# ru-wang/slam-plus-plus

Hardware: AMD Instinct MI355X
Metric: Λ-solve block-nnz/sec + batch GN iters/sec, Venice BA, 1→8 MI355X (higher is better)
Workload: dtype f64; 1 GPU; venice871-shaped synthetic BA (871 cams, 530304 points, 2838740 observations, LM-damped); nnzb=3369915, n=1596138, mode=schur+dense, n_reduced=5226, schur_pairs=12875640, parallelism=single GPU

## Files before the change

### include/spp_hip.h

```cpp
#ifndef SPP_HIP_H
#define SPP_HIP_H

#include <stddef.h>
#include <stdint.h>

#ifdef __cplusplus
extern "C" {
#endif

#define SPP_OK            0
#define SPP_NOT_POSDEF    1
#define SPP_E_BADARG     -1
#define SPP_E_NOMEM      -2
#define SPP_E_HIP        -3
#define SPP_E_NO_DEVICE  -4
#define SPP_E_STATE      -5
#define SPP_E_UNSUPPORTED -6

#define SPP_MODE_AUTO     0
#define SPP_MODE_SPARSE   1
#define SPP_MODE_SCHUR    2
#define SPP_MODE_SCHUR_SPARSE 3

#define SPP_FLAG_PROFILE  1
#define SPP_FLAG_SCHUR_PARTIAL 2

typedef struct spp_ctx spp_ctx;

spp_ctx *spp_create(int device, int flags);
void spp_destroy(spp_ctx *ctx);
int spp_free_memory(spp_ctx *ctx);
int spp_last_error(const spp_ctx *ctx, char *buf, size_t buf_size);
double *spp_host_staging(spp_ctx *ctx, int64_t n_doubles);
int spp_set_stream(spp_ctx *ctx, void *hip_stream);
int spp_synchronize(spp_ctx *ctx);

int spp_analyze(spp_ctx *ctx, int64_t nb, const int64_t *h_col_ptr, const int64_t *h_row_idx,
	const int64_t *h_blk_off, const int32_t *h_dim, int mode);

int spp_set_shard(spp_ctx *ctx, int rank, int world_size);

#define SPP_MODE_SCHUR_MIS 4

#define SPP_INFO_MODE           0
#define SPP_INFO_N              1
#define SPP_INFO_NNZB           2
#define SPP_INFO_NVALS          3
#define SPP_INFO_FACTOR_NNZ     4
#define SPP_INFO_FACTOR_FLOPS   5
#define SPP_INFO_N_REDUCED      6
#define SPP_INFO_N_POSES        7
#define SPP_INFO_N_LANDMARKS    8
#define SPP_INFO_SCHUR_PAIRS    9
#define SPP_INFO_N_OBS          10
#define SPP_INFO_SOLVE_BYTES    11
#define SPP_INFO_N_SUPERNODES   12
#define SPP_INFO_N_LEVELS       13
#define SPP_INFO_S_LD           14
#define SPP_INFO_S_NNZB         15
#define SPP_INFO_DENSE_STREAMED 16
#define SPP_INFO_LM_STREAM      17
#define SPP_INFO_BS_GROUPS      18
#define SPP_INFO_SCHUR_SIDE     19
#define SPP_INFO_S_CLEAR        20
#define SPP_INFO_S_DEVICE_PTR   21
#define SPP_INFO_ASM_HUB_CHUNK   22
#define SPP_INFO_SOLVE_ASYNC    23
#define SPP_INFO_FACTOR_KEPT    24
#define SPP_INFO_SPARSE_FACTOR_KEPT 25
#define SPP_INFO_SCHUR_SPARSE_FACTOR_KEPT 26
int spp_get_info(const spp_ctx *ctx, int what, int64_t *out);
int spp_get_ordering(const spp_ctx *ctx, int64_t *h_order);
int64_t spp_sparse_fronts(const spp_ctx *ctx, int64_t capacity, int32_t *h, int32_t *w, int32_t *pad, int32_t *cls, int32_t *level,
	int32_t *parent, int32_t *team);

#define SPP_ORDER_AMD 0
#define SPP_ORDER_ND  1
int spp_block_ordering(int64_t nb, const int64_t *col_ptr, const int64_t *row_idx, int method, int64_t *h_order);

int spp_schur_plan_host(int64_t nb, const int32_t *dim, const int64_t *col_ptr, const int64_t *row_idx, int shard_rank,
	int shard_world, int sparse_S, int64_t *out, double *seconds);

int spp_factor_solve(spp_ctx *ctx, const double *h_vals, double *h_rhs_inout);

int spp_factor_solve_device(spp_ctx *ctx, const double *d_vals, double *d_rhs_inout);

int spp_solve_device(spp_ctx *ctx, const double *d_vals, double *d_B, int64_t ldb, int64_t nrhs);
int spp_marginals_device(spp_ctx *ctx, const double *d_vals, int64_t n_sel, const int64_t *h_vertices, double *d_cov);

int spp_sparse_solve_device(spp_ctx *ctx, double *d_B, int64_t ldb, int64_t nrhs);
int spp_sparse_marginals_device(spp_ctx *ctx, int64_t n_sel, const int64_t *h_vertices, double *d_cov);
int spp_sparse_sigma_device(spp_ctx *ctx, double *d_sigma);

int spp_schur_sigma_device(spp_ctx *ctx, const double *d_vals, double *d_sigma);

int spp_schur_sparse_solve_device(spp_ctx *ctx, const double *d_vals, double *d_B, int64_t ldb, int64_t nrhs);
int spp_schur_sparse_marginals_device(spp_ctx *ctx, const double *d_vals, int64_t n_sel, const int64_t *h_vertices, double *d_cov);
int spp_schur_sparse_sigma_device(spp_ctx *ctx, const double *d_vals, double *d_sigma);

int spp_schur_buffer_size(const spp_ctx *ctx, int64_t *n_doubles);
int spp_schur_form(spp_ctx *ctx, const double *d_vals, const double *d_rhs, double *d_S_rhs);
int spp_schur_finish(spp_ctx *ctx, const double *d_vals, double *d_S_rhs, double *d_rhs_inout);
int spp_schur_packed_size(const spp_ctx *ctx, int64_t *n_doubles);
int spp_schur_pack(spp_ctx *ctx, const double *d_S_rhs, double *d_packed);
int spp_schur_unpack(spp_ctx *ctx, const double *d_packed, double *d_S_rhs);

int spp_assemble_analyze(spp_ctx *ctx, int64_t nv, const int32_t *h_dim,
	int64_t ne, const int64_t *h_v0, const int64_t *h_v1, int d0, int d1, int rd,
	int64_t unary_vertex);
int spp_assemble_get_structure(const spp_ctx *ctx, int64_t *h_col_ptr, int64_t *h_row_idx,
	int64_t *h_blk_off);
int spp_assemble_device(spp_ctx *ctx, const double *d_J0, const double *d_J1,
	const double *d_Omega, const double *d_r, double damping, double *d_vals_out, double *d_eta_out);
int spp_assemble_set_edge_weights(spp_ctx *ctx, const double *d_w);
#define SPP_MAX_EDGE_GROUPS 4
int spp_assemble_analyze_groups(spp_ctx *ctx, int64_t nv, const int32_t *h_dim, int n_groups,
	const int64_t *h_ne, const int64_t *const *h_v0, const int64_t *const *h_v1, const int64_t *const *h_seq,
	const int32_t *h_d0, const int32_t *h_d1, const int32_t *h_rd, int64_t unary_vertex);
int spp_assemble_groups_device(spp_ctx *ctx, const double *const *d_J0, const double *const *d_J1,
	const double *const *d_Omega, const double *const *d_r, double damping, double *d_vals_out, double *d_eta_out);
int spp_assemble_set_group_edge_weights(spp_ctx *ctx, int group, const double *d_w);
int spp_assemble_analyze_ternary(spp_ctx *ctx, int64_t nv, const int32_t *h_dim, int64_t ne, const int64_t *h_v0,
	const int64_t *h_v1, const int64_t *h_v2, int d0, int d1, int d2, int live2, int rd, int64_t unary_vertex);
int spp_assemble_ternary_device(spp_ctx *ctx, const double *d_J0, const double *d_J1, const double *d_J2,
	const double *d_Omega, const double *d_r, double damping, double *d_vals_out, double *d_eta_out);
int spp_edge_robust_weights_device(spp_ctx *ctx, int64_t n_edges, int rd, int kind, double scale, double param,
	const double *d_r, double *d_w_out);

int spp_se2_linearize_device(spp_ctx *ctx, int64_t n_edges, const int32_t *d_v0, const int32_t *d_v1,
	const double *d_poses, const double *d_measurements, double *d_J0, double *d_J1, double *d_r);
int spp_se2_update_device(spp_ctx *ctx, int64_t n_vertices, double *d_poses, const double *d_dx, int apply,
	double *h_dx_norm2);

int spp_se2_linearize_at_device(spp_ctx *ctx, int64_t n_edges, const int64_t *d_off0, const int64_t *d_off1,
	const double *d_state, const double *d_measurements, double *d_J0, double *d_J1, double *d_r);
int spp_se2_rb_linearize_device(spp_ctx *ctx, int64_t n_edges, const int64_t *d_pose_off, const int64_t *d_lm_off,
	const double *d_state, const double *d_measurements, double *d_J0, double *d_J1, double *d_r);
int spp_slam2d_update_device(spp_ctx *ctx, int64_t n, double *d_state, const double *d_dx, int64_t n_pose_angles,
	const int64_t *d_angle_off, int apply, double *h_dx_norm2);

int spp_se3_linearize_device(spp_ctx *ctx, int64_t n_edges, const int32_t *d_v0, const int32_t *d_v1,
	const double *d_poses, const double *d_measurements, double *d_J0, double *d_J1, double *d_r);
int spp_se3_update_device(spp_ctx *ctx, int64_t n_vertices, double *d_poses, const double *d_dx, int apply,
	double *h_dx_norm2);

int spp_se3_linearize_at_device(spp_ctx *ctx, int64_t n_edges, const int64_t *d_off0, const int64_t *d_off1,
	const double *d_state, const double *d_measurements, double *d_J0, double *d_J1, double *d_r);
int spp_se3_xyz_linearize_device(spp_ctx *ctx, int64_t n_edges, const int64_t *d_pose_off, const int64_t *d_lm_off,
	const double *d_state, const double *d_measurements, double *d_J0, double *d_J1, double *d_r);
int spp_slam3d_update_device(spp_ctx *ctx, int64_t n, double *d_state, const double *d_dx, int64_t n_poses,
	const int64_t *d_pose_off, int apply, double *h_dx_norm2);

int spp_rocv_range_linearize_device(spp_ctx *ctx, int64_t n_edges, const int64_t *d_recv_off, const int64_t *d_lm_off,
	const double *d_state, const double *d_measurements, double *d_J0, double *d_J1, double *d_r);
int spp_rocv_cv_linearize_device(spp_ctx *ctx, int64_t n_edges, const int64_t *d_off0, const int64_t *d_off1,
	const double *d_state, const double *d_dt, double *d_J0, double *d_J1, double *d_r);

int spp_ba_linearize_device(spp_ctx *ctx, int64_t n_obs, const int32_t *d_cam_of, const int32_t *d_pt_of,
	const double *d_cams, const double *d_intrinsics, const double *d_points, const double *d_measurements,
	double *d_J0, double *d_J1, double *d_r);
int spp_ba_update_device(spp_ctx *ctx, int64_t n_cams, double *d_cams, const int64_t *d_cam_dxoff,
	int64_t n_points, double *d_points, const int64_t *d_pt_dxoff, const double *d_dx, int64_t n_dx, int apply,
	double *h_dx_norm2);

int spp_sim3_ba_linearize_device(spp_ctx *ctx, int64_t n_obs, const int32_t *d_cam_of, const int32_t *d_pt_of,
	const double *d_cams, const double *d_intrinsics, const double *d_points, const double *d_measurements,
	double *d_J0, double *d_J1, double *d_r);
int spp_sim3_update_device(spp_ctx *ctx, int64_t n_cams, double *d_cams, const int64_t *d_cam_dxoff,
	int64_t n_points, double *d_points, const int64_t *d_pt_dxoff, const double *d_dx, int64_t n_dx, int apply,
	double *h_dx_norm2);

int spp_ba_stereo_linearize_device(spp_ctx *ctx, int64_t n_obs, const int32_t *d_cam_of, const int32_t *d_pt_of,
	const double *d_cams, const double *d_intrinsics, const double *d_points, const double *d_measurements,
	double *d_J0, double *d_J1, double *d_r);

int spp_ba_intrinsics_linearize_device(spp_ctx *ctx, int64_t n_obs, const int32_t *d_cam_of, const int32_t *d_pt_of,
	const int32_t *d_intr_of, const double *d_cams, const double *d_intrinsics, const double *d_points,
	const double *d_measurements, double *d_J0, double *d_J1, double *d_J2, double *d_r);
int spp_ba_intrinsics_update_device(spp_ctx *ctx, int64_t n_intrinsics, double *d_intrinsics, const int64_t *d_intr_dxoff,
	const double *d_dx, int apply, double *h_dx_norm2);

int spp_edge_chi2_device(spp_ctx *ctx, int64_t n_edges, int rd, const double *d_r, const double *d_Omega, double *h_chi2);
int spp_edge_hessian_maxdiag_device(spp_ctx *ctx, int64_t n_edges, int rd, int d0, int d1, const double *d_J0,
	const double *d_J1, const double *d_Omega, double *h_max);
int spp_lm_gain_denominator_device(spp_ctx *ctx, int64_t n, const double *d_dx, const double *d_eta, double alpha,
	double *h_out);

int spp_device_malloc(spp_ctx *ctx, size_t bytes, void **d_ptr);
int spp_device_free(spp_ctx *ctx, void *d_ptr);
int spp_memcpy_h2d(spp_ctx *ctx, void *d_dst, const void *h_src, size_t bytes);
int spp_memcpy_d2h(spp_ctx *ctx, void *h_dst, const void *d_src, size_t bytes);
int spp_memcpy_d2d(spp_ctx *ctx, void *d_dst, const void *d_src, size_t bytes);

int spp_set_profiling(spp_ctx *ctx, int on);

#define SPP_PHASE_PERMUTE   0
#define SPP_PHASE_SCHUR_INV 1
#define SPP_PHASE_SCHUR_GEMM 2
#define SPP_PHASE_SCHUR_RHS 3
#define SPP_PHASE_FACTOR    4
#define SPP_PHASE_TRISOLVE  5
#define SPP_PHASE_BACKSUBST 6
#define SPP_PHASE_ASSEMBLE  7
#define SPP_PHASE_TOTAL     8
#define SPP_N_PHASES        9
int spp_get_phase_ms(spp_ctx *ctx, double *ms_out );
int spp_get_dominant_kernel(spp_ctx *ctx, double *ms_total, int64_t *n_launches, double *flops);

int spp_microbench_copy(spp_ctx *ctx, size_t bytes, int iters, double *gb_per_s);
int spp_microbench_mfma_f64(spp_ctx *ctx, int iters, double *tflops);
int spp_microbench_ctile(spp_ctx *ctx, int n, int iters, double *gb_per_s);
int spp_microbench_update(spp_ctx *ctx, int64_t m, int iters, double *ms_per_launch);

int spp_dense_potrf_upper(spp_ctx *ctx, double *d_A, int64_t n, int64_t ld);
int spp_dense_posv(spp_ctx *ctx, double *d_A, int64_t n, int64_t ld, double *d_b);
int spp_dense_posv_multi(spp_ctx *ctx, double *d_A, int64_t n, int64_t ld, double *d_B, int64_t ldb, int64_t nrhs);
int spp_dense_potri(spp_ctx *ctx, double *d_A, int64_t n, int64_t ld, double *d_Z, int64_t ldz);
int spp_schur_sigma_dense_device(spp_ctx *ctx);
int spp_schur_sparse_sigma_inverse_device(spp_ctx *ctx);
int spp_dense_posv_masked(spp_ctx *ctx, double *d_A, int64_t n, int64_t ld, double *d_b, const uint64_t *words, int64_t nwords);
int spp_tile_mask_host(int64_t n, int bs, int64_t nblk, const int32_t *i1, const int32_t *i2, int has_rhs, int fill,
	uint64_t *words, int64_t *n_updates);
int spp_schur_tile_mask_host(int64_t nb, const int32_t *dim, const int64_t *col_ptr, const int64_t *row_idx, int shard_rank,
	int shard_world, uint64_t *words);
int spp_schur_cam_order_host(int64_t nb, const int32_t *dim, const int64_t *col_ptr, const int64_t *row_idx, int shard_rank,
	int shard_world, int flags, const int64_t *order_in, int64_t *cam_order, double *figures);
int spp_tail_order_host(int64_t n, int has_rhs, const uint64_t *words, int64_t nwords, int resident, int early, double beta,
	int32_t *table, int32_t *info);
int spp_tail_plan_host(int64_t n, int has_rhs, const uint64_t *words, int64_t nwords, const int32_t *step_order, int64_t norder,
	int front, int tail_rows, int resident, int early, double beta, uint64_t *rowbits, int32_t *steps, int32_t *table, int32_t *info);
int spp_dense_posv_ordered(spp_ctx *ctx, double *d_A, int64_t n, int64_t ld, double *d_b, const uint64_t *words, int64_t nwords,
	const int32_t *step_order);
int spp_tail_step_order_host(int64_t n, const uint64_t *words, int64_t nwords, int32_t *step_order);
int spp_schur_step_order_host(int64_t nb, const int32_t *dim, const int64_t *col_ptr, const int64_t *row_idx, int shard_rank,
	int shard_world, int flags, int32_t *step_order);
int spp_dense_gemm_tn_sub(spp_ctx *ctx, int64_t m, int64_t n, int64_t k,
	const double *d_A, int64_t lda, const double *d_B, int64_t ldb, double *d_C, int64_t ldc);
int spp_dense_gemm_tn_sub_upper(spp_ctx *ctx, int64_t m, int64_t n, int64_t k,
	const double *d_A, int64_t lda, const double *d_B, int64_t ldb, double *d_C, int64_t ldc);
int spp_dense_front_factor(spp_ctx *ctx, double *d_F, int64_t ld, int64_t w, int64_t h, double *d_image);

const char *spp_version(void);

#ifdef __cplusplus
}
#endif
#endif
```

### slam_plus_plus_amd/api.py

```python
import ctypes
import os

import numpy as np

_HERE = os.path.dirname(os.path.abspath(__file__))
LIB_PATH = os.environ.get("SPP_LIB") or os.path.join(_HERE, "libspp_hip.so")

SPP_OK, SPP_NOT_POSDEF = 0, 1
MODE_AUTO, MODE_SPARSE, MODE_SCHUR, MODE_SCHUR_SPARSE, MODE_SCHUR_MIS = 0, 1, 2, 3, 4
FLAG_PROFILE = 1
INFO = dict(MODE=0, N=1, NNZB=2, NVALS=3, FACTOR_NNZ=4, FACTOR_FLOPS=5, N_REDUCED=6, N_POSES=7,
            N_LANDMARKS=8, SCHUR_PAIRS=9, N_OBS=10, SOLVE_BYTES=11, N_SUPERNODES=12, N_LEVELS=13, S_LD=14, S_NNZB=15, DENSE_STREAMED=16,
            LM_STREAM=17, BS_GROUPS=18, SCHUR_SIDE=19, S_CLEAR=20, S_DEVICE_PTR=21, ASM_HUB_CHUNK=22, SOLVE_ASYNC=23, FACTOR_KEPT=24,
            SPARSE_FACTOR_KEPT=25, SCHUR_SPARSE_FACTOR_KEPT=26)
PHASES = ["permute", "schur_inv", "schur_gemm", "schur_rhs", "factor", "trisolve", "backsubst", "assemble", "total"]

EXPORTS = [
    "spp_create", "spp_destroy", "spp_free_memory", "spp_last_error", "spp_host_staging", "spp_set_stream", "spp_synchronize",
    "spp_analyze", "spp_set_shard", "spp_get_info", "spp_get_ordering", "spp_sparse_fronts", "spp_factor_solve",
    "spp_factor_solve_device", "spp_solve_device", "spp_marginals_device", "spp_sparse_solve_device", "spp_sparse_marginals_device", "spp_sparse_sigma_device",
    "spp_schur_sigma_device", "spp_dense_potri", "spp_schur_sigma_dense_device",
    "spp_schur_sparse_solve_device", "spp_schur_sparse_marginals_device", "spp_schur_sparse_sigma_device",
    "spp_schur_sparse_sigma_inverse_device",
    "spp_schur_buffer_size", "spp_schur_form", "spp_schur_finish",
    "spp_schur_packed_size", "spp_schur_pack", "spp_schur_unpack",
    "spp_assemble_analyze", "spp_assemble_get_structure", "spp_assemble_device", "spp_assemble_set_edge_weights",
    "spp_assemble_analyze_groups", "spp_assemble_groups_device", "spp_assemble_set_group_edge_weights",
    "spp_assemble_analyze_ternary", "spp_assemble_ternary_device", "spp_ba_intrinsics_linearize_device",
    "spp_ba_intrinsics_update_device",
    "spp_se2_linearize_at_device", "spp_se2_rb_linearize_device", "spp_slam2d_update_device",
    "spp_se3_linearize_at_device", "spp_se3_xyz_linearize_device", "spp_slam3d_update_device", "spp_rocv_range_linearize_device",
    "spp_rocv_cv_linearize_device", "spp_device_malloc",
    "spp_device_free", "spp_memcpy_h2d", "spp_memcpy_d2h", "spp_memcpy_d2d", "spp_get_phase_ms", "spp_get_dominant_kernel",
    "spp_microbench_copy", "spp_microbench_mfma_f64", "spp_microbench_ctile", "spp_microbench_update", "spp_block_ordering", "spp_schur_plan_host", "spp_set_profiling", "spp_se2_linearize_device", "spp_se2_update_device", "spp_ba_linearize_device", "spp_ba_stereo_linearize_device", "spp_ba_update_device", "spp_sim3_ba_linearize_device", "spp_sim3_update_device", "spp_se3_linearize_device", "spp_se3_update_device", "spp_edge_chi2_device", "spp_edge_robust_weights_device", "spp_edge_hessian_maxdiag_device",
    "spp_lm_gain_denominator_device", "spp_dense_potrf_upper", "spp_dense_posv", "spp_dense_posv_multi",
    "spp_dense_posv_masked", "spp_tile_mask_host", "spp_schur_tile_mask_host", "spp_tail_order_host", "spp_tail_plan_host", "spp_schur_cam_order_host",
    "spp_dense_posv_ordered", "spp_tail_step_order_host", "spp_schur_step_order_host",
    "spp_dense_gemm_tn_sub", "spp_dense_gemm_tn_sub_upper", "spp_dense_front_factor", "spp_version",
]

_lib = None
_c_i64p = ctypes.POINTER(ctypes.c_int64)
_c_i32p = ctypes.POINTER(ctypes.c_int32)
_c_f64p = ctypes.POINTER(ctypes.c_double)


class SppError(RuntimeError):
    """std::runtime_error of the C++ adapter (reference LinearSolver_Schur_GPU.cpp:734-797)."""


def load_library():
    global _lib
    if _lib is not None:
        return _lib
    if not os.path.exists(LIB_PATH):
        raise SppError("libspp_hip.so is not built: run `python -m slam_plus_plus_amd.build` "
                       "(hipcc --offload-arch=gfx950); there is no CPU fallback")
    lib = ctypes.CDLL(LIB_PATH)
    vp, i64, i32, dbl, cint = ctypes.c_void_p, ctypes.c_int64, ctypes.c_int32, ctypes.c_double, ctypes.c_int
    sig = {
        "spp_create": (vp, [cint, cint]),
        "spp_destroy": (None, [vp]),
        "spp_free_memory": (cint, [vp]),
        "spp_last_error": (cint, [vp, ctypes.c_char_p, ctypes.c_size_t]),
        "spp_host_staging": (vp, [vp, i64]),
        "spp_set_stream": (cint, [vp, vp]),
        "spp_synchronize": (cint, [vp]),
        "spp_analyze": (cint, [vp, i64, vp, vp, vp, vp, cint]),
        "spp_set_shard": (cint, [vp, cint, cint]),
        "spp_get_info": (cint, [vp, cint, _c_i64p]),
        "spp_get_ordering": (cint, [vp, vp]),
        "spp_sparse_fronts": (i64, [vp, i64, vp, vp, vp, vp, vp, vp, vp]),
        "spp_factor_solve": (cint, [vp, vp, vp]),
        "spp_factor_solve_device": (cint, [vp, vp, vp]),
        "spp_solve_device": (cint, [vp, vp, vp, i64, i64]),
        "spp_marginals_device": (cint, [vp, vp, i64, vp, vp]),
        "spp_sparse_solve_device": (cint, [vp, vp, i64, i64]),
        "spp_sparse_marginals_device": (cint, [vp, i64, vp, vp]),
        "spp_sparse_sigma_device": (cint, [vp, vp]),
        "spp_schur_sigma_device": (cint, [vp, vp, vp]),
        "spp_schur_sigma_dense_device": (cint, [vp]),
        "spp_schur_sparse_solve_device": (cint, [vp, vp, vp, i64, i64]),
        "spp_schur_sparse_marginals_device": (cint, [vp, vp, i64, vp, vp]),
        "spp_schur_sparse_sigma_device": (cint, [vp, vp, vp]),
        "spp_schur_sparse_sigma_inverse_device": (cint, [vp]),
        "spp_dense_potri": (cint, [vp, vp, i64, i64, vp, i64]),
        "spp_schur_buffer_size": (cint, [vp, _c_i64p]),
        "spp_schur_form": (cint, [vp, vp, vp, vp]),
        "spp_schur_finish": (cint, [vp, vp, vp, vp]),
        "spp_schur_packed_size": (cint, [vp, _c_i64p]),
        "spp_schur_pack": (cint, [vp, vp, vp]),
        "spp_schur_unpack": (cint, [vp, vp, vp]),
        "spp_assemble_analyze": (cint, [vp, i64, vp, i64, vp, vp, cint, cint, cint, i64]),
        "spp_assemble_get_structure": (cint, [vp, vp, vp, vp]),
        "spp_assemble_device": (cint, [vp, vp, vp, vp, vp, dbl, vp, vp]),
        "spp_assemble_set_edge_weights": (cint, [vp, vp]),
        "spp_assemble_analyze_groups": (cint, [vp, i64, vp, cint, vp, vp, vp, vp, vp, vp, vp, i64]),
        "spp_assemble_groups_device": (cint, [vp, vp, vp, vp, vp, dbl, vp, vp]),
        "spp_assemble_set_group_edge_weights": (cint, [vp, cint, vp]),
        "spp_assemble_analyze_ternary": (cint, [vp, i64, vp, i64, vp, vp, vp, cint, cint, cint, cint, cint, i64]),
        "spp_assemble_ternary_device": (cint, [vp, vp, vp, vp, vp, vp, dbl, vp, vp]),
        "spp_ba_intrinsics_linearize_device": (cint, [vp, i64, vp, vp, vp, vp, vp, vp, vp, vp, vp, vp, vp]),
        "spp_ba_intrinsics_update_device": (cint, [vp, i64, vp, vp, vp, cint, _c_f64p]),
        "spp_se2_linearize_at_device": (cint, [vp, i64, vp, vp, vp, vp, vp, vp, vp]),
        "spp_se2_rb_linearize_device": (cint, [vp, i64, vp, vp, vp, vp, vp, vp, vp]),
        "spp_slam2d_update_device": (cint, [vp, i64, vp, vp, i64, vp, cint, _c_f64p]),
        "spp_se3_linearize_at_device": (cint, [vp, i64, vp, vp, vp, vp, vp, vp, vp]),
        "spp_se3_xyz_linearize_device": (cint, [vp, i64, vp, vp, vp, vp, vp, vp, vp]),
        "spp_slam3d_update_device": (cint, [vp, i64, vp, vp, i64, vp, cint, _c_f64p]),
        "spp_rocv_range_linearize_device": (cint, [vp, i64, vp, vp, vp, vp, vp, vp, vp]),
        "spp_rocv_cv_linearize_device": (cint, [vp, i64, vp, vp, vp, vp, vp, vp, vp]),
        "spp_device_malloc": (cint, [vp, ctypes.c_size_t, ctypes.POINTER(vp)]),
        "spp_device_free": (cint, [vp, vp]),
        "spp_memcpy_h2d": (cint, [vp, vp, vp, ctypes.c_size_t]),
        "spp_memcpy_d2h": (cint, [vp, vp, vp, ctypes.c_size_t]),
        "spp_memcpy_d2d": (cint, [vp, vp, vp, ctypes.c_size_t]),
        "spp_get_phase_ms": (cint, [vp, _c_f64p]),
        "spp_get_dominant_kernel": (cint, [vp, _c_f64p, _c_i64p, _c_f64p]),
        "spp_microbench_copy": (cint, [vp, ctypes.c_size_t, cint, _c_f64p]),
        "spp_microbench_mfma_f64": (cint, [vp, cint, _c_f64p]),
        "spp_microbench_ctile": (cint, [vp, cint, cint, _c_f64p]),
        "spp_microbench_update": (cint, [vp, ctypes.c_int64, cint, _c_f64p]),
        "spp_block_ordering": (cint, [ctypes.c_int64, vp, vp, cint, vp]),
        "spp_schur_plan_host": (cint, [ctypes.c_int64, vp, vp, vp, cint, cint, cint, vp, vp]),
        "spp_set_profiling": (cint, [vp, cint]),
        "spp_se2_linearize_device": (cint, [vp, ctypes.c_int64, vp, vp, vp, vp, vp, vp, vp]),
        "spp_se2_update_device": (cint, [vp, ctypes.c_int64, vp, vp, cint, _c_f64p]),
        "spp_se3_linearize_device": (cint, [vp, ctypes.c_int64, vp, vp, vp, vp, vp, vp, vp]),
        "spp_se3_update_device": (cint, [vp, ctypes.c_int64, vp, vp, cint, _c_f64p]),
        "spp_edge_chi2_device": (cint, [vp, ctypes.c_int64, cint, vp, vp, _c_f64p]),
        "spp_edge_robust_weights_device": (cint, [vp, ctypes.c_int64, cint, cint, dbl, dbl, vp, vp]),
        "spp_edge_hessian_maxdiag_device": (cint, [vp, ctypes.c_int64, cint, cint, cint, vp, vp, vp, _c_f64p]),
        "spp_lm_gain_denominator_device": (cint, [vp, ctypes.c_int64, vp, vp, ctypes.c_double, _c_f64p]),
        "spp_ba_linearize_device": (cint, [vp, ctypes.c_int64, vp, vp, vp, vp, vp, vp, vp, vp, vp]),
        "spp_ba_stereo_linearize_device": (cint, [vp, ctypes.c_int64, vp, vp, vp, vp, vp, vp, vp, vp, vp]),
        "spp_ba_update_device": (cint, [vp, ctypes.c_int64, vp, vp, ctypes.c_int64, vp, vp, vp, ctypes.c_int64, cint, _c_f64p]),
        "spp_sim3_ba_linearize_device": (cint, [vp, ctypes.c_int64, vp, vp, vp, vp, vp, vp, vp, vp, vp]),
        "spp_sim3_update_device": (cint, [vp, ctypes.c_int64, vp, vp, ctypes.c_int64, vp, vp, vp, ctypes.c_int64, cint, _c_f64p]),
        "spp_dense_potrf_upper": (cint, [vp, vp, i64, i64]),
        "spp_dense_posv": (cint, [vp, vp, i64, i64, vp]),
        "spp_dense_posv_multi": (cint, [vp, vp, i64, i64, vp, i64, i64]),
        "spp_dense_posv_masked": (cint, [vp, vp, i64, i64, vp, vp, i64]),
        "spp_tile_mask_host": (cint, [i64, cint, i64, vp, vp, cint, cint, vp, vp]),
        "spp_schur_tile_mask_host": (cint, [i64, vp, vp, vp, cint, cint, vp]),
        "spp_tail_order_host": (cint, [i64, cint, vp, i64, cint, cint, dbl, vp, vp]),
        "spp_tail_plan_host": (cint, [i64, cint, vp, i64, vp, i64, cint, cint, cint, cint, dbl, vp, vp, vp, vp]),
        "spp_schur_cam_order_host": (cint, [i64, vp, vp, vp, cint, cint, cint, vp, vp, vp]),
        "spp_dense_posv_ordered": (cint, [vp, vp, i64, i64, vp, vp, i64, vp]),
        "spp_tail_step_order_host": (cint, [i64, vp, i64, vp]),
        "spp_schur_step_order_host": (cint, [i64, vp, vp, vp, cint, cint, cint, vp]),
        "spp_dense_gemm_tn_sub": (cint, [vp, i64, i64, i64, vp, i64, vp, i64, vp, i64]),
        "spp_dense_gemm_tn_sub_upper": (cint, [vp, i64, i64, i64, vp, i64, vp, i64, vp, i64]),
        "spp_dense_front_factor": (cint, [vp, vp, i64, i64, i64, vp]),
        "spp_version": (ctypes.c_char_p, []),
    }
    for name, (res, args) in sig.items():
        fn = getattr(lib, name)
        fn.restype = res
        fn.argtypes = args
    _lib = lib
    return lib


def _ptr(a):
    return a.ctypes.data_as(ctypes.c_void_p)


ORDER_AMD, ORDER_ND = 0, 1


def block_ordering(lam, method=ORDER_AMD):
    lib = load_library()
    col_ptr = np.ascontiguousarray(lam.col_ptr, dtype=np.int64)
    row_idx = np.ascontiguousarray(lam.row_idx, dtype=np.int64)
    out = np.empty(lam.nb, dtype=np.int64)
    code = lib.spp_block_ordering(lam.nb, _ptr(col_ptr), _ptr(row_idx), method, _ptr(out))
    if code != 0:
        raise SppError("spp_block_ordering failed: %d" % code)
    return out


def schur_plan_host(lam, shard_rank=0, shard_world=1, sparse_S=False, mis=False):
    lib = load_library()
    col_ptr = np.ascontiguousarray(lam.col_ptr, dtype=np.int64)
    row_idx = np.ascontiguousarray(lam.row_idx, dtype=np.int64)
    dim = np.ascontiguousarray(lam.dim, dtype=np.int32)
    out = np.zeros(9, dtype=np.int64)
    sec = ctypes.c_double(0.0)
    code = lib.spp_schur_plan_host(lam.nb, _ptr(dim), _ptr(col_ptr), _ptr(row_idx), shard_rank, shard_world,
                                   (1 if sparse_S else 0) | (2 if mis else 0), _ptr(out), ctypes.byref(sec))
    if code != 0:
        raise SppError("spp_schur_plan_host failed: %d" % code)
    keys = ("nc", "nl", "no", "n_pairs", "n_sblk", "n_items", "n_multi", "checksum", "checksum_all")
    d = dict(zip(keys, (int(v) for v in out)))
    d["seconds"] = sec.value
    return d


def tile_mask_host(n, bs, i1, i2, has_rhs=True, fill=True):
    lib = load_library()
    i1 = np.ascontiguousarray(i1, dtype=np.int32)
    i2 = np.ascontiguousarray(i2, dtype=np.int32)
    words = np.zeros(64, dtype=np.uint64)
    upd = ctypes.c_int64(0)
    code = lib.spp_tile_mask_host(n, bs, i1.size, _ptr(i1), _ptr(i2), 1 if has_rhs else 0, 1 if fill else 0, _ptr(words),
                                  ctypes.byref(upd))
    if code < 0:
        raise SppError("spp_tile_mask_host failed: %d" % code)
    return words[:code].copy(), upd.value


def schur_tile_mask_host(lam, shard_rank=0, shard_world=1):
    lib = load_library()
    col_ptr = np.ascontiguousarray(lam.col_ptr, dtype=np.int64)
    row_idx = np.ascontiguousarray(lam.row_idx, dtype=np.int64)
    dim = np.ascontiguousarray(lam.dim, dtype=np.int32)
    words = np.zeros(64, dtype=np.uint64)
    code = lib.spp_schur_tile_mask_host(lam.nb, _ptr(dim), _ptr(col_ptr), _ptr(row_idx), shard_rank, shard_world, _ptr(words))
    if code < 0:
        raise SppError("spp_schur_tile_mask_host failed: %d" % code)
    return words[:code].copy()


def schur_cam_order_host(lam, order=None, sparse_S=False, mis=False, shard_rank=0, shard_world=1):
    lib = load_library()
    col_ptr = np.ascontiguousarray(lam.col_ptr, dtype=np.int64)
    row_idx = np.ascontiguousarray(lam.row_idx, dtype=np.int64)
    dim = np.ascontiguousarray(lam.dim, dtype=np.int32)
    nc = int((dim == dim.max()).sum()) if not mis else int(dim.size)
    out = np.full(max(nc, 1), -1, dtype=np.int64)
    fig = np.zeros(8, dtype=np.float64)
    oin = None if order is None else np.ascontiguousarray(order, dtype=np.int64)
    if oin is not None and oin.size != nc:
        raise SppError("schur_cam_order_host: order must list every camera once")
    code = lib.spp_schur_cam_order_host(lam.nb, _ptr(dim), _ptr(col_ptr), _ptr(row_idx), shard_rank, shard_world,
                                        (1 if sparse_S else 0) | (2 if mis else 0),
                                        _ptr(oin) if oin is not None else None, _ptr(out), _ptr(fig))
    if code < 0:
        raise SppError("spp_schur_cam_order_host failed: %d" % code)
    keys = ("tiles", "updates", "path", "cost_us")
    natural = dict(zip(keys, (int(fig[0]), int(fig[1]), int(fig[2]), float(fig[3]))))
    chosen = dict(zip(keys, (int(fig[4]), int(fig[5]), int(fig[6]), float(fig[7]))))
    return out[out >= 0], bool(code), natural, chosen


def tail_order_host(n, words, has_rhs=True, resident=256, early=True, beta=0.0):
    lib = load_library()
    words = np.ascontiguousarray(words if words is not None else [], dtype=np.uint64)
    table = np.zeros(64 * 65 // 2 + 64, dtype=np.int32)
    info = np.zeros(5, dtype=np.int32)
    code = lib.spp_tail_order_host(int(n), 1 if has_rhs else 0, _ptr(words) if words.size else None, words.size, int(resident),
                                   int(early), float(beta), _ptr(table), _ptr(info))
    if code < 0:
        raise SppError("spp_tail_order_host failed: %d" % code)
    tiles = [(int(t) >> 16, int(t) & 0xffff) for t in table[:code]]
    return tiles, dict(zip(("n_early", "r_star", "rows_resident", "live_demand", "widest"), (int(v) for v in info)))


TAIL_NO_STEP = 127
SPP_E_BADARG = -1


def tail_plan_host(n, words, step_order=None, front=0, has_rhs=True, tail_rows=44, resident=256, early=3, beta=0.0, tail_mask=True):
    lib = load_library()
    words = np.ascontiguousarray(words if words is not None else [], dtype=np.uint64)
    so = np.ascontiguousarray(step_order if step_order is not None else [], dtype=np.int32)
    rowbits = np.zeros(65, dtype=np.uint64)
    steps = np.zeros(72, dtype=np.int32)
    table = np.zeros(64 * 65 // 2 + 64, dtype=np.int32)
    info = np.zeros(5, dtype=np.int32)
    code = lib.spp_tail_plan_host(int(n), 1 if has_rhs else 0, _ptr(words) if words.size else None, words.size,
                                  _ptr(so) if so.size else None, so.size, int(front), int(tail_rows), int(resident),
                                  int(early) | (0 if tail_mask else 4), float(beta), _ptr(rowbits), _ptr(steps), _ptr(table), _ptr(info))
    if code < 0:
        err = SppError("spp_tail_plan_host failed: %d" % code)
        err.code = code
        raise err
    if code == 0:
        return None
    tr = -(-int(n) // 128) - int(front)
    return {"rowbits": [int(w) for w in rowbits[:tr + 1]], "steps": steps.tolist(),
            "tiles": [(int(t) >> 16, int(t) & 0xffff) for t in table[:code]],
            "info": dict(zip(("n_early", "r_star", "rows_resident", "live_demand", "widest"), (int(v) for v in info)))}


def tail_step_order_host(n, words):
    lib = load_library()
    words = np.ascontiguousarray(words, dtype=np.uint64)
    out = np.zeros(64, dtype=np.int32)
    code = lib.spp_tail_step_order_host(int(n), _ptr(words), words.size, _ptr(out))
    if code < 0:
        raise SppError("spp_tail_step_order_host failed: %d" % code)
    return out[:code].copy()


def schur_step_order_host(lam, sparse_S=False, mis=False, shard_rank=0, shard_world=1):
    lib = load_library()
    col_ptr = np.ascontiguousarray(lam.col_ptr, dtype=np.int64)
    row_idx = np.ascontiguousarray(lam.row_idx, dtype=np.int64)
    dim = np.ascontiguousarray(lam.dim, dtype=np.int32)
    out = np.zeros(64, dtype=np.int32)
    code = lib.spp_schur_step_order_host(lam.nb, _ptr(dim), _ptr(col_ptr), _ptr(row_idx), shard_rank, shard_world,
                                         (1 if sparse_S else 0) | (2 if mis else 0), _ptr(out))
    if code < 0:
        raise SppError("spp_schur_step_order_host failed: %d" % code)
    return out[:code].copy()


class DeviceArray:

    def __init__(self, ctx, n, dtype=np.float64):
        self.ctx, self.n, self.dtype = ctx, int(n), np.dtype(dtype)
        p = ctypes.c_void_p()
        ctx._check(ctx.lib.spp_device_malloc(ctx.h, self.n * self.dtype.itemsize, ctypes.byref(p)))
        self.ptr = p.value

    @classmethod
    def from_host(cls, ctx, arr):
        arr = np.ascontiguousarray(arr)
        d = cls(ctx, arr.size, arr.dtype)
        d.upload(arr)
        return d

    def upload(self, arr):
        arr = np.ascontiguousarray(arr, dtype=self.dtype)
        assert arr.size == self.n
        self.ctx._check(self.ctx.lib.spp_memcpy_h2d(self.ctx.h, self.ptr, _ptr(arr), arr.nbytes))

    def download(self):
        out = np.empty(self.n, dtype=self.dtype)
        self.ctx._check(self.ctx.lib.spp_memcpy_d2h(self.ctx.h, _ptr(out), self.ptr, out.nbytes))
        return out

    def copy_from(self, other):
        assert other.n * other.dtype.itemsize <= self.n * self.dtype.itemsize
        self.ctx._check(self.ctx.lib.spp_memcpy_d2d(self.ctx.h, self.ptr, other.ptr, other.n * other.dtype.itemsize))

    def free(self):
        if self.ptr:
            self.ctx.lib.spp_device_free(self.ctx.h, self.ptr)
            self.ptr = None


class Context:

    def __init__(self, device=0, flags=0):
        self.lib = load_library()
        self.h = self.lib.spp_create(int(device), int(flags))
        if not self.h:
            raise SppError("spp_create failed: no usable HIP device %d (the solver has no CPU fallback)" % device)

    def close(self):
        if getattr(self, "h", None):
            self.lib.spp_destroy(self.h)
            self.h = None

    def __del__(self):
        try:
            self.close()
        except Exception:
            pass

    def last_error(self):
        buf = ctypes.create_string_buffer(1024)
        self.lib.spp_last_error(self.h, buf, 1024)
        return buf.value.decode(errors="replace")

    def _check(self, code):
        if code < 0:
            if code == -2:
                raise MemoryError(self.last_error())
            raise SppError("spp error %d: %s" % (code, self.last_error()))
        return code

    def analyze(self, bcsc, mode=MODE_AUTO):
        self._keep = bcsc
        return self._check(self.lib.spp_analyze(self.h, bcsc.nb, _ptr(bcsc.col_ptr), _ptr(bcsc.row_idx),
                                                 _ptr(bcsc.blk_off), _ptr(bcsc.dim), mode))

    def set_shard(self, rank, world):
        return self._check(self.lib.spp_set_shard(self.h, rank, world))

    def info(self, key):
        out = ctypes.c_int64()
        self._check(self.lib.spp_get_info(self.h, INFO[key], ctypes.byref(out)))
        return out.value

    def ordering(self, nb):
        out = np.empty(nb, dtype=np.int64)
        self._check(self.lib.spp_get_ordering(self.h, _ptr(out)))
        return out

    def sparse_fronts(self):
        keys = ("h", "w", "pad", "cls", "level", "parent", "team")
        ns = self._check(self.lib.spp_sparse_fronts(self.h, 0, None, None, None, None, None, None, None))
        out = {k: np.zeros(ns, dtype=np.int32) for k in keys}
        if ns:
            self._check(self.lib.spp_sparse_fronts(self.h, ns, *[_ptr(out[k]) for k in keys]))
        return out

    def se2_linearize_device(self, n_edges, d_v0, d_v1, d_poses, d_meas, d_J0, d_J1, d_r):
        return self._check(self.lib.spp_se2_linearize_device(self.h, n_edges, d_v0, d_v1, d_poses, d_meas, d_J0, d_J1, d_r))

    def se2_update_device(self, n_vertices, d_poses, d_dx, apply=True):
        out = ctypes.c_double()
        self._check(self.lib.spp_se2_update_device(self.h, n_vertices, d_poses, d_dx, 1 if apply else 0, ctypes.byref(out)))
        return out.value ** 0.5

    def se2_linearize_at_device(self, n_edges, d_off0, d_off1, d_state, d_meas, d_J0, d_J1, d_r):
        return self._check(self.lib.spp_se2_linearize_at_device(self.h, n_edges, d_off0, d_off1, d_state, d_meas, d_J0, d_J1, d_r))

    def se2_rb_linearize_device(self, n_edges, d_pose_off, d_lm_off, d_state, d_meas, d_J0, d_J1, d_r):
        return self._check(self.lib.spp_se2_rb_linearize_device(self.h, n_edges, d_pose_off, d_lm_off, d_state, d_meas, d_J0, d_J1, d_r))

    def slam2d_update_device(self, n, d_state, d_dx, n_pose_angles, d_angle_off, apply=True):
        out = ctypes.c_double()
        self._check(self.lib.spp_slam2d_update_device(self.h, n, d_state, d_dx, n_pose_angles, d_angle_off, 1 if apply else 0,
                                                      ctypes.byref(out)))
        return out.value ** 0.5

    def se3_linearize_at_device(self, n_edges, d_off0, d_off1, d_state, d_meas, d_J0, d_J1, d_r):
        return self._check(self.lib.spp_se3_linearize_at_device(self.h, n_edges, d_off0, d_off1, d_state, d_meas, d_J0, d_J1, d_r))

    def se3_xyz_linearize_device(self, n_edges, d_pose_off, d_lm_off, d_state, d_meas, d_J0, d_J1, d_r):
        return self._check(self.lib.spp_se3_xyz_linearize_device(self.h, n_edges, d_pose_off, d_lm_off, d_state, d_meas, d_J0, d_J1, d_r))

    def slam3d_update_device(self, n, d_state, d_dx, n_poses, d_pose_off, apply=True):
        out = ctypes.c_double()
        self._check(self.lib.spp_slam3d_update_device(self.h, n, d_state, d_dx, n_poses, d_pose_off, 1 if apply else 0,
                                                      ctypes.byref(out)))
        return out.value ** 0.5

    def rocv_range_linearize_device(self, n_edges, d_recv_off, d_lm_off, d_state, d_meas, d_J0, d_J1, d_r):
        return self._check(self.lib.spp_rocv_range_linearize_device(self.h, n_edges, d_recv_off, d_lm_off, d_state, d_meas, d_J0, d_J1, d_r))

    def rocv_cv_linearize_device(self, n_edges, d_off0, d_off1, d_state, d_dt, d_J0, d_J1, d_r):
        return self._check(self.lib.spp_rocv_cv_linearize_device(self.h, n_edges, d_off0, d_off1, d_state, d_dt, d_J0, d_J1, d_r))

# ... 346 lines not shown
```

### slam_plus_plus_amd/csrc/spp_api.cpp

```cpp

#include "spp_internal.h"
#include <string.h>
#include <new>

using namespace spp;

namespace spp {

void phases_reset(spp_ctx *ctx)
{
	if(!(ctx->flags & SPP_FLAG_PROFILE))
		return;
	if(!ctx->timer.created) {
		for(int i = 0; i < 2 * SPP_N_PHASES; ++ i)
			SPP_HIP_CHECK(hipEventCreate(&ctx->timer.ev[i]));
		ctx->timer.created = true;
	}
	for(int i = 0; i < SPP_N_PHASES; ++ i) {
		ctx->timer.used[i] = false;
		ctx->phase_ms[i] = 0;
	}
	ctx->dom_used = 0;
	ctx->dom_flops = 0;
}

void phase_begin(spp_ctx *ctx, int phase)
{
	if(!(ctx->flags & SPP_FLAG_PROFILE) || !ctx->timer.created)
		return;
	SPP_HIP_CHECK(hipEventRecord(ctx->timer.ev[2 * phase], ctx->stream));
}

void phase_end(spp_ctx *ctx, int phase)
{
	if(!(ctx->flags & SPP_FLAG_PROFILE) || !ctx->timer.created)
		return;
	SPP_HIP_CHECK(hipEventRecord(ctx->timer.ev[2 * phase + 1], ctx->stream));
	ctx->timer.used[phase] = true;
}

void phases_collect(spp_ctx *ctx)
{
	if(!(ctx->flags & SPP_FLAG_PROFILE) || !ctx->timer.created)
		return;
	SPP_HIP_CHECK(hipStreamSynchronize(ctx->stream));
	for(int i = 0; i < SPP_N_PHASES; ++ i) {
		if(!ctx->timer.used[i])
			continue;
		float ms = 0;
		if(hipEventElapsedTime(&ms, ctx->timer.ev[2 * i], ctx->timer.ev[2 * i + 1]) == hipSuccess)
			ctx->phase_ms[i] = ms;
	}
}

void dom_begin(spp_ctx *ctx)
{
	if(!(ctx->flags & SPP_FLAG_PROFILE))
		return;
	if(ctx->dom_used + 2 > ctx->dom_events.size()) {
		size_t old = ctx->dom_events.size();
		ctx->dom_events.resize(old + 64);
		for(size_t i = old; i < ctx->dom_events.size(); ++ i)
			SPP_HIP_CHECK(hipEventCreate(&ctx->dom_events[i]));
	}
	SPP_HIP_CHECK(hipEventRecord(ctx->dom_events[ctx->dom_used], ctx->stream));
}

void dom_end(spp_ctx *ctx, double flops)
{
	if(!(ctx->flags & SPP_FLAG_PROFILE))
		return;
	SPP_HIP_CHECK(hipEventRecord(ctx->dom_events[ctx->dom_used + 1], ctx->stream));
	ctx->dom_used += 2;
	ctx->dom_flops += flops;
}

}

static inline void drop_kept_factors(spp_ctx *ctx)
{
	ctx->schur.factor_kept = false;
	ctx->schur.sparse_factor_kept = false;
	ctx->sparse_factor_kept = false;
}

static void ctx_drain(spp_ctx *ctx)
{
	(void)hipStreamSynchronize(ctx->stream);
	if(ctx->side_stream)
		(void)hipStreamSynchronize(ctx->side_stream);
	ctx->status_pending = false;
}

#define SPP_TRY(ctx) try {
#define SPP_CATCH(ctx) } catch(const spp::Error &e) { if(ctx) (ctx)->last_error = e.what(); return e.code; } \
	catch(const std::bad_alloc &) { if(ctx) (ctx)->last_error = "host allocation failed"; return SPP_E_NOMEM; } \
	catch(const std::exception &e) { if(ctx) (ctx)->last_error = e.what(); return SPP_E_HIP; }

static inline void store_if(double *h_out, double value)
{
	if(h_out)
		*h_out = value;
}

template <class Body>
static int geometry_call(spp_ctx *ctx, Body body)
{
	SPP_TRY(ctx)
	SPP_HIP_CHECK(hipSetDevice(ctx->device));
	body();
	return SPP_OK;
	SPP_CATCH(ctx)
}

extern "C" {

const char *spp_version(void)
{
	return "slam_plus_plus_amd 0.1 (gfx950, fp64)";
}

spp_ctx *spp_create(int device, int flags)
{
	int count = 0;
	if(hipGetDeviceCount(&count) != hipSuccess || count <= 0 || device < 0 || device >= count)
		return nullptr;
	if(hipSetDevice(device) != hipSuccess)
		return nullptr;
	spp_ctx *ctx = new(std::nothrow) spp_ctx;
	if(!ctx)
		return nullptr;
	ctx->device = device;
	ctx->flags = flags;
	if(hipStreamCreateWithFlags(&ctx->stream, hipStreamNonBlocking) != hipSuccess) {
		delete ctx;
		return nullptr;
	}
	ctx->own_stream = true;
	return ctx;
}

int spp_free_memory(spp_ctx *ctx)
{
	if(!ctx)
		return SPP_E_BADARG;
	SPP_TRY(ctx)
	(void)hipSetDevice(ctx->device);
	ctx_drain(ctx);
	drop_kept_factors(ctx);
	ctx->schur.release_all();
	sparse_release(ctx);
	assemble_release(ctx);
	ctx->dense.trsm_w.release();
	ctx->again_panel.release();
	ctx->again_cols.release();
	ctx->again_rows.release();
	ctx->dense.tinv.release();
	ctx->dense.tinv_all.release();
	ctx->dense.xtmp.release();
	ctx->dense.la_cnt.release();
	ctx->dense.la_trace.release();
	ctx->geom_partial.release();
	ctx->dense.flags.release();
	ctx->dense.trsv_pay.release();
	ctx->dense.trsv_m.release();
	ctx->dense.tail_pub.release();
	ctx->dense.tail_order.release();
	ctx->dense.tail_plan.key = TailPlan::Key();
	ctx->dense.tail_dinv.release();
	ctx->dense.tail_epoch = 0;
	ctx->dense.epoch = 0;
	ctx->dense.sync.release();
	ctx->dense.fuse_cnt.release();
	ctx->dense.fuse_expect.clear();
	ctx->dense.sync_epoch = 0;
	ctx->d_vals.release();
	ctx->d_rhs.release();
	ctx->mode = -1;
	return SPP_OK;
	SPP_CATCH(ctx)
}

void spp_destroy(spp_ctx *ctx)
{
	if(!ctx)
		return;
	if(ctx->plan_trash.joinable())
		ctx->plan_trash.join();
	spp_free_memory(ctx);
	ctx->dense.info.release();
	if(ctx->dense.aux) {
		dense_aux_park(ctx->device, ctx->dense.aux);
		(void)hipEventDestroy(ctx->dense.ev[0]);
		(void)hipEventDestroy(ctx->dense.ev[1]);
	}
	if(ctx->dense.chain) {
		(void)hipStreamDestroy(ctx->dense.chain);
		if(ctx->dense.ev_chain)
			(void)hipEventDestroy(ctx->dense.ev_chain);
	}
	if(ctx->side_stream) {
		(void)hipStreamDestroy(ctx->side_stream);
		(void)hipEventDestroy(ctx->side_ev[0]);
		(void)hipEventDestroy(ctx->side_ev[1]);
	}
	for(int i = 0; i < 2; ++ i)
		if(ctx->status_ev[i])
			(void)hipEventDestroy(ctx->status_ev[i]);
	if(ctx->h_status)
		(void)hipHostFree(ctx->h_status);
	if(ctx->dense.h_chain_err)
		(void)hipHostFree(ctx->dense.h_chain_err);
	if(ctx->h_staging)
		(void)hipHostFree(ctx->h_staging);
	if(ctx->timer.created)
		for(int i = 0; i < 2 * SPP_N_PHASES; ++ i)
			(void)hipEventDestroy(ctx->timer.ev[i]);
	for(size_t i = 0; i < ctx->dom_events.size(); ++ i)
		(void)hipEventDestroy(ctx->dom_events[i]);
	if(ctx->own_stream && ctx->stream)
		(void)hipStreamDestroy(ctx->stream);
	delete ctx;
}

int spp_last_error(const spp_ctx *ctx, char *buf, size_t buf_size)
{
	if(!ctx || !buf || !buf_size)
		return SPP_E_BADARG;
	strncpy(buf, ctx->last_error.c_str(), buf_size - 1);
	buf[buf_size - 1] = 0;
	return SPP_OK;
}

double *spp_host_staging(spp_ctx *ctx, int64_t n_doubles)
{
	if(!ctx || n_doubles < 0)
		return nullptr;
	if((size_t)n_doubles <= ctx->h_staging_cap && ctx->h_staging)
		return ctx->h_staging;
	(void)hipSetDevice(ctx->device);
	(void)hipStreamSynchronize(ctx->stream);
	if(ctx->h_staging) {
		(void)hipHostFree(ctx->h_staging);
		ctx->h_staging = nullptr;
		ctx->h_staging_cap = 0;
	}
	const size_t want = (size_t)(n_doubles > 0 ? n_doubles : 1);
	if(hipHostMalloc((void**)&ctx->h_staging, want * sizeof(double), hipHostMallocDefault) != hipSuccess) {
		(void)hipGetLastError();
		ctx->h_staging = nullptr;
		ctx->last_error = "hipHostMalloc of the staging buffer failed";
		return nullptr;
	}
	ctx->h_staging_cap = want;
	return ctx->h_staging;
}

int spp_set_stream(spp_ctx *ctx, void *hip_stream)
{
	if(!ctx)
		return SPP_E_BADARG;
	ctx_drain(ctx);
	if(ctx->own_stream && ctx->stream)
		(void)hipStreamDestroy(ctx->stream);
	ctx->stream = (hipStream_t)hip_stream;
	ctx->own_stream = false;
	return SPP_OK;
}

int spp_synchronize(spp_ctx *ctx)
{
	if(!ctx)
		return SPP_E_BADARG;
	SPP_TRY(ctx)
	SPP_HIP_CHECK(hipStreamSynchronize(ctx->stream));
	dense_chain_check(ctx);
	return SPP_OK;
	SPP_CATCH(ctx)
}

int spp_set_profiling(spp_ctx *ctx, int on)
{
	if(!ctx)
		return SPP_E_BADARG;
	ctx->flags = on ? (ctx->flags | SPP_FLAG_PROFILE) : (ctx->flags & ~SPP_FLAG_PROFILE);
	return SPP_OK;
}

int spp_set_shard(spp_ctx *ctx, int rank, int world_size)
{
	if(!ctx || world_size < 1 || rank < 0 || rank >= world_size)
		return SPP_E_BADARG;
	drop_kept_factors(ctx);
	ctx->shard_rank = rank;
	ctx->shard_world = world_size;
	return SPP_OK;
}

int spp_analyze(spp_ctx *ctx, int64_t nb, const int64_t *col_ptr, const int64_t *row_idx,
	const int64_t *blk_off, const int32_t *dim, int mode)
{
	if(!ctx)
		return SPP_E_BADARG;
	SPP_TRY(ctx)
	SPP_REQUIRE(nb > 0 && col_ptr && row_idx && blk_off && dim, SPP_E_BADARG, "spp_analyze: null or empty structure");
	SPP_REQUIRE(col_ptr[0] == 0 && col_ptr[nb] >= nb, SPP_E_BADARG, "spp_analyze: column pointers must start at 0 and hold every diagonal block");
	SPP_HIP_CHECK(hipSetDevice(ctx->device));
	ctx->mode = -1;
	drop_kept_factors(ctx);
	ctx_drain(ctx);
	VClock clk("spp_analyze");
	Structure st;
	st.nb = nb;
	st.nnzb = col_ptr[nb];
	st.col_ptr.assign(col_ptr, col_ptr + nb + 1);
	SPP_REQUIRE(st.nnzb >= nb, SPP_E_BADARG, "spp_analyze: fewer blocks than block columns");
	for(int64_t j = 0; j < nb; ++ j)
		SPP_REQUIRE(col_ptr[j + 1] > col_ptr[j], SPP_E_BADARG, "every block column needs its diagonal block");
	st.dim.assign(dim, dim + nb);
	st.base.resize(nb + 1);
	st.base[0] = 0;
	for(int64_t j = 0; j < nb; ++ j) {
		SPP_REQUIRE(dim[j] > 0 && dim[j] <= 8, SPP_E_BADARG, "block widths must be in 1..8");
		st.base[j + 1] = st.base[j] + dim[j];
	}
	st.n = st.base[nb];
	st.row_idx.resize(st.nnzb);
	st.blk_off.resize(st.nnzb);
	{
		const int nt = plan_threads(st.nnzb);
		std::vector<int64_t> jcut, nvals_t(nt, 0);
		balanced_cuts(st.col_ptr, nt, jcut);
		run_threads(nt, [&](int t) {
			const int64_t p0 = col_ptr[jcut[t]], p1 = col_ptr[jcut[t + 1]];
			if(p1 > p0) {
				memcpy(st.row_idx.data() + p0, row_idx + p0, (size_t)(p1 - p0) * sizeof(int64_t));
				memcpy(st.blk_off.data() + p0, blk_off + p0, (size_t)(p1 - p0) * sizeof(int64_t));
			}
			int64_t nv = 0;
			for(int64_t j = jcut[t]; j < jcut[t + 1]; ++ j) {
				for(int64_t p = col_ptr[j]; p < col_ptr[j + 1]; ++ p) {
					const int64_t i = row_idx[p];
					SPP_REQUIRE(i >= 0 && i <= j, SPP_E_BADARG, "only the upper triangle may be stored");
					SPP_REQUIRE(p == col_ptr[j] || row_idx[p - 1] < i, SPP_E_BADARG, "rows must ascend within a column");
					SPP_REQUIRE(blk_off[p] >= 0, SPP_E_BADARG, "negative block offset");
					nv = std::max<int64_t>(nv, blk_off[p] + (int64_t)dim[i] * dim[j]);
				}
				SPP_REQUIRE(row_idx[col_ptr[j + 1] - 1] == j, SPP_E_BADARG, "diagonal block missing (must be last in its column)");
			}
			nvals_t[t] = nv;
		});
		st.nvals = 0;
		for(int t = 0; t < nt; ++ t)
			st.nvals = std::max(st.nvals, nvals_t[t]);
	}
	ctx->st = std::move(st);
	Structure &st_ref = ctx->st;
	clk.lap("structure copied + validated");
	ctx->schur.release_all();
	sparse_release(ctx);
	clk.lap("old plans released");
	int dp, dl;
	int chosen = mode;
	if(mode == SPP_MODE_AUTO) {
		chosen = SPP_MODE_SPARSE;
		if(schur_applicable(st_ref, &dp, &dl)) {
			int64_t n_red = 0;
			for(int64_t j = 0; j < nb; ++ j)
				n_red += (dim[j] == dp) ? dp : 0;
			chosen = (n_red <= 16384) ? SPP_MODE_SCHUR : SPP_MODE_SCHUR_SPARSE;
		}
	}
	SPP_REQUIRE(chosen == SPP_MODE_SCHUR || chosen == SPP_MODE_SPARSE || chosen == SPP_MODE_SCHUR_SPARSE ||
		chosen == SPP_MODE_SCHUR_MIS, SPP_E_BADARG, "unknown mode");
	SPP_REQUIRE((chosen != SPP_MODE_SPARSE && chosen != SPP_MODE_SCHUR_MIS) || ctx->shard_world == 1, SPP_E_UNSUPPORTED,
		"only the Schur modes shard (over landmarks); pose graphs run as replicas (DESIGN.md, multi-GPU)");
	ctx->mode = -1;
	if(chosen == SPP_MODE_SCHUR || chosen == SPP_MODE_SCHUR_SPARSE || chosen == SPP_MODE_SCHUR_MIS) {
		const bool mis = chosen == SPP_MODE_SCHUR_MIS;
		const bool sparse_S = chosen != SPP_MODE_SCHUR;
		build_schur_plan(ctx, sparse_S, mis);
		clk.lap("schur plan (all of it)");
		ctx->schur.mis = mis;
		ctx->order.clear();
		ctx->order.reserve((size_t)st_ref.nb);
		if(sparse_S) {
			sparse_analyze(ctx, ctx->schur.s_st);
			std::vector<int64_t> red = ctx->order;
			ctx->order.clear();
			for(size_t i = 0; i < red.size(); ++ i)
				ctx->order.push_back(ctx->schur.pose_block[red[i]]);
			chosen = SPP_MODE_SCHUR;
		} else
		for(size_t i = 0; i < ctx->schur.pose_block.size(); ++ i)
			ctx->order.push_back(ctx->schur.pose_block[i]);
		for(int64_t j = 0; j < st_ref.nb; ++ j)
			if(ctx->schur.is_lm[j])
				ctx->order.push_back(j);
	} else
		sparse_analyze(ctx, ctx->st);
	ctx->mode = chosen;
	clk.lap("plan + ordering");
	return SPP_OK;
	SPP_CATCH(ctx)
}

int spp_get_info(const spp_ctx *ctx, int what, int64_t *out)
{
	if(!ctx || !out)
		return SPP_E_BADARG;
	if(ctx->mode < 0 && what != SPP_INFO_NNZB && what != SPP_INFO_NVALS && what != SPP_INFO_N && what != SPP_INFO_DENSE_STREAMED &&
	   what != SPP_INFO_ASM_HUB_CHUNK && what != SPP_INFO_FACTOR_KEPT && what != SPP_INFO_SPARSE_FACTOR_KEPT &&
	   what != SPP_INFO_SCHUR_SPARSE_FACTOR_KEPT)
		return SPP_E_STATE;
	switch(what) {
	case SPP_INFO_MODE: *out = (ctx->mode != SPP_MODE_SCHUR) ? ctx->mode : ctx->schur.mis ? SPP_MODE_SCHUR_MIS :
		ctx->schur.sparse_S ? SPP_MODE_SCHUR_SPARSE : SPP_MODE_SCHUR; break;
	case SPP_INFO_N: *out = ctx->st.n; break;
	case SPP_INFO_NNZB: *out = ctx->st.nnzb; break;
	case SPP_INFO_NVALS: *out = ctx->st.nvals; break;
	case SPP_INFO_FACTOR_NNZ: *out = ctx->factor_nnz; break;
	case SPP_INFO_FACTOR_FLOPS: *out = ctx->factor_flops; break;
	case SPP_INFO_N_REDUCED: *out = (ctx->mode == SPP_MODE_SCHUR) ? ctx->schur.n_red : 0; break;
	case SPP_INFO_N_POSES: *out = (ctx->mode == SPP_MODE_SCHUR) ? ctx->schur.nc : ctx->st.nb; break;
	case SPP_INFO_N_LANDMARKS: *out = (ctx->mode == SPP_MODE_SCHUR) ? ctx->schur.nl : 0; break;
	case SPP_INFO_SCHUR_PAIRS: *out = (ctx->mode == SPP_MODE_SCHUR) ? ctx->schur.n_pairs : 0; break;
	case SPP_INFO_N_OBS: *out = (ctx->mode == SPP_MODE_SCHUR) ? ctx->schur.no : 0; break;
	case SPP_INFO_SOLVE_BYTES: *out = ctx->solve_bytes; break;
	case SPP_INFO_N_SUPERNODES: *out = ctx->sparse ? sparse_info(ctx, what) : 0; break;
	case SPP_INFO_N_LEVELS: *out = ctx->sparse ? sparse_info(ctx, what) : 0; break;
	case SPP_INFO_S_LD: *out = (ctx->mode == SPP_MODE_SCHUR && !ctx->schur.sparse_S) ? ctx->schur.ld : 0; break;
	case SPP_INFO_S_NNZB: *out = (ctx->mode == SPP_MODE_SCHUR) ? ctx->schur.n_sblk : 0; break;
	case SPP_INFO_DENSE_STREAMED: *out = ctx->dense.tail_rows_last; break;
	case SPP_INFO_LM_STREAM: *out = (ctx->mode == SPP_MODE_SCHUR) ? ctx->schur.lm_stream_last : 0; break;
	case SPP_INFO_BS_GROUPS: *out = (ctx->mode == SPP_MODE_SCHUR) ? ctx->schur.n_bs : 0; break;
	case SPP_INFO_SCHUR_SIDE: *out = (ctx->mode == SPP_MODE_SCHUR) ? ctx->schur.side_last : 0; break;
	case SPP_INFO_SOLVE_ASYNC: *out = (ctx->mode == SPP_MODE_SCHUR) ? ctx->schur.async_last : 0; break;
	case SPP_INFO_S_CLEAR: *out = (ctx->mode == SPP_MODE_SCHUR) ? ctx->schur.clear_last : 0; break;
	case SPP_INFO_S_DEVICE_PTR: *out = (ctx->mode == SPP_MODE_SCHUR) ? (int64_t)(uintptr_t)ctx->schur.S.p : 0; break;
	case SPP_INFO_ASM_HUB_CHUNK: *out = ASM_HUB_CHUNK; break;
	case SPP_INFO_FACTOR_KEPT: *out = (ctx->mode == SPP_MODE_SCHUR && ctx->schur.factor_kept) ? 1 : 0; break;
	case SPP_INFO_SPARSE_FACTOR_KEPT: *out = (ctx->mode == SPP_MODE_SPARSE && ctx->sparse_factor_kept) ? 1 : 0; break;
	case SPP_INFO_SCHUR_SPARSE_FACTOR_KEPT: *out = (ctx->mode == SPP_MODE_SCHUR && ctx->schur.sparse_factor_kept) ? 1 : 0; break;
	default: return SPP_E_BADARG;
	}
	return SPP_OK;
}

int spp_get_ordering(const spp_ctx *ctx, int64_t *h_order)
{
	if(!ctx || !h_order)
		return SPP_E_BADARG;
	if(ctx->mode < 0)
		return SPP_E_STATE;
	for(size_t i = 0; i < ctx->order.size(); ++ i)
		h_order[i] = ctx->order[i];
	return SPP_OK;
}

int64_t spp_sparse_fronts(const spp_ctx *ctx, int64_t capacity, int32_t *h, int32_t *w, int32_t *pad, int32_t *cls, int32_t *level,
	int32_t *parent, int32_t *team)
{
	if(!ctx || capacity < 0)
		return SPP_E_BADARG;
#ifdef SPP_HAVE_SPARSE
	if(ctx->sparse)
		return sparse_fronts(ctx, capacity, h, w, pad, cls, level, parent, team);
#endif
	return 0;
}

int spp_block_ordering(int64_t nb, const int64_t *col_ptr, const int64_t *row_idx, int method, int64_t *h_order)
{
	if(nb <= 0 || !col_ptr || !row_idx || !h_order || (method != SPP_ORDER_AMD && method != SPP_ORDER_ND))
		return SPP_E_BADARG;
	try {
		for(int64_t j = 0; j < nb; ++ j)
			for(int64_t p = col_ptr[j]; p < col_ptr[j + 1]; ++ p)
				if(row_idx[p] < 0 || row_idx[p] > j)
					return SPP_E_BADARG;
		std::vector<int64_t> order;
		if(method == SPP_ORDER_AMD)
			min_degree_order(nb, col_ptr, row_idx, order);
		else
			nested_dissection_order(nb, col_ptr, row_idx, order);
		for(int64_t k = 0; k < nb; ++ k)
			h_order[k] = order[k];
		return SPP_OK;
	} catch(const std::bad_alloc &) {
		return SPP_E_NOMEM;
	} catch(...) {
		return SPP_E_HIP;
	}
}

static bool structure_of_pattern(int64_t nb, const int32_t *dim, const int64_t *col_ptr, const int64_t *row_idx, Structure &st)
{
	st.nb = nb;
	st.nnzb = col_ptr[nb];
	st.col_ptr.assign(col_ptr, col_ptr + nb + 1);
	st.row_idx.assign(row_idx, row_idx + st.nnzb);
	st.dim.assign(dim, dim + nb);
	st.base.resize(nb + 1);
	st.base[0] = 0;
	for(int64_t j = 0; j < nb; ++ j)
		st.base[j + 1] = st.base[j] + dim[j];
	st.n = st.base[nb];
	st.blk_off.resize(st.nnzb);
	int64_t off = 0;
	for(int64_t j = 0; j < nb; ++ j)
		for(int64_t p = col_ptr[j]; p < col_ptr[j + 1]; ++ p) {
			if(row_idx[p] < 0 || row_idx[p] > j)
				return false;
			st.blk_off[p] = off;
			off += (int64_t)dim[row_idx[p]] * dim[j];
		}
	st.nvals = off;
	return true;
}

extern "C++" {
template <class F>
static int schur_host_entry(int64_t nb, const int32_t *dim, const int64_t *col_ptr, const int64_t *row_idx, int shard_rank,
	int shard_world, const void *out, F fn)
{
	if(nb <= 0 || !dim || !col_ptr || !row_idx || !out || shard_world < 1 || shard_rank < 0 || shard_rank >= shard_world)
		return SPP_E_BADARG;
	try {
		Structure st;
		if(!structure_of_pattern(nb, dim, col_ptr, row_idx, st))
			return SPP_E_BADARG;
		return fn(st);
	} catch(const Error &e) {
		return e.code;
	} catch(const std::bad_alloc &) {
		return SPP_E_NOMEM;
	} catch(...) {
		return SPP_E_HIP;
	}
}
}

int spp_schur_plan_host(int64_t nb, const int32_t *dim, const int64_t *col_ptr, const int64_t *row_idx, int shard_rank,
	int shard_world, int sparse_S, int64_t *out, double *seconds)
{
	return schur_host_entry(nb, dim, col_ptr, row_idx, shard_rank, shard_world, out, [&](const Structure &st) {
		const double sec = schur_plan_host_probe(st, shard_rank, shard_world, (sparse_S & 1) != 0, (sparse_S & 2) != 0, out);
		if(seconds)
			*seconds = sec;
		return (int)SPP_OK;
	});
}

int spp_schur_tile_mask_host(int64_t nb, const int32_t *dim, const int64_t *col_ptr, const int64_t *row_idx, int shard_rank,
	int shard_world, uint64_t *words)
{
	return schur_host_entry(nb, dim, col_ptr, row_idx, shard_rank, shard_world, words, [&](const Structure &st) {
		std::vector<uint64_t> w;
		schur_tile_mask_host_probe(st, w);
		for(size_t q = 0; q < w.size(); ++ q)
			words[q] = w[q];
		return (int)w.size();
	});
}

int spp_schur_cam_order_host(int64_t nb, const int32_t *dim, const int64_t *col_ptr, const int64_t *row_idx, int shard_rank,
	int shard_world, int flags, const int64_t *order_in, int64_t *cam_order, double *figures)
{
	if(!figures)
		return SPP_E_BADARG;
	return schur_host_entry(nb, dim, col_ptr, row_idx, shard_rank, shard_world, cam_order, [&](const Structure &st) {
		if(order_in) {
			int64_t nc = 0;
			const int dmax = *std::max_element(dim, dim + nb);
			for(int64_t j = 0; j < nb; ++ j)
				nc += dim[j] == dmax;
			std::vector<char> seen((size_t)nc, 0);
			for(int64_t q = 0; q < nc; ++ q) {
				if(order_in[q] < 0 || order_in[q] >= nc || seen[order_in[q]])
					return (int)SPP_E_BADARG;
				seen[order_in[q]] = 1;
			}
		}
		std::vector<int32_t> order;
		TileDagCost cost[2];
		const bool used = schur_cam_order_host_probe(st, shard_rank, shard_world, (flags & 1) != 0, (flags & 2) != 0, order_in, order, cost);
// ... 783 lines not shown
	SPP_TRY(ctx)
	SPP_HIP_CHECK(hipSetDevice(ctx->device));
	*gb_per_s = microbench_ctile(ctx, n, iters);
	return SPP_OK;
	SPP_CATCH(ctx)
}

int spp_microbench_update(spp_ctx *ctx, int64_t m, int iters, double *ms_per_launch)
{
	if(!ctx || !ms_per_launch || m < 128 || iters < 1)
		return SPP_E_BADARG;
	SPP_TRY(ctx)
	SPP_HIP_CHECK(hipSetDevice(ctx->device));
	*ms_per_launch = microbench_update(ctx, m, iters);
	return SPP_OK;
	SPP_CATCH(ctx)
}

int spp_microbench_mfma_f64(spp_ctx *ctx, int iters, double *tflops)
{
	if(!ctx || !tflops)
		return SPP_E_BADARG;
	SPP_TRY(ctx)
	SPP_HIP_CHECK(hipSetDevice(ctx->device));
	*tflops = microbench_mfma_f64(ctx, iters);
	return SPP_OK;
	SPP_CATCH(ctx)
}

int spp_dense_potrf_upper(spp_ctx *ctx, double *d_A, int64_t n, int64_t ld)
{
	if(!ctx || !d_A || n <= 0 || ld < n)
		return SPP_E_BADARG;
	SPP_TRY(ctx)
	drop_kept_factors(ctx);
	SPP_HIP_CHECK(hipSetDevice(ctx->device));
	const int64_t ldp = ((n + 1 + DENSE_NB - 1) / DENSE_NB) * DENSE_NB;
	DevBuf<double> tmp;
	tmp.reserve((size_t)ldp * ldp);
	SPP_HIP_CHECK(hipMemsetAsync(tmp.p, 0, (size_t)ldp * ldp * sizeof(double), ctx->stream));
	SPP_HIP_CHECK(hipMemcpy2DAsync(tmp.p, ldp * sizeof(double), d_A, ld * sizeof(double), n * sizeof(double), n,
		hipMemcpyDeviceToDevice, ctx->stream));
	dense_set_padding(ctx, tmp.p, ldp, n);
	int ret = dense_potrf_upper(ctx, tmp.p, n, ldp, true);
	SPP_HIP_CHECK(hipMemcpy2DAsync(d_A, ld * sizeof(double), tmp.p, ldp * sizeof(double), n * sizeof(double), n,
		hipMemcpyDeviceToDevice, ctx->stream));
	SPP_HIP_CHECK(hipStreamSynchronize(ctx->stream));
	return ret;
	SPP_CATCH(ctx)
}

int spp_dense_posv_multi(spp_ctx *ctx, double *d_A, int64_t n, int64_t ld, double *d_B, int64_t ldb, int64_t nrhs)
{
	if(!ctx || !d_A || !d_B || n <= 0 || ld < n || ldb < n || nrhs < 1)
		return SPP_E_BADARG;
	SPP_TRY(ctx)
	drop_kept_factors(ctx);
	SPP_HIP_CHECK(hipSetDevice(ctx->device));
	const int64_t ldp = ((n + 1 + DENSE_NB - 1) / DENSE_NB) * DENSE_NB;
	DevBuf<double> tmp;
	tmp.reserve((size_t)ldp * ldp);
	SPP_HIP_CHECK(hipMemsetAsync(tmp.p, 0, (size_t)ldp * ldp * sizeof(double), ctx->stream));
	SPP_HIP_CHECK(hipMemcpy2DAsync(tmp.p, ldp * sizeof(double), d_A, ld * sizeof(double), n * sizeof(double), n,
		hipMemcpyDeviceToDevice, ctx->stream));
	dense_set_padding(ctx, tmp.p, ldp, n);
	int ret = dense_potrf_upper(ctx, tmp.p, n, ldp, true);
	if(ret == SPP_OK)
		dense_potrs_multi(ctx, tmp.p, n, ldp, d_B, ldb, nrhs);
	SPP_HIP_CHECK(hipMemcpy2DAsync(d_A, ld * sizeof(double), tmp.p, ldp * sizeof(double), n * sizeof(double), n,
		hipMemcpyDeviceToDevice, ctx->stream));
	SPP_HIP_CHECK(hipStreamSynchronize(ctx->stream));
	return ret;
	SPP_CATCH(ctx)
}

int spp_dense_potri(spp_ctx *ctx, double *d_A, int64_t n, int64_t ld, double *d_Z, int64_t ldz)
{
	if(!ctx || !d_A || !d_Z || n <= 0 || ld < n || ldz < n)
		return SPP_E_BADARG;
	SPP_TRY(ctx)
	drop_kept_factors(ctx);
	SPP_HIP_CHECK(hipSetDevice(ctx->device));
	const int64_t ldp = ((n + 1 + DENSE_NB - 1) / DENSE_NB) * DENSE_NB;
	DevBuf<double> tmp;
	tmp.reserve((size_t)ldp * ldp);
	SPP_HIP_CHECK(hipMemsetAsync(tmp.p, 0, (size_t)ldp * ldp * sizeof(double), ctx->stream));
	SPP_HIP_CHECK(hipMemcpy2DAsync(tmp.p, ldp * sizeof(double), d_A, ld * sizeof(double), n * sizeof(double), n,
		hipMemcpyDeviceToDevice, ctx->stream));
	dense_set_padding(ctx, tmp.p, ldp, n);
	int ret = dense_potrf_upper(ctx, tmp.p, n, ldp, true);
	if(ret == SPP_OK)
		dense_potri_upper(ctx, tmp.p, n, ldp, d_Z, ldz);
	SPP_HIP_CHECK(hipMemcpy2DAsync(d_A, ld * sizeof(double), tmp.p, ldp * sizeof(double), n * sizeof(double), n,
		hipMemcpyDeviceToDevice, ctx->stream));
	SPP_HIP_CHECK(hipStreamSynchronize(ctx->stream));
	return ret;
	SPP_CATCH(ctx)
}

int spp_dense_posv(spp_ctx *ctx, double *d_A, int64_t n, int64_t ld, double *d_b)
{
	return spp_dense_posv_masked(ctx, d_A, n, ld, d_b, nullptr, 0);
}

int spp_tile_mask_host(int64_t n, int bs, int64_t nblk, const int32_t *i1, const int32_t *i2, int has_rhs, int fill,
	uint64_t *words, int64_t *n_updates)
{
	if(n <= 0 || bs <= 0 || nblk < 0 || (nblk && (!i1 || !i2)) || !words)
		return SPP_E_BADARG;
	try {
		std::vector<uint64_t> w;
		tile_mask_mark(n, bs, nblk, i1, i2, w);
		const int64_t upd = tile_mask_close(n, has_rhs != 0, fill != 0, w);
		if(n_updates)
			*n_updates = upd;
		for(size_t q = 0; q < w.size(); ++ q)
			words[q] = w[q];
		return (int)w.size();
	} catch(...) {
		return SPP_E_NOMEM;
	}
}

int spp_tail_plan_host(int64_t n, int has_rhs, const uint64_t *words, int64_t nwords, const int32_t *step_order, int64_t norder,
	int front, int tail_rows, int resident, int early, double beta, uint64_t *rowbits, int32_t *steps, int32_t *table, int32_t *info)
{
	const int64_t nsteps = (n + DENSE_NB - 1) / DENSE_NB;
	if(n <= 0 || nwords < 0 || nwords > TAIL_MAX_ROWS || (nwords && (!words || nwords != nsteps)) || norder < 0 || (norder && !step_order) ||
	   front < 0 || !table || !(beta >= 0))
		return SPP_E_BADARG;
	try {
		const std::vector<uint64_t> mask(words, words + nwords);
		const std::vector<int32_t> order(step_order, step_order + norder);
		const TailSwitches sw = {tail_rows, (early & 4) ? 0 : 1, early & 1, (early >> 1) & 1, beta};
		const TailPlan p = tail_plan(nwords ? &mask : nullptr, norder ? &order : nullptr, nsteps, n, has_rhs ? n + 1 : n, (int64_t)front - 1,
			resident, sw);
		if(!p.applies)
			return 0;
		if(rowbits)
			std::copy(p.key.rowbits.begin(), p.key.rowbits.end(), rowbits);
		for(int q = 0; steps && q < 8 * TAIL_SORDER_WORDS; ++ q)
			steps[q] = tail_sorder_at(p.sorder, q);
		std::copy(p.table.begin(), p.table.end(), table);
		if(info)
			std::copy(p.info, p.info + 5, info);
		return (int)p.table.size();
	} catch(const Error &e) {
		return e.code;
	} catch(...) {
		return SPP_E_NOMEM;
	}
}

int spp_tail_order_host(int64_t n, int has_rhs, const uint64_t *words, int64_t nwords, int resident, int early, double beta,
	int32_t *table, int32_t *info)
{
	const int64_t Tr = (n + DENSE_NB - 1) / DENSE_NB, Tc = has_rhs ? n / DENSE_NB + 1 : Tr;
	if(n <= 0 || Tr > 64 || Tc > 64)
		return SPP_E_BADARG;
	try {
		std::vector<int32_t> order;
		if(nwords == Tr && words && (early & 2))
			tail_step_order(std::vector<uint64_t>(words, words + nwords), order);
		return spp_tail_plan_host(n, has_rhs, words, nwords, order.data(), (int64_t)order.size(), 0, TAIL_MAX_ROWS, resident, (early ? 1 : 0) | (early & 2), beta,
			nullptr, nullptr, table, info);
	} catch(...) {
		return SPP_E_NOMEM;
	}
}

int spp_tail_step_order_host(int64_t n, const uint64_t *words, int64_t nwords, int32_t *step_order)
{
	const int64_t Tr = (n + DENSE_NB - 1) / DENSE_NB;
	if(n <= 0 || n / DENSE_NB + 1 > 64 || !words || nwords != Tr || !step_order)
		return SPP_E_BADARG;
	try {
		std::vector<uint64_t> mask(words, words + nwords);
		tile_mask_close(n, true, true, mask);
		std::vector<int32_t> order;
		tail_step_order(mask, order);
		for(size_t q = 0; q < order.size(); ++ q)
			step_order[q] = order[q];
		return (int)order.size();
	} catch(...) {
		return SPP_E_NOMEM;
	}
}

static int dense_posv_entry(spp_ctx *ctx, double *d_A, int64_t n, int64_t ld, double *d_b, const uint64_t *words, int64_t nwords,
	const int32_t *step_order)
{
	if(!ctx || !d_A || !d_b || n <= 0 || ld < n || nwords < 0 || (nwords && !words))
		return SPP_E_BADARG;
	SPP_TRY(ctx)
	drop_kept_factors(ctx);
	SPP_HIP_CHECK(hipSetDevice(ctx->device));
	std::vector<uint64_t> mask(words, words + nwords);
	std::vector<int32_t> order;
	if(nwords) {
		SPP_REQUIRE(nwords == (n + DENSE_NB - 1) / DENSE_NB, SPP_E_BADARG, "posv: one mask word per tile row of 128");
		tile_mask_close(n, true, true, mask);
	}
	if(step_order) {
		SPP_REQUIRE(is_permutation(step_order, nwords), SPP_E_BADARG, "posv: the step order must be a permutation of the tile rows 0 .. nwords - 1");
		order.assign(step_order, step_order + nwords);
	}
	TileMaskGuard guard(ctx->dense, &mask, &order);
	const int64_t ldp = ((n + 1 + DENSE_NB - 1) / DENSE_NB) * DENSE_NB;
	DevBuf<double> tmp;
	tmp.reserve((size_t)ldp * ldp);
	SPP_HIP_CHECK(hipMemsetAsync(tmp.p, 0, (size_t)ldp * ldp * sizeof(double), ctx->stream));
	SPP_HIP_CHECK(hipMemcpy2DAsync(tmp.p, ldp * sizeof(double), d_A, ld * sizeof(double), n * sizeof(double), n,
		hipMemcpyDeviceToDevice, ctx->stream));
	dense_set_padding(ctx, tmp.p, ldp, n);
	SPP_HIP_CHECK(hipMemcpyAsync(tmp.p + n * ldp, d_b, n * sizeof(double), hipMemcpyDeviceToDevice, ctx->stream));
	int ret = dense_potrf_upper(ctx, tmp.p, n, ldp, true);
	if(ret == SPP_OK) {
		dense_potrs_upper(ctx, tmp.p, n, ldp, tmp.p + n * ldp);
		SPP_HIP_CHECK(hipMemcpyAsync(d_b, tmp.p + n * ldp, n * sizeof(double), hipMemcpyDeviceToDevice, ctx->stream));
		SPP_HIP_CHECK(hipMemcpy2DAsync(d_A, ld * sizeof(double), tmp.p, ldp * sizeof(double), n * sizeof(double), n,
			hipMemcpyDeviceToDevice, ctx->stream));
	}
	SPP_HIP_CHECK(hipStreamSynchronize(ctx->stream));
	dense_chain_check(ctx);
	return ret;
	SPP_CATCH(ctx)
}

int spp_dense_posv_masked(spp_ctx *ctx, double *d_A, int64_t n, int64_t ld, double *d_b, const uint64_t *words, int64_t nwords)
{
	return dense_posv_entry(ctx, d_A, n, ld, d_b, words, nwords, nullptr);
}

int spp_dense_posv_ordered(spp_ctx *ctx, double *d_A, int64_t n, int64_t ld, double *d_b, const uint64_t *words, int64_t nwords,
	const int32_t *step_order)
{
	if(!step_order || nwords <= 0)
		return SPP_E_BADARG;
	return dense_posv_entry(ctx, d_A, n, ld, d_b, words, nwords, step_order);
}

int spp_dense_gemm_tn_sub(spp_ctx *ctx, int64_t m, int64_t n, int64_t k, const double *d_A, int64_t lda,
	const double *d_B, int64_t ldb, double *d_C, int64_t ldc)
{
	if(!ctx || !d_A || !d_B || !d_C)
		return SPP_E_BADARG;
	SPP_TRY(ctx)
	drop_kept_factors(ctx);
	SPP_REQUIRE((lda % 2) == 0 && (ldb % 2) == 0, SPP_E_BADARG, "gemm_tn_sub: lda/ldb must be even (16-byte loads)");
	SPP_HIP_CHECK(hipSetDevice(ctx->device));
	dense_gemm_tn_sub(ctx, m, n, k, d_A, lda, d_B, ldb, d_C, ldc, false);
	SPP_HIP_CHECK(hipStreamSynchronize(ctx->stream));
	return SPP_OK;
	SPP_CATCH(ctx)
}

int spp_dense_gemm_tn_sub_upper(spp_ctx *ctx, int64_t m, int64_t n, int64_t k, const double *d_A, int64_t lda,
	const double *d_B, int64_t ldb, double *d_C, int64_t ldc)
{
	if(!ctx || !d_A || !d_B || !d_C)
		return SPP_E_BADARG;
	SPP_TRY(ctx)
	drop_kept_factors(ctx);
	SPP_REQUIRE((lda % 2) == 0 && (ldb % 2) == 0, SPP_E_BADARG, "gemm_tn_sub: lda/ldb must be even (16-byte loads)");
	SPP_HIP_CHECK(hipSetDevice(ctx->device));
	dense_gemm_tn_sub(ctx, m, n, k, d_A, lda, d_B, ldb, d_C, ldc, true);
	SPP_HIP_CHECK(hipStreamSynchronize(ctx->stream));
	return SPP_OK;
	SPP_CATCH(ctx)
}

int spp_dense_front_factor(spp_ctx *ctx, double *d_F, int64_t ld, int64_t w, int64_t h, double *d_image)
{
	if(!ctx || !d_F)
		return SPP_E_BADARG;
	SPP_TRY(ctx)
	drop_kept_factors(ctx);
	SPP_HIP_CHECK(hipSetDevice(ctx->device));
	return dense_front_factor(ctx, d_F, ld, w, h, d_image);
	SPP_CATCH(ctx)
}

}
```

### slam_plus_plus_amd/csrc/spp_dense.hip

```cpp

#include "spp_internal.h"
#include "spp_tiles.h"
#include "spp_dense_dev.h"
#include <stdio.h>
#include <stdlib.h>
#include <string.h>
#include <algorithm>
#include <vector>
#include <mutex>

namespace spp {


constexpr int BK = 16;
constexpr int LDS_STRIDE = 18;

template <int BM, int BN, int WM, int WN, int MODE, int DEPTH, int BKT, int SC1 = 0>
__device__ __forceinline__ void gemm_tn_tile(const int64_t m0, const int64_t n0, int64_t M, int64_t N, int K,
	const double *__restrict__ A, int64_t lda, const double *B, int64_t ldb, double *C, int64_t ldc, double *gemm_lds)
{
	constexpr int NWM = BM / WM, NWN = BN / WN, NT = NWM * NWN * 64;
	constexpr int TA = WM / 16, TB = WN / 16;
	constexpr int PPC = BKT / 2, LSTR = BKT + 2;
	constexpr int PA = (BM * PPC) / NT, PB = (BN * PPC) / NT;
// ... 1082 lines not shown
			init[8 * nsteps + 8 + 4 * k] = (long long)((~0ull) >> 1);
		SPP_HIP_CHECK(hipMemcpyAsync(dw.la_trace.p, init.data(), nw * sizeof(long long), hipMemcpyHostToDevice, s));
		SPP_HIP_CHECK(hipStreamSynchronize(s));
		a.trace = dw.la_trace.p;
	}
	SPP_HIP_CHECK(hipMemsetAsync(a.cnt, 0, nints * sizeof(int), s));
	SPP_HIP_CHECK(hipEventRecord(dw.ev[0], s));
	SPP_HIP_CHECK(hipStreamWaitEvent(sc, dw.ev[0], 0));
	SPP_HIP_CHECK(hipStreamWaitEvent(sb, dw.ev[0], 0));
	hipLaunchKernelGGL(la_chain_kernel, dim3((unsigned)(1 + LA_G1 + a.g2)), dim3(LA_THREADS), LA_LDS_DOUBLES * sizeof(double), sc, a);
	const int64_t slots = sw.la_slots > 0 ? sw.la_slots : 512;
	for(int k = 0; k < a.nsteps; ++ k) {
		const int64_t c1 = (int64_t)NB * (k + 1);
		if(c1 >= ncols || rows - c1 <= 0)
			break;
		const int nr = (int)((rows - c1 + NB - 1) / NB), nc = (int)((ncols - c1 + NB - 1) / NB);
		const int npri = (nc > 2) ? (nc - 2) + std::min(2, nr - 1) : 0;
		const int64_t ntr = nr - 1, ntc = nc - 1;
		const int64_t T = ntr > 0 ? ntr * (ntr + 1) / 2 + (ntc - ntr) * ntr : 0;
		const int64_t n128 = (T / slots) * slots;
		const int64_t grid = 4 * (int64_t)npri + n128 + 4 * (T - n128);
		if(grid > 0)
			hipLaunchKernelGGL(la_bulk_kernel, dim3((unsigned)grid), dim3(1024), LA_BULK_LDS_DOUBLES * sizeof(double), sb,
				a, k, nr, nc, npri, n128);
	}
	SPP_HIP_CHECK(hipEventRecord(dw.ev[1], sb));
	SPP_HIP_CHECK(hipEventRecord(dw.ev_chain, sc));
	SPP_HIP_CHECK(hipStreamWaitEvent(s, dw.ev[1], 0));
	SPP_HIP_CHECK(hipStreamWaitEvent(s, dw.ev_chain, 0));
	SPP_HIP_CHECK(hipGetLastError());
	if(tracing) {
		std::vector<long long> h((size_t)12 * nsteps + 16);
		SPP_HIP_CHECK(hipMemcpyAsync(h.data(), dw.la_trace.p, h.size() * sizeof(long long), hipMemcpyDeviceToHost, s));
		SPP_HIP_CHECK(hipStreamSynchronize(s));
		fprintf(stderr, "[spp] lookahead factorization, %d steps: potrf start / duration / gap to the next start (us)\n", a.nsteps);
		for(int k = 0; k < a.nsteps; ++ k)
			fprintf(stderr, "  k %2d  start %8.1f  potrf %5.1f  publish %4.1f | b1 seen +%4.1f  done +%4.1f | c1 seen +%4.1f  done +%4.1f | step %5.1f\n", k,
				(h[8 * k] - h[0]) * 0.01, (h[8 * k + 2] - h[8 * k]) * 0.01, (h[8 * k + 1] - h[8 * k + 2]) * 0.01,
				(h[8 * k + 3] - h[8 * k + 1]) * 0.01, (h[8 * k + 4] - h[8 * k + 1]) * 0.01, (h[8 * k + 5] - h[8 * k + 1]) * 0.01,
				(h[8 * k + 6] - h[8 * k + 1]) * 0.01, k + 1 < a.nsteps ? (h[8 * (k + 1)] - h[8 * k]) * 0.01 : 0.0);
		fprintf(stderr, "[spp] per step: panel (rest) done / bulk launch: first tile starts, priority tiles done, last tile done, busy workgroup-us (all relative to potrf(0) start)\n");
		for(int k = 0; k < a.nsteps; ++ k) {
			const long long *b = h.data() + 8 * nsteps + 8 + 4 * k;
			fprintf(stderr, "  k %2d  panel done %8.1f | bulk start %8.1f  pri done %8.1f  end %8.1f  busy %9.1f\n", k, h[8 * k + 7] ? (h[8 * k + 7] - h[0]) * 0.01 : 0.0,
				b[1] ? (b[0] - h[0]) * 0.01 : 0.0, b[3] ? (b[3] - h[0]) * 0.01 : 0.0, b[1] ? (b[1] - h[0]) * 0.01 : 0.0, b[2] * 0.01);
		}
	}
}

void dense_factor_steps(spp_ctx *ctx, double *d_A, int64_t ld, int64_t n, int64_t rows, int64_t ncols,
	int64_t nsteps, bool has_rhs)
{
	ensure_dense_work(ctx, nsteps);
	ctx->dense.tail_rows_last = 0;
	ctx->dense.tail_masked_whole = false;
	const bool captured = capturing(ctx->stream);
	if(!captured && la_usable(ctx, nsteps)) {
		dense_factor_lookahead(ctx, d_A, ld, n, rows, ncols, nsteps, has_rhs);
		ctx->dense.tinv_half = 0;
		return;
	}
	ctx->dense.tinv_half = nsteps;
	const bool flags = !captured && nsteps >= 4 && flag_schedule_usable(ctx);
	dense_factor_steps_enqueue(ctx, d_A, ld, n, rows, ncols, nsteps, has_rhs, flags, !captured);
}

static void flag_signal(hipStream_t st, int *flag, int value)
{
	hipLaunchKernelGGL(flag_signal_kernel, dim3(1), dim3(64), 0, st, flag, value);
}

static FlagWait make_flag_wait(spp_ctx *ctx, const int *flag, int value, long long timeout_ticks = WAIT_TICKS_DEFAULT)
{
	return FlagWait{flag, value, {ctx->dense.info.p + 2, timeout_ticks}};
}

static void flag_wait(spp_ctx *ctx, hipStream_t st, const int *flag, int value, long long timeout_ticks)
{
	hipLaunchKernelGGL(flag_wait_kernel, dim3(1), dim3(64), 0, st, make_flag_wait(ctx, flag, value, timeout_ticks));
}

static bool streams_concurrent(spp_ctx *ctx, hipStream_t a, hipStream_t b, int slot)
{
	DenseWork &dw = ctx->dense;
	hipStream_t st[2] = {a, b};
	dw.sync.reserve(16);
	SPP_HIP_CHECK(hipMemsetAsync(dw.sync.p, 0, 16 * sizeof(int), ctx->stream));
	SPP_HIP_CHECK(hipStreamSynchronize(ctx->stream));
	for(int p = 0; p < 2; ++ p) {
		flag_wait(ctx, st[p], dw.sync.p + slot + p, 1, 20 * WAIT_TICKS_PER_MS);
		flag_signal(st[1 - p], dw.sync.p + slot + p, 1);
	}
	for(int i = 0; i < 2; ++ i)
		SPP_HIP_CHECK(hipStreamSynchronize(st[i]));
	int h_abort = 0;
	SPP_HIP_CHECK(hipMemcpy(&h_abort, dw.info.p + 2, sizeof(int), hipMemcpyDeviceToHost));
	if(h_abort) {
		SPP_HIP_CHECK(hipMemset(dw.info.p + 2, 0, sizeof(int)));
		return false;
	}
	return true;
}

static bool flag_schedule_usable(spp_ctx *ctx)
{
	if(!switches().dense_sched)
		return false;
	DenseWork &dw = ctx->dense;
	if(dw.sync_state == 0 || dw.sync_stream != ctx->stream) {
		if(capturing(ctx->stream))
			return false;
		dw.sync_state = streams_concurrent(ctx, ctx->stream, dw.aux, 0) ? 1 : -1;
		dw.sync_stream = ctx->stream;
	}
	return dw.sync_state == 1;
}

static bool dense_tail_applies(spp_ctx *ctx, int64_t rows, int64_t nsteps)
{
	return !ctx->dense.tail_disabled && nsteps * NB >= rows && !(ctx->dense.ident_from >= 0 && ctx->dense.ident_from < rows);
}

static bool launch_dense_tail(spp_ctx *ctx, double *d_A, int64_t ld, int64_t rows, int64_t ncols, int64_t nsteps, int64_t k, bool has_rhs)
{
	const Switches &sw = switches();
	DenseWork &dw = ctx->dense;
	const int64_t c1 = (k + 1) * NB;
	if(!dense_tail_applies(ctx, rows, nsteps))
		return false;
	hipStream_t s = ctx->stream;
	static uint64_t attr_seen = 0;
	if(first_on_this_device(attr_seen))
		SPP_HIP_CHECK(hipFuncSetAttribute((const void*)dense_tail_kernel, hipFuncAttributeMaxDynamicSharedMemorySize,
			TAIL_LDS_DOUBLES * (int)sizeof(double)));
	if(dw.tail_resident < 0) {
		int per_cu = 0;
		hipDeviceProp_t prop;
		if(hipOccupancyMaxActiveBlocksPerMultiprocessor(&per_cu, (const void*)dense_tail_kernel, POTRF_THREADS,
		   TAIL_LDS_DOUBLES * sizeof(double)) == hipSuccess && hipGetDeviceProperties(&prop, ctx->device) == hipSuccess)
			dw.tail_resident = std::max(per_cu, 0) * prop.multiProcessorCount;
		else {
			(void)hipGetLastError();
			dw.tail_resident = 0;
		}
	}
	TailPlan plan = tail_plan(dw.tile_mask, dw.step_order, nsteps, rows, ncols, k, dw.tail_resident, TailSwitches::of(sw), &dw.tail_plan);
	if(!plan.applies)
		return false;
	if(plan.table_fresh && !dw.tail_plan.table.empty())
		SPP_HIP_CHECK(hipStreamSynchronize(s));
	dw.tail_plan = std::move(plan);
	const TailPlan &p = dw.tail_plan;
	const int Tr = p.key.Tr, Tc = p.key.Tc, ntile = (int)p.table.size();
	if(dw.tail_pub.cap < (size_t)Tr * Tc) {
		dw.tail_pub.reserve(std::max<size_t>((size_t)Tr * Tc, 24 * 25));
		SPP_HIP_CHECK(hipMemsetAsync(dw.tail_pub.p, 0, dw.tail_pub.cap * sizeof(int), s));
		dw.tail_epoch = 0;
	}
	if(dw.tail_dinv.cap < (size_t)Tr * 8 * 256)
		dw.tail_dinv.reserve(std::max<size_t>((size_t)Tr * 8 * 256, (size_t)24 * 8 * 256));
	if(++ dw.tail_epoch >= (1 << 26)) {
		SPP_HIP_CHECK(hipMemsetAsync(dw.tail_pub.p, 0, dw.tail_pub.cap * sizeof(int), s));
		dw.tail_epoch = 1;
	}
	if(p.table_fresh) {
		if(sw.verbose)
			fprintf(stderr, "[spp] streamed tail: %d x %d tiles, %d listed, %d resident; %d tiles of rows %d.. seated first (whole rows resident %d, live demand %d)\n",
				Tr, Tc, ntile, p.resident, p.info[0], p.info[1], p.info[2], p.info[3]);
		dw.tail_order.upload(p.table, s);
	}
	if(sw.verbose && p.ordered)
		fprintf(stderr, "[spp] streamed tail: %d steps in the caller's step order\n", Tr);
	TailArgs a;
	a.order = dw.tail_order.p;
	memset(a.rowbits, 0, sizeof(a.rowbits));
	std::copy(p.key.rowbits.begin(), p.key.rowbits.end(), a.rowbits);
	static_assert(sizeof(a.sorder) == sizeof(p.sorder), "one layout of the step list");
	memcpy(a.sorder, p.sorder, sizeof(a.sorder));
	a.A = d_A;
	a.ld = ld;
	a.rows = rows;
	a.ncols = ncols;
	a.c0 = c1;
	a.have_pre = p.key.have_pre ? 1 : 0;
	a.Tr = Tr;
	a.Tc = Tc;
	a.has_rhs = has_rhs ? 1 : 0;
	a.tinv = dw.tinv_all.p + (size_t)(k + 1) * NB * NB;
	a.dbuf = dw.tail_dinv.p;
	a.pub = dw.tail_pub.p;
	a.epoch = dw.tail_epoch;
	a.info = dw.info.p;
	a.bound = {dw.info.p + 2, sw.tail_timeout_ticks};
	static int launches = 0;
	DevBuf<long long> trace;
	a.trace = nullptr;
	if(sw.tail_trace && ++ launches == sw.tail_trace) {
		trace.reserve((size_t)Tr * 8);
		SPP_HIP_CHECK(hipMemsetAsync(trace.p, 0, (size_t)Tr * 8 * sizeof(long long), s));
		a.trace = trace.p;
	}
	dom_begin(ctx);
	hipLaunchKernelGGL(dense_tail_kernel, dim3((unsigned)ntile), dim3(POTRF_THREADS), TAIL_LDS_DOUBLES * sizeof(double), s, a);
	{
		const double m = (double)(rows - c1);
		dom_end(ctx, m * m * m / 3.0 + (a.have_pre ? (double)NB * m * (m + 1.0) : 0.0) + 2.0 * m * m);
	}
	dw.tail_rows_last = Tr;
	dw.tail_masked_whole = p.masked && !p.key.have_pre;
	SPP_HIP_CHECK(hipGetLastError());
	if(a.trace) {
		std::vector<long long> h((size_t)Tr * 8);
		SPP_HIP_CHECK(hipStreamSynchronize(s));
		SPP_HIP_CHECK(hipMemcpy(h.data(), trace.p, h.size() * sizeof(long long), hipMemcpyDeviceToHost));
		fprintf(stderr, "[spp] streamed tail, %d tile rows, %d of %d tiles launched (us from the launch's first stamp): diagonal tile: updates complete / factored+inverted | first panel tile: first row tile seen / last seen / last published\n", Tr, ntile, Tr * Tc - Tr * (Tr - 1) / 2);
		const long long t0 = h[0];
		for(int i = 0; i < Tr; ++ i)
			fprintf(stderr, "  row %2d  start %7.1f  updated %7.1f  done %7.1f | %7.1f %7.1f %7.1f\n", i, (h[8 * i] - t0) * 0.01, (h[8 * i + 1] - t0) * 0.01,
				(h[8 * i + 2] - t0) * 0.01, h[8 * i + 3] ? (h[8 * i + 3] - t0) * 0.01 : 0.0, h[8 * i + 4] ? (h[8 * i + 4] - t0) * 0.01 : 0.0, h[8 * i + 5] ? (h[8 * i + 5] - t0) * 0.01 : 0.0);
	}
	return true;
}

class StepHandOffs {
	spp_ctx *ctx;
	DenseWork &dw;
	const hipStream_t s, s2;
	const hipEvent_t evA, evB;
	const bool use_flags;
	int ep = 0;
	int64_t panel = -1, bulk = -1;
	int64_t held_panel = -1;
	int64_t held_bulk = -1;
	int64_t chain_owes = -1;

	int *panel_flag(int64_t k) const { return dw.sync.p + 2 * k; }
	int *bulk_flag(int64_t k) const { return dw.sync.p + 2 * k + 1; }
	void send_held_bulk()
	{
		if(held_bulk >= 0)
			flag_signal(s2, bulk_flag(held_bulk), ep);
		held_bulk = -1;
	}

public:
	StepHandOffs(spp_ctx *c, int64_t nsteps, bool flags) : ctx(c), dw(c->dense), s(c->stream), s2(c->dense.aux), evA(c->dense.ev[0]),
		evB(c->dense.ev[1]), use_flags(flags)
	{
		if(!use_flags)
			return;
		if(dw.sync.cap < (size_t)(2 * nsteps + 16)) {
			dw.sync.reserve((size_t)(2 * nsteps + 16));
			SPP_HIP_CHECK(hipMemsetAsync(dw.sync.p, 0, dw.sync.cap * sizeof(int), s));
			dw.sync_epoch = 1;
		}
		ep = ++ dw.sync_epoch;
		SPP_HIP_CHECK(hipEventRecord(evA, s));
		SPP_HIP_CHECK(hipStreamWaitEvent(s2, evA, 0));
	}
	void panel_complete(int64_t k)
	{
		panel = k;
		if(use_flags)
			held_panel = k;
		else
			SPP_HIP_CHECK(hipEventRecord(evA, s));
	}
	void bulk_takes_panel()
	{
		if(use_flags && held_bulk >= 0) {
			hipLaunchKernelGGL(flag_signal_wait_kernel, dim3(1), dim3(64), 0, s2, bulk_flag(held_bulk), ep, make_flag_wait(ctx, panel_flag(panel), ep));
			held_bulk = -1;
		} else if(use_flags)
			flag_wait(ctx, s2, panel_flag(panel), ep);
		else
			SPP_HIP_CHECK(hipStreamWaitEvent(s2, evA, 0));
	}
	void bulk_complete(int64_t k)
	{
		bulk = k;
		if(use_flags)
			held_bulk = k;
		else
			SPP_HIP_CHECK(hipEventRecord(evB, s2));
	}
	void chain_waits_now()
	{
		if(!use_flags) {
			SPP_HIP_CHECK(hipStreamWaitEvent(s, evB, 0));
			return;
		}
		if(held_bulk == bulk)
			send_held_bulk();
		if(held_panel >= 0)
			flag_signal(s, panel_flag(held_panel), ep);
		held_panel = -1;
		flag_wait(ctx, s, bulk_flag(bulk), ep);
	}
	void chain_waits_before_tile_row()
	{
		if(use_flags)
			chain_owes = bulk;
		else
			SPP_HIP_CHECK(hipStreamWaitEvent(s, evB, 0));
	}
	void flush()
	{
		if(chain_owes >= 0 && held_bulk == chain_owes)
			send_held_bulk();
		if(chain_owes >= 0 && held_panel >= 0)
			hipLaunchKernelGGL(flag_signal_wait_kernel, dim3(1), dim3(64), 0, s, panel_flag(held_panel), ep, make_flag_wait(ctx, bulk_flag(chain_owes), ep));
		else if(chain_owes >= 0)
			flag_wait(ctx, s, bulk_flag(chain_owes), ep);
		else if(held_panel >= 0)
			flag_signal(s, panel_flag(held_panel), ep);
		chain_owes = held_panel = -1;
	}
	void join()
	{
		held_bulk = -1;
		if(use_flags)
			SPP_HIP_CHECK(hipEventRecord(evB, s2));
		SPP_HIP_CHECK(hipStreamWaitEvent(s, evB, 0));
	}
};

static void dense_factor_steps_enqueue(spp_ctx *ctx, double *d_A, int64_t ld, int64_t n, int64_t rows, int64_t ncols,
	int64_t nsteps, bool has_rhs, bool use_flags, bool allow_fused)
{
	hipStream_t s = ctx->stream, s2 = ctx->dense.aux;
	DenseWork &dw = ctx->dense;
	const int64_t n_id = (dw.ident_from >= 0 && dw.ident_from < n) ? dw.ident_from : n;
	StepHandOffs hand(ctx, nsteps, use_flags);
	bool bulk_pending = false;
	const int fused = allow_fused ? switches().fused : 0;
	if(fused) {
		static uint64_t fattr_seen = 0;
		if(first_on_this_device(fattr_seen)) {
			SPP_HIP_CHECK(hipFuncSetAttribute((const void*)update_potrf_kernel, hipFuncAttributeMaxDynamicSharedMemorySize,
				POTRF_LDS_DOUBLES * (int)sizeof(double)));
		}
		if(dw.fuse_cnt.cap < (size_t)(nsteps + 2) || dw.fuse_dirty) {
			dw.fuse_cnt.reserve(std::max<size_t>((size_t)(nsteps + 2), 64));
			SPP_HIP_CHECK(hipMemsetAsync(dw.fuse_cnt.p, 0, dw.fuse_cnt.cap * sizeof(int), s));
			dw.fuse_expect.assign(dw.fuse_cnt.cap, 0);
			dw.fuse_dirty = false;
		}
	}
	static_assert(POTRF_LDS_DOUBLES >= (64 + 64) * FS_STRIDE, "the fused kernel's LDS is sized by the factorization");
	auto fused_update_potrf = [&](int64_t r0, int64_t m, int64_t kp0, int64_t kn) {
		const int64_t N = ncols - r0;
		if(m <= 0 || N <= 0)
			return false;
		const int64_t md = std::min<int64_t>(NB, m), nd = std::min<int64_t>(NB, N);
		const int ti = (int)((md + 31) / 32), tj = (int)((nd + 31) / 32);
		int nA = 0;
		for(int j = 0; j < tj; ++ j)
			nA += std::min(j, ti - 1) + 1;
		const int64_t nbi = (m + 63) / 64, nbj = (N + 63) / 64;
		const int do_potrf = kn >= 0 ? 1 : 0;
		const int64_t kn0 = (kn >= 0 ? kn : 0) * NB;
		const int n_valid = (int)std::max<int64_t>(0, std::min<int64_t>(NB, n_id - kn0));
		const size_t slot = (size_t)(kn >= 0 ? kn : nsteps + 1);
		dw.fuse_expect[slot] += nA;
		hipLaunchKernelGGL(update_potrf_kernel, dim3((unsigned)(nA + do_potrf + nbi * nbj)), dim3(POTRF_THREADS),
			POTRF_LDS_DOUBLES * sizeof(double), s, m, N, d_A + kp0 + r0 * ld, ld, d_A + r0 + r0 * ld, nA, dw.fuse_expect[slot], do_potrf,
			n_valid, (has_rhs && n_valid < NB) ? 1 : 0, dw.tinv_all.p + (size_t)(kn >= 0 ? kn : 0) * NB * NB, dw.info.p, kn0,
			dw.fuse_cnt.p + slot, WaitBound{dw.info.p + 2, WAIT_TICKS_DEFAULT});
		return true;
	};
	auto potrf_and_panel = [&](int64_t k, bool potrf_done = false) {
		const int64_t k0 = k * NB;
		const int n_valid = (int)std::max<int64_t>(0, std::min<int64_t>(NB, n_id - k0));
		double *tinv = ctx->dense.tinv_all.p + (size_t)k * NB * NB;
		if(!potrf_done)
			hipLaunchKernelGGL(potrf_diag_kernel, dim3(1), dim3(POTRF_THREADS), POTRF_LDS_DOUBLES * sizeof(double), s,
				d_A + k0 + k0 * ld, ld, n_valid, (has_rhs && n_valid < NB) ? 1 : 0, tinv, ctx->dense.info.p, k0);
		const int64_t c1 = k0 + NB;
		if(c1 < ncols)
			launch_panel_solve(s, ncols - c1, tinv, d_A + k0 + c1 * ld, ld);
	};
	auto tile_row = [&](int64_t r0, int64_t kp0) {
		const int64_t m = std::min<int64_t>(NB, rows - r0);
		if(m <= 0 || r0 >= ncols)
			return;
		const double *P = d_A + kp0 + r0 * ld;
		hand.flush();
		launch_gemm_staged<32, 32, 16, 16, 0>(s, m, ncols - r0, NB, P, ld, P, ld, d_A + r0 + r0 * ld, ld, true);
	};
	if(allow_fused && nsteps >= 2 && switches().tail_rows * NB >= rows && dense_tail_applies(ctx, rows, nsteps) &&
		launch_dense_tail(ctx, d_A, ld, rows, ncols, nsteps, -1, has_rhs)) {
		dw.tinv_half = 0;
		SPP_HIP_CHECK(hipGetLastError());
		return;
	}
	potrf_and_panel(0);
	const int64_t single_below = 2560, single_mixed_above = 1280;
	for(int64_t k = 0; k < nsteps; ++ k) {
		const int64_t k0 = k * NB, c1 = k0 + NB, c2 = c1 + NB;
		if(c1 >= ncols || rows - c1 <= 0)
			break;
		if(rows - c1 <= single_below || (allow_fused && switches().tail_rows * NB >= rows - c1 && dense_tail_applies(ctx, rows, nsteps))) {
			if(bulk_pending) {
				hand.chain_waits_now();
				bulk_pending = false;
			}
			const double *P = d_A + k0 + c1 * ld;
			if(allow_fused && launch_dense_tail(ctx, d_A, ld, rows, ncols, nsteps, k, has_rhs)) {
				dw.tinv_half = k + 1;
				break;
			}
			if(fused && k + 1 < nsteps && rows - c1 >= NB) {
				fused_update_potrf(c1, rows - c1, k0, k + 1);
				potrf_and_panel(k + 1, true);
				continue;
			}
			if(rows - c1 >= single_mixed_above) {
				dom_begin(ctx);
				const bool big = dense_gemm_tn_sub(ctx, rows - c1, ncols - c1, NB, P, ld, P, ld, d_A + c1 + c1 * ld, ld, true);
				const double mr = (double)(rows - c1);
				if(big)
					dom_end(ctx, 2.0 * NB * (0.5 * mr * (mr + 1.0) + mr * (double)(ncols - rows)));
			} else
				launch_gemm_staged<32, 32, 16, 16, 0>(s, rows - c1, ncols - c1, NB, P, ld, P, ld, d_A + c1 + c1 * ld, ld, true);
			if(k + 1 < nsteps)
				potrf_and_panel(k + 1);
			continue;
		}
		hand.panel_complete(k);
		if(bulk_pending) {
			hand.chain_waits_before_tile_row();
			bulk_pending = false;
		}
		const bool have_bulk = rows - c2 > 0 && c2 < ncols;
		bool fused_done = false;
		if(have_bulk) {
			hand.bulk_takes_panel();
			const double *P = d_A + k0 + c2 * ld;
			hipStream_t keep = ctx->stream;
			ctx->stream = s2;
			dom_begin(ctx);
			const bool big = dense_gemm_tn_sub(ctx, rows - c2, ncols - c2, NB, P, ld, P, ld, d_A + c2 + c2 * ld, ld, true);
			const double mr = (double)(rows - c2);
			if(big)
				dom_end(ctx, 2.0 * NB * (0.5 * mr * (mr + 1.0) + mr * (double)(ncols - rows)));
			ctx->stream = keep;
			hand.bulk_complete(k);
			bulk_pending = true;
		}
		if(fused && k + 1 < nsteps && rows - c1 >= NB) {
			hand.flush();
			fused_update_potrf(c1, NB, k0, k + 1);
			fused_done = true;
		} else
			tile_row(c1, k0);
		hand.flush();
		if(k + 1 < nsteps)
			potrf_and_panel(k + 1, fused_done);
	}
	if(bulk_pending)
		hand.join();
	SPP_HIP_CHECK(hipGetLastError());
}

void dense_reserve(spp_ctx *ctx, int64_t nblk)
{
	ensure_dense_work(ctx, nblk);
}

void dense_info_ensure(spp_ctx *ctx)
{
	ensure_info(ctx);
}

void dense_info_reset_on(spp_ctx *ctx, hipStream_t st)
{
	hipLaunchKernelGGL(set_info_kernel, dim3(1), dim3(1), 0, st, ctx->dense.info.p);
}

void dense_info_reset(spp_ctx *ctx)
{
	ensure_info(ctx);
	dense_info_reset_on(ctx, ctx->stream);
}

void dense_chain_check(spp_ctx *ctx)
{
	if(ctx->dense.h_chain_err && *ctx->dense.h_chain_err) {
		*ctx->dense.h_chain_err = 0;
		ctx->dense.chain_disabled = true;
		throw Error(SPP_E_HIP, "backward substitution: a workgroup of the chain kernel timed out waiting for its predecessor; "
			"the following calls launch per block row");
	}
}

int dense_info_fetch(spp_ctx *ctx, bool *dag_aborted)
{
	int h_info[4] = {0, 0, 0, 0};
	dense_info_copy_on(ctx, ctx->stream, h_info);
	SPP_HIP_CHECK(hipStreamSynchronize(ctx->stream));
	return dense_info_eval(ctx, h_info, dag_aborted);
}

void dense_info_copy_on(spp_ctx *ctx, hipStream_t st, int *h_status4)
{
	SPP_HIP_CHECK(hipMemcpyAsync(h_status4, ctx->dense.info.p, 4 * sizeof(int), hipMemcpyDeviceToHost, st));
}

int dense_info_eval(spp_ctx *ctx, const int *h_status4, bool *dag_aborted, bool drain_first)
{
	const int h_info[4] = {h_status4[0], h_status4[1], h_status4[2], h_status4[3]};
	if(drain_first && (h_info[0] | h_info[2] | h_info[3]))
		SPP_HIP_CHECK(hipStreamSynchronize(ctx->stream));
	if(h_info[3]) {
		SPP_HIP_CHECK(hipMemset(ctx->dense.info.p + 3, 0, sizeof(int)));
		sparse_dag_disable(ctx);
		if(dag_aborted) {
			*dag_aborted = true;
			return 0;
		}
		throw Error(SPP_E_HIP, "sparse factorization: a front timed out waiting for another front's flag; "
			"the following calls launch level by level");
	}
	if(h_info[2] && h_info[0]) {
		SPP_HIP_CHECK(hipMemset(ctx->dense.info.p + 2, 0, sizeof(int)));
		return h_info[0];
	}
	if(h_info[2] == TAIL_ABORT_TIMEOUT) {
		SPP_HIP_CHECK(hipMemset(ctx->dense.info.p + 2, 0, sizeof(int)));
		ctx->dense.tail_disabled = true;
		ctx->dense.fuse_dirty = true;
		throw Error(SPP_E_HIP, "dense factorization: the streamed launch (spp_dense_tail.h) timed out waiting for a tile; "
			"the following calls use the per-step schedule");
	}
	if(h_info[2]) {
		SPP_HIP_CHECK(hipMemset(ctx->dense.info.p + 2, 0, sizeof(int)));
		ctx->dense.sync_state = -1;
		ctx->dense.fuse_dirty = true;
		throw Error(SPP_E_HIP, "dense factorization: a cross-stream flag wait timed out (streams not concurrent?); "
			"the following calls use the event schedule");
	}
	return h_info[0];
}

bool dense_potrf_upper_enqueue(spp_ctx *ctx, double *d_A, int64_t n, int64_t ld, bool info_reset)
{
	SPP_REQUIRE(ld % NB == 0 && n < ld, SPP_E_BADARG, "dense_potrf_upper: ld must be a multiple of 128 and > n");
	if(info_reset)
		dense_info_reset(ctx);
	dense_factor_steps(ctx, d_A, ld, n, n, n + 1, (n + NB - 1) / NB, true);
	return ctx->dense.tail_masked_whole;
}

int dense_potrf_upper(spp_ctx *ctx, double *d_A, int64_t n, int64_t ld, bool )
{
	SPP_REQUIRE(ld % NB == 0 && n < ld, SPP_E_BADARG, "dense_potrf_upper: ld must be a multiple of 128 and > n");
	dense_info_reset(ctx);
	dense_factor_steps(ctx, d_A, ld, n, n, n + 1, (n + NB - 1) / NB, true);
	return dense_info_fetch(ctx) ? SPP_NOT_POSDEF : SPP_OK;
}

__global__ __launch_bounds__(256)
void front_image_kernel(double *F, int64_t ld, double *P, int64_t ldp, int w, int pad, int h, int to_image)
{
	const int c = (int)blockIdx.x, hp = h + pad;
	const bool cpad = c >= w && c < w + pad;
	const int cu = c < w ? c : c - pad;
	for(int r = threadIdx.x; r < hp; r += 256) {
		const bool rpad = r >= w && r < w + pad;
		const int ru = r < w ? r : r - pad;
		if(to_image)
			P[r + (int64_t)c * ldp] = (cpad || rpad) ? (r == c ? 1.0 : 0.0) : (r <= c ? F[ru + (int64_t)cu * ld] : 0.0);
		else if(!cpad && !rpad)
			F[ru + (int64_t)cu * ld] = P[r + (int64_t)c * ldp];
	}
}

int dense_front_factor(spp_ctx *ctx, double *d_F, int64_t ld, int64_t w, int64_t h, double *d_image)
{
	SPP_REQUIRE(w > 0 && h >= w && ld >= h && h < (1 << 20), SPP_E_BADARG, "front factor: need 0 < w <= h <= ld");
	hipStream_t s = ctx->stream;
	const int64_t pad = ((w + NB - 1) / NB) * NB - w, hp = h + pad, ldp = (hp + 1) & ~int64_t(1);
	const size_t img = (size_t)ldp * hp, band = (size_t)ldp * NB;
	DevBuf<double> P;
	P.reserve(img + band);
	SPP_HIP_CHECK(hipMemsetAsync(P.p + img, 0xff, band * sizeof(double), s));
	hipLaunchKernelGGL(front_image_kernel, dim3((unsigned)hp), dim3(256), 0, s, d_F, ld, P.p, ldp, (int)w, (int)pad, (int)h, 1);
	dense_info_reset(ctx);
	{
		struct IdentGuard {
			DenseWork &d;
			IdentGuard(DenseWork &dw, int64_t from) : d(dw) { d.ident_from = from; }
			~IdentGuard() { d.ident_from = -1; }
		} guard(ctx->dense, w);
		dense_factor_steps(ctx, P.p, ldp, w + pad, hp, hp, (w + pad) / NB, false);
	}
	const int info = dense_info_fetch(ctx);
	hipLaunchKernelGGL(front_image_kernel, dim3((unsigned)hp), dim3(256), 0, s, d_F, ld, P.p, ldp, (int)w, (int)pad, (int)h, 0);
	if(d_image)
		SPP_HIP_CHECK(hipMemcpyAsync(d_image, P.p, (size_t)hp * ldp * sizeof(double), hipMemcpyDeviceToDevice, s));
	std::vector<unsigned long long> hb(band);
	SPP_HIP_CHECK(hipMemcpyAsync(hb.data(), P.p + img, band * sizeof(double), hipMemcpyDeviceToHost, s));
	SPP_HIP_CHECK(hipStreamSynchronize(s));
	for(size_t q = 0; q < band; ++ q)
		SPP_REQUIRE(hb[q] == ~0ull, SPP_E_HIP, "front factor: a write past the end of the front's image");
	return info ? SPP_NOT_POSDEF : SPP_OK;
}

static void chain_err_ensure(DenseWork &dw)
{
	if(dw.h_chain_err)
		return;
	SPP_HIP_CHECK(hipHostMalloc((void**)&dw.h_chain_err, sizeof(int), hipHostMallocMapped | hipHostMallocCoherent));
	*dw.h_chain_err = 0;
	SPP_HIP_CHECK(hipHostGetDevicePointer((void**)&dw.d_chain_err, dw.h_chain_err, 0));
}

void dense_potrs_upper(spp_ctx *ctx, const double *d_R, int64_t n, int64_t ld, double *d_b)
{
	const int64_t nblk = (n + NB - 1) / NB;
	hipStream_t s = ctx->stream;
	if(ctx->dense.tinv_half > 0) {
		hipLaunchKernelGGL(tinv_finish_kernel, dim3((unsigned)ctx->dense.tinv_half), dim3(1024), 0, s, ctx->dense.tinv_all.p);
		ctx->dense.tinv_half = 0;
	}
	const int use_chain = (capturing(s) || ctx->dense.chain_disabled) ? 0 : switches().trsv_chain;
	ensure_info(ctx);
	const WaitBound bound{ctx->dense.info.p + 1, switches().chain_timeout_ticks};
	if(use_chain == 2 && nblk > 1 && nblk <= 4096) {
		DenseWork &dw = ctx->dense;
		const size_t need = (size_t)nblk * NB * 4;
		if(dw.trsv_pay.cap < need) {
			dw.trsv_pay.reserve(need);
			SPP_HIP_CHECK(hipMemsetAsync(dw.trsv_pay.p, 0, dw.trsv_pay.cap * sizeof(double), s));
		}
		chain_err_ensure(dw);
		++ dw.epoch;
		const unsigned long long K = (2ull * (unsigned long long)dw.epoch + 1ull) * 0x9E3779B97F4A7C15ull;
		TrsvPay *xpay = (TrsvPay*)dw.trsv_pay.p, *wpay = xpay + (size_t)nblk * NB;
		if(switches().trsv_mform) {
			if(dw.trsv_m.cap < (size_t)nblk * NB * NB)
				dw.trsv_m.reserve((size_t)nblk * NB * NB);
			static uint64_t attr_seen = 0;
			if(first_on_this_device(attr_seen))
				SPP_HIP_CHECK(hipFuncSetAttribute((const void*)trsv_m_kernel, hipFuncAttributeMaxDynamicSharedMemorySize, TRSVM_LDS_DOUBLES * (int)sizeof(double)));
			hipLaunchKernelGGL(trsv_m_kernel, dim3((unsigned)nblk - 1, 8), dim3(1024), TRSVM_LDS_DOUBLES * sizeof(double), s, d_R, ld, n, dw.tinv_all.p, dw.trsv_m.p);
			hipLaunchKernelGGL((trsv_back_chain2_kernel<8, true>), dim3((unsigned)nblk + 1), dim3(512), 0, s,
				d_R, ld, n, (int)nblk, dw.tinv_all.p, dw.trsv_m.p, d_b, xpay, wpay, K, bound, dw.d_chain_err);
		} else
			hipLaunchKernelGGL((trsv_back_chain2_kernel<8, false>), dim3((unsigned)nblk + 1), dim3(512), 0, s,
				d_R, ld, n, (int)nblk, dw.tinv_all.p, (const double*)nullptr, d_b, xpay, wpay, K, bound, dw.d_chain_err);
		SPP_HIP_CHECK(hipGetLastError());
		return;
	}
	if(use_chain && nblk > 1 && nblk <= 1024) {
		DenseWork &dw = ctx->dense;
		if(dw.flags.cap < (size_t)nblk) {
			dw.flags.reserve((size_t)nblk);
			SPP_HIP_CHECK(hipMemsetAsync(dw.flags.p, 0, (size_t)nblk * sizeof(int), s));
			dw.epoch = 0;
		}
		chain_err_ensure(dw);
		++ dw.epoch;
		hipLaunchKernelGGL(trsv_back_chain_kernel, dim3((unsigned)nblk), dim3(256), 0, s, d_R, ld, n, (int)nblk,
// ... 176 lines not shown
```

### slam_plus_plus_amd/csrc/spp_dense_tail.h

```cpp
#pragma once
#include "spp_dense_dev.h"

namespace spp {

struct TailArgs {
	double *A;
	int64_t ld;
	int64_t rows;
	int64_t ncols;
	int64_t c0;
	int have_pre;
	int Tr, Tc;
	int has_rhs;
	double *tinv;
	double *dbuf;
	int *pub;
	int epoch;
	int *info;
	WaitBound bound;
	long long *trace;
	const int *order;
	unsigned long long rowbits[TAIL_MAX_ROWS + 1];
	unsigned long long sorder[TAIL_MAX_ROWS / 8 + 1];
};

constexpr int TAIL_ABORT_TIMEOUT = 2;

constexpr int TAIL_LDS_DOUBLES = POTRF_LDS_DOUBLES_INV2 + 16;

#ifndef SPP_TAIL_PLAIN_LD
#define SPP_TAIL_PLAIN_LD 0
#endif
__device__ __forceinline__ double tail_ld(const double *p)
{
#if SPP_TAIL_PLAIN_LD
	return __hip_atomic_load(p, __ATOMIC_RELAXED, __HIP_MEMORY_SCOPE_WORKGROUP);
#else
	return __hip_atomic_load(p, __ATOMIC_RELAXED, __HIP_MEMORY_SCOPE_AGENT);
#endif
}

__device__ __noinline__ void tail_first_tile(double *sm, const v4f64 t00, const int lane, int *info, const int64_t k0)
{
	const int l15 = lane & 15, l4 = lane >> 4;
#pragma unroll
	for(int r = 0; r < 4; ++ r)
		sm[(l4 + 4 * r) + l15 * TS] = t00[r];
	if(lane == 0)
		potrf_lds2_fail(sm)[0] = 0;
	__builtin_amdgcn_fence(__ATOMIC_ACQ_REL, "wavefront");
	__builtin_amdgcn_wave_barrier();
	diag_tile_factor<TS>(sm, potrf_lds2_dv(sm), potrf_lds2_gd0(sm), potrf_lds2_dinv(sm), 0, lane, potrf_lds2_fail(sm), info, k0);
}

__global__ __launch_bounds__(POTRF_THREADS)
void dense_tail_kernel(const TailArgs a)
{
	extern __shared__ double sm[];
	const int tid = threadIdx.x, lane = tid & 63, wave = __builtin_amdgcn_readfirstlane(tid >> 6);
	const int l15 = lane & 15, l4 = lane >> 4;
	int *st = (int*)(sm + POTRF_LDS_DOUBLES_INV2);
	const int ord = a.order[blockIdx.x];
	const int ti = ord >> 16, tj = ord & 0xffff;
	const bool diag = ti == tj;
	const int64_t i0 = a.c0 + (int64_t)NB * ti, j0 = a.c0 + (int64_t)NB * tj;
	const int tag = a.epoch << 4;
	auto stamp = [&](int slot) { if(a.trace && tid == 0) a.trace[ti * 8 + slot] = wall_clock64(); };
	if(diag) stamp(0);
	auto pub_count = [&](const int v, const int w) -> int {
		const int cv = ((v >> 4) == a.epoch) ? (v & 15) : 0, cw = ((w >> 4) == a.epoch) ? (w & 15) : 0;
		return cv < cw ? cv : cw;
	};
	auto wait_pub = [&](const int *p, const int *q, const int need) -> int {
		if(tid == 0) {
			int c = 0;
			const bool ok = bounded_wait<1, 1>(a.bound, TAIL_ABORT_TIMEOUT, [&]() {
				const int v = wait_ld(p);
				c = pub_count(v, q ? wait_ld(q) : v);
				return c >= need;
			});
			st[1] = ok ? c : -1;
		}
		lds_barrier();
		const int got = st[1];
		lds_barrier();
		return got;
	};
	int ra[4], cb[4];
#pragma unroll
	for(int u = 0; u < 4; ++ u) {
		if(!diag) {
			ra[u] = wave & 7;
			cb[u] = 4 * (wave >> 3) + u;
		} else {
			int q = (wave == 0) ? (u == 0 ? 0 : 36) : wave + 15 * u, c = 0;
			if(q >= 36)
				ra[u] = cb[u] = -1;
			else {
				while(q > c) {
					q -= c + 1;
					++ c;
				}
				ra[u] = q;
				cb[u] = c;
			}
		}
	}
	v4f64 acc[4];
	{
		double *img = sm;
#pragma unroll 4
		for(int q = 0; q < NB * NB / POTRF_THREADS; ++ q) {
			const int e = tid + q * POTRF_THREADS, r = e & (NB - 1), c = e >> 7;
			const int64_t row = i0 + r, col = j0 + c;
			img[r + c * TS] = (col < a.ncols) ? a.A[row + col * a.ld] : ((diag && row == col) ? 1.0 : 0.0);
		}
		lds_barrier();
#pragma unroll
		for(int u = 0; u < 4; ++ u)
#pragma unroll
			for(int r = 0; r < 4; ++ r)
				acc[u][r] = (ra[u] < 0) ? 0.0 : img[(16 * ra[u] + l4 + 4 * r) + (16 * cb[u] + l15) * TS];
		lds_barrier();
	}
	bool pre_first = false;
	{
		const int ek = tid & 15, ec = tid >> 4;
		constexpr int PS = 18;
		const int ekp = 4 * (ek & 3) + (ek >> 2);
		unsigned long long ksteps = 0;
		for(int k = a.have_pre ? -1 : 0; k < ti; ++ k) {
			const unsigned long long w = a.rowbits[k + 1];
			ksteps |= ((w >> ti) & (w >> tj) & 1) << (k + 1);
		}
		unsigned long long steps = 0;
		for(int q = 0; 8 * q < a.Tr + a.have_pre; ++ q) {
			const unsigned long long word = a.sorder[q];
#pragma unroll
			for(int b = 0; b < 8; ++ b) {
				const int k = (int)(signed char)(unsigned char)(word >> (8 * b));
				if(k < ti && ((ksteps >> (k + 1)) & 1) != 0)
					steps |= 1ull << (8 * q + b);
			}
		}
		const int nst = 8 * __builtin_popcountll(steps);
		double va[2], vb[2];
		auto fetch = [&](const int k, const int J) {
			const double *rowp = a.A + (a.c0 + (int64_t)NB * k) + 16 * J + ek;
#pragma unroll
			for(int h = 0; h < 2; ++ h) {
				const int64_t ca = i0 + ec + 64 * h, cb = j0 + ec + 64 * h;
				va[h] = (ca < (diag ? a.ncols : a.rows)) ? tail_ld(rowp + ca * a.ld) : 0.0;
				vb[h] = (!diag && cb < a.ncols) ? tail_ld(rowp + cb * a.ld) : 0.0;
			}
		};
		int avail = a.have_pre ? 8 : 0;
		pre_first = diag && nst > 0 && (nst & 1) == 0 && a.rows - i0 >= 16;
		bool inflight = false;
		int k = a.have_pre ? -1 : 0;
		int knext = steps ? tail_sorder_at(a.sorder, __builtin_ctzll(steps)) : k;
		for(int sidx = 0; sidx < nst; ++ sidx) {
			const int J = sidx & 7;
			if(J == 0) {
				k = knext;
				steps &= steps - 1;
				if(steps)
					knext = tail_sorder_at(a.sorder, __builtin_ctzll(steps));
			}
			if(J == 0 && k >= 0)
				avail = 0;
			if(!inflight) {
				if(J >= avail) {
					avail = wait_pub(a.pub + k * a.Tc + ti, a.pub + k * a.Tc + tj, J + 1);
					if(avail < 0)
						return;
				}
				fetch(k, J);
			}
			int pk = -1;
			if(tid == 0 && k >= 0 && J + 1 < 8 && J + 1 >= avail)
				pk = pub_count(__hip_atomic_load(a.pub + k * a.Tc + ti, __ATOMIC_RELAXED, __HIP_MEMORY_SCOPE_AGENT),
					__hip_atomic_load(a.pub + k * a.Tc + tj, __ATOMIC_RELAXED, __HIP_MEMORY_SCOPE_AGENT));
			double *sa = sm + (sidx & 1) * 2 * NB * PS, *sb = diag ? sa : sa + NB * PS;
#pragma unroll
			for(int h = 0; h < 2; ++ h) {
				sa[ekp + (ec + 64 * h) * PS] = va[h];
				if(!diag)
					sb[ekp + (ec + 64 * h) * PS] = vb[h];
			}
			if(tid == 0)
				st[2 + (sidx & 1)] = pk;
			lds_barrier();
			{
				const int seen = st[2 + (sidx & 1)];
				if(seen > avail)
					avail = seen;
			}
			inflight = (sidx + 1 < nst) && (J + 1 < 8) && (J + 1 < avail);
			if(inflight)
				fetch(k, J + 1);
			double fa[4];
#pragma unroll
			for(int u = 0; u < 4; ++ u) {
				if(ra[u] < 0)
					continue;
				double fb[4];
				if(u == 0 || diag) {
					const bool row_live = i0 + 16 * ra[u] + l15 < a.rows;
					const double2 a01 = *(const double2*)(sa + 4 * l4 + (16 * ra[u] + l15) * PS), a23 = *(const double2*)(sa + 4 * l4 + 2 + (16 * ra[u] + l15) * PS);
					fa[0] = row_live ? -a01.x : 0.0;
					fa[1] = row_live ? -a01.y : 0.0;
					fa[2] = row_live ? -a23.x : 0.0;
					fa[3] = row_live ? -a23.y : 0.0;
				}
				{
					const double2 b01 = *(const double2*)(sb + 4 * l4 + (16 * cb[u] + l15) * PS), b23 = *(const double2*)(sb + 4 * l4 + 2 + (16 * cb[u] + l15) * PS);
					fb[0] = b01.x;
					fb[1] = b01.y;
					fb[2] = b23.x;
					fb[3] = b23.y;
				}
#pragma unroll
				for(int kk = 0; kk < 4; ++ kk)
					acc[u] = __builtin_amdgcn_mfma_f64_16x16x4f64(fa[kk], fb[kk], acc[u], 0, 0, 0);
				if(u == 0 && pre_first && sidx == nst - 1 && wave == 0) {
					tail_first_tile(sm, acc[0], lane, a.info, i0);
				}
			}
		}
		lds_barrier();
	}
	if(diag) stamp(1);
	double *T = sm;
#pragma unroll
	for(int u = 0; u < 4; ++ u)
#pragma unroll
		for(int r = 0; r < 4; ++ r)
			if(ra[u] >= 0 && !(pre_first && wave == 0 && u == 0))
				T[(16 * ra[u] + l4 + 4 * r) + (16 * cb[u] + l15) * TS] = acc[u][r];
	lds_barrier();
	if(diag) {
		const int64_t nv = a.rows - i0;
		const int n_valid = (int)(nv < 0 ? 0 : (nv > NB ? NB : nv));
		PotrfPub pb;
		pb.flag = a.pub + ti * a.Tc + ti;
		pb.base = tag;
		pb.dbuf = a.dbuf + (size_t)ti * 8 * 256;
		pb.abort = a.bound.abort;
		potrf_diag_body<false, 1, 2, true>(a.A + i0 + i0 * a.ld, a.ld, n_valid, (a.has_rhs && n_valid < NB) ? 1 : 0,
			a.tinv + (size_t)ti * NB * NB, a.info, i0, sm, pb, pre_first ? 1 : 0);
		stamp(2);
		return;
	}
	double *Dv = T + NB * TS;
	double *Rr = Dv + 16 * PT;
	const double *Rii = a.A + i0 + i0 * a.ld;
	int avail = 0;
	bool inflight = false;
	double dvr = 0, rr[2] = {0, 0};
	auto fetch_panel = [&](const int J) {
		if(tid < 256)
			dvr = tail_ld(a.dbuf + ((size_t)ti * 8 + J) * 256 + tid);
#pragma unroll
		for(int h = 0; h < 2; ++ h) {
			const int e = tid + POTRF_THREADS * h, k = e & 15, c = e >> 4;
			if(e < 16 * (NB - 16 * (J + 1)))
				rr[h] = tail_ld(Rii + (16 * J + k) + (int64_t)(16 * (J + 1) + c) * a.ld);
		}
	};
	for(int J = 0; J < 8; ++ J) {
		if(!inflight) {
			if(J >= avail) {
				avail = wait_pub(a.pub + ti * a.Tc + ti, nullptr, J + 1);
				if(avail < 0)
					return;
			}
			fetch_panel(J);
		}
		if(tj == ti + 1 && J == 0) stamp(3);
		if(tj == ti + 1 && J == 7) stamp(4);
		int pk = -1;
		if(tid == 0 && J + 1 < 8 && J + 1 >= avail) {
			const int v = __hip_atomic_load(a.pub + ti * a.Tc + ti, __ATOMIC_RELAXED, __HIP_MEMORY_SCOPE_AGENT);
			pk = pub_count(v, v);
		}
		if(tid < 256)
			Dv[(tid & 15) + (tid >> 4) * PT] = dvr;
#pragma unroll
		for(int h = 0; h < 2; ++ h) {
			const int e = tid + POTRF_THREADS * h;
			if(e < 16 * (NB - 16 * (J + 1)))
				Rr[(e & 15) + (e >> 4) * PT] = rr[h];
		}
		if(tid == 0)
			st[2 + (J & 1)] = pk;
		lds_barrier();
		{
			const int seen = st[2 + (J & 1)];
			if(seen > avail)
				avail = seen;
		}
		inflight = (J + 1 < 8) && (J + 1 < avail);
		if(inflight)
			fetch_panel(J + 1);
		if(wave < 8) {
			double *Y = T + 16 * J + (16 * wave) * TS;
			const v4f64 x = tile_atb(Dv, 1, PT, Y, 1, TS, lane);
			__builtin_amdgcn_fence(__ATOMIC_ACQ_REL, "wavefront");
			__builtin_amdgcn_wave_barrier();
			const int64_t col = j0 + 16 * wave + l15;
#pragma unroll
			for(int r = 0; r < 4; ++ r) {
				Y[(l4 + 4 * r) + l15 * TS] = x[r];
				if(col < a.ncols)
					__hip_atomic_store(&a.A[(i0 + 16 * J + l4 + 4 * r) + col * a.ld], x[r], __ATOMIC_RELAXED, __HIP_MEMORY_SCOPE_AGENT);
			}
		}
		lds_barrier();
		{
			const int b = wave & 7;
			double xb[4];
#pragma unroll
			for(int kk = 0; kk < 4; ++ kk)
				xb[kk] = T[16 * J + (4 * kk + l4) + (16 * b + l15) * TS];
			auto row_update = [&](const int I) {
				const double *Ra = Rr + 16 * (I - J - 1) * PT;
				v4f64 d = (v4f64){0, 0, 0, 0};
#pragma unroll
				for(int kk = 0; kk < 4; ++ kk)
					d = __builtin_amdgcn_mfma_f64_16x16x4f64(Ra[(4 * kk + l4) + l15 * PT], xb[kk], d, 0, 0, 0);
				double *D = T + 16 * I + (16 * b) * TS;
#pragma unroll
				for(int r = 0; r < 4; ++ r)
					D[(l4 + 4 * r) + l15 * TS] -= d[r];
			};
			{
				const int I = J + 1 + (wave >> 3);
				if(I < 8)
					row_update(I);
			}
			if(wave < 8)
				asm volatile("s_waitcnt vmcnt(0)" ::: "memory");
			lds_barrier();
			if(tid == 0)
				__hip_atomic_store(a.pub + ti * a.Tc + tj, tag | (J + 1), __ATOMIC_RELAXED, __HIP_MEMORY_SCOPE_AGENT);
			for(int I = J + 3 + (wave >> 3); I < 8; I += 2)
				row_update(I);
			lds_barrier();
		}
		if(tj == ti + 1 && J == 7) stamp(5);
	}
}

}
```

### slam_plus_plus_amd/csrc/spp_internal.h

```cpp
#pragma once

#include <hip/hip_runtime.h>
#include <stdint.h>
#include <string>
#include <vector>
#include <sys/mman.h>
#include <utility>
#include <functional>
#include <new>
#include <exception>
#include <thread>
#include <stdexcept>
#include <algorithm>
#include <string.h>
#include <chrono>
#include <stdio.h>
#include <stdlib.h>
#include "../../include/spp_hip.h"
#include "spp_switches.h"

namespace spp {

struct Error : std::runtime_error {
	int code;
// ... 113 lines not shown
	struct Item { void **pp; size_t *pcap; bool *powned; size_t off, n; };
	std::vector<Item> items;
	explicit UploadArena(hipStream_t s) : stream(s) { host.reserve(size_t(1) << 20); }
	template <class T, class A>
	void add(DevBuf<T> &b, const std::vector<T, A> &v)
	{
		if(v.size() * sizeof(T) > (size_t(256) << 10)) {
			b.upload(v, stream);
			return;
		}
		b.release();
		const size_t off = (host.size() + 255) & ~(size_t)255, bytes = std::max<size_t>(v.size(), 1) * sizeof(T);
		host.resize(off + bytes);
		if(!v.empty())
			memcpy(host.data() + off, v.data(), v.size() * sizeof(T));
		Item it = {(void**)&b.p, &b.cap, &b.owned, off, std::max<size_t>(v.size(), 1)};
		items.push_back(it);
	}
	void commit(DevBuf<unsigned char> &store)
	{
		store.release();
		store.reserve(std::max<size_t>(host.size(), 256));
		if(!host.empty())
			SPP_HIP_CHECK(hipMemcpyAsync(store.p, host.data(), host.size(), hipMemcpyHostToDevice, stream));
		for(size_t i = 0; i < items.size(); ++ i) {
			*items[i].pp = store.p + items[i].off;
			*items[i].pcap = items[i].n;
			*items[i].powned = false;
		}
	}
};

struct Structure {
	int64_t nb = 0, n = 0, nnzb = 0, nvals = 0;
	HVec<int64_t> col_ptr, row_idx, blk_off, base;
	HVec<int32_t> dim;
};

struct SaccItem {
	int32_t beg, end;
	int32_t kind;
	int32_t a_tr;
	int64_t dst;
	int64_t aoff;
};

struct SchurDims {
	int dp = 0, dl = 0;
	int64_t nc = 0, nl = 0;
	int64_t nl_total = 0;
	int64_t no = 0;
	int64_t n_red = 0, ld = 0;
	int64_t n_sblk = 0;
	int64_t n_pairs = 0;
	int64_t n_items = 0, n_multi = 0;
	int32_t xcd_max_items = 0;
	bool u_landmark_major = true;
	bool factored = true;
};

struct SchurPlan : SchurDims {
	bool add_A = true;
	bool sparse_S = false;
	bool mis = false;
	Structure s_st;
	DevBuf<int64_t> sblk_voff;
	std::vector<int64_t> pose_block;
	std::vector<int64_t> lm_block;
	std::vector<uint8_t> is_lm;
	std::vector<uint64_t> tile_mask;
	std::vector<int32_t> step_order;
	DevBuf<int32_t> lm_ptr;
	DevBuf<int32_t> bs_ptr;
	int64_t n_bs = 0;
	int lm_stream_last = 0;
	DevBuf<int64_t> lm_coff;
	DevBuf<int64_t> lm_rbase;
	DevBuf<int32_t> obs_pose;
	DevBuf<int32_t> obs_lm;
	DevBuf<int64_t> obs_off;
	DevBuf<int64_t> pose_rbase;
	DevBuf<int32_t> cam_ptr;
	DevBuf<int32_t> cam_obs;
	DevBuf<int32_t> obs_wpos;
	DevBuf<SaccItem> items;
	DevBuf<int32_t> xcd_beg;
	DevBuf<int32_t> sblk_i1, sblk_i2;
	DevBuf<int64_t> sblk_aoff;
	DevBuf<int32_t> pair_a, pair_b;
	DevBuf<int32_t> multi_blk;
	DevBuf<int32_t> multi_ptr;
	DevBuf<double> cinv;
	DevBuf<double> lfac;
	DevBuf<double> W;
	DevBuf<double> Up;
	DevBuf<double> xw;
	DevBuf<double> partial;
	DevBuf<double> S;
	bool unlisted_dirty = true;
	bool side_pending = false, side_padded = false;
	int side_last = 0, clear_last = 0;
	bool factor_kept = false;
	DevBuf<double> sigma_Z;
	DevBuf<int64_t> sigma_cc;
	std::vector<int64_t> sigma_cc_host;
	int64_t sigma_ncc = -1;
	bool sparse_factor_kept = false;
	DevBuf<double> sigma_Zb;
	DevBuf<int64_t> sigma_scol, sigma_srow;
	int async_last = 0;
	void release_all();
};

constexpr int TAIL_MAX_ROWS = 64;
constexpr int TAIL_NO_STEP = 127;
constexpr int TAIL_SORDER_WORDS = TAIL_MAX_ROWS / 8 + 1;

__host__ __device__ inline int tail_sorder_at(const unsigned long long *sorder, const int p)
{
	return (int)(signed char)(unsigned char)(sorder[p >> 3] >> (8 * (p & 7)));
}

inline void tail_sorder_pack(unsigned long long *sorder, const int *list, const int n)
{
	for(int p = 0; p < 8 * TAIL_SORDER_WORDS; ++ p) {
		if(!(p & 7))
			sorder[p >> 3] = 0;
		sorder[p >> 3] |= (unsigned long long)(unsigned char)(signed char)(p < n ? list[p] : TAIL_NO_STEP) << (8 * (p & 7));
	}
}

struct TailSwitches {
	int tail_rows, tail_mask, tail_early, tail_early_lead;
	double tail_order_beta;
	static TailSwitches of(const Switches &sw) { return TailSwitches{sw.tail_rows, sw.tail_mask, sw.tail_early, sw.tail_early_lead, sw.tail_order_beta}; }
};

struct TailPlan {
	bool applies = false;
	struct Key {
		int Tr = 0, Tc = 0;
		bool have_pre = false;
		bool early = false;
		bool lead = false;
		std::vector<uint64_t> rowbits;
		bool operator ==(const Key &o) const
		{
			return Tr == o.Tr && Tc == o.Tc && have_pre == o.have_pre && early == o.early && lead == o.lead && rowbits == o.rowbits;
		}
	} key;
	bool masked = false;
	bool ordered = false;
	unsigned long long sorder[TAIL_SORDER_WORDS];
	int resident = 0;
	bool table_fresh = false;
	std::vector<int> table;
	int info[5] = {0, 0, 0, 0, 0};
};

struct DenseWork {
	DevBuf<double> tinv;
	DevBuf<int> info;
	DevBuf<double> tinv_all;
	int64_t tinv_half = 0;
	DevBuf<double> xtmp;
	DevBuf<int> flags;
	DevBuf<int> tail_pub;
	DevBuf<double> tail_dinv;
	int tail_epoch = 0;
	DevBuf<int> tail_order;
	TailPlan tail_plan;
	int tail_resident = -1;
	const std::vector<uint64_t> *tile_mask = nullptr;
	const std::vector<int32_t> *step_order = nullptr;
	bool tail_masked_whole = false;
	int tail_rows_last = 0;
	bool tail_disabled = false;
	DevBuf<double> trsv_m;
	DevBuf<double> trsv_pay;
	DevBuf<double> trsm_w;
	uint64_t epoch = 0;
	int *h_chain_err = nullptr;
	int *d_chain_err = nullptr;
	bool chain_disabled = false;
	hipStream_t aux = nullptr;
	hipEvent_t ev[2] = {nullptr, nullptr};
	DevBuf<int> sync;
	DevBuf<int> fuse_cnt;
	std::vector<int> fuse_expect;
	bool fuse_dirty = false;
	int64_t ident_from = -1;
	hipStream_t chain = nullptr;
	hipEvent_t ev_chain = nullptr;
	DevBuf<int> la_cnt;
	DevBuf<long long> la_trace;
	int la_state = 0;
	int la_reserve = 0;
	int la_ncu = 0;
	int sync_epoch = 0;
	int sync_state = 0;
	hipStream_t sync_stream = nullptr;
};

struct SparsePlan;

struct AssemblePlan;

struct PhaseTimer {
	hipEvent_t ev[2 * SPP_N_PHASES];
	bool used[SPP_N_PHASES];
	bool created = false;
};

}

struct spp_ctx {
	int device = 0;
	int flags = 0;
	hipStream_t stream = nullptr;
	bool own_stream = false;
	hipStream_t side_stream = nullptr;
	hipEvent_t side_ev[2] = {nullptr, nullptr};
	hipEvent_t status_ev[2] = {nullptr, nullptr};
	int *h_status = nullptr;
	bool status_pending = false;
	std::string last_error;
	int mode = -1;
	int shard_rank = 0, shard_world = 1;
	spp::Structure st;
	std::vector<int64_t> order;
	std::thread plan_trash;
	spp::SchurPlan schur;
	spp::DenseWork dense;
	spp::SparsePlan *sparse = nullptr;
	spp::AssemblePlan *assemble = nullptr;
	spp::DevBuf<double> d_vals, d_rhs;
	double *h_staging = nullptr;
	size_t h_staging_cap = 0;
	spp::DevBuf<double> again_panel, again_cols;
	spp::DevBuf<int64_t> again_rows;
	std::vector<int64_t> again_rows_host;
	bool sparse_factor_kept = false;
	spp::DevBuf<double> geom_partial;
	spp::PhaseTimer timer;
	double phase_ms[SPP_N_PHASES] = {0};
	std::vector<hipEvent_t> dom_events;
	size_t dom_used = 0;
	double dom_flops = 0;
	int64_t factor_flops = 0, solve_bytes = 0, factor_nnz = 0;
};

namespace spp {

void se2_linearize(spp_ctx *ctx, int64_t ne, const int32_t *d_v0, const int32_t *d_v1, const double *d_poses,
	const double *d_meas, double *d_J0, double *d_J1, double *d_r);
double se2_update(spp_ctx *ctx, int64_t nv, double *d_poses, const double *d_dx, bool apply);
void se2_linearize_at(spp_ctx *ctx, int64_t ne, const int64_t *d_off0, const int64_t *d_off1, const double *d_state,
	const double *d_meas, double *d_J0, double *d_J1, double *d_r);
void se2_rb_linearize(spp_ctx *ctx, int64_t ne, const int64_t *d_off0, const int64_t *d_off1, const double *d_state,
	const double *d_meas, double *d_J0, double *d_J1, double *d_r);
double slam2d_update(spp_ctx *ctx, int64_t n, double *d_state, const double *d_dx, int64_t n_angles,
	const int64_t *d_angle_off, bool apply);
void se3_linearize_at(spp_ctx *ctx, int64_t ne, const int64_t *d_off0, const int64_t *d_off1, const double *d_state,
	const double *d_meas, double *d_J0, double *d_J1, double *d_r);
void se3_xyz_linearize(spp_ctx *ctx, int64_t ne, const int64_t *d_pose_off, const int64_t *d_lm_off, const double *d_state,
	const double *d_meas, double *d_J0, double *d_J1, double *d_r);
double slam3d_update(spp_ctx *ctx, int64_t n, double *d_state, const double *d_dx, int64_t n_poses,
	const int64_t *d_pose_off, bool apply);
void rocv_range_linearize(spp_ctx *ctx, int64_t ne, const int64_t *d_recv_off, const int64_t *d_lm_off, const double *d_state,
	const double *d_meas, double *d_J0, double *d_J1, double *d_r);
void rocv_cv_linearize(spp_ctx *ctx, int64_t ne, const int64_t *d_off0, const int64_t *d_off1, const double *d_state,
	const double *d_dt, double *d_J0, double *d_J1, double *d_r);
double edge_chi2(spp_ctx *ctx, int64_t ne, int rd, const double *d_r, const double *d_Om);
void edge_robust_weights(spp_ctx *ctx, int64_t ne, int rd, int kind, double scale, double param, const double *d_r, double *d_w);
double edge_hessian_maxdiag(spp_ctx *ctx, int64_t ne, int rd, int d0, int d1, const double *d_J0, const double *d_J1,
	const double *d_Om);
double lm_gain_denominator(spp_ctx *ctx, int64_t n, const double *d_dx, const double *d_rhs, double alpha);
void se3_linearize(spp_ctx *ctx, int64_t ne, const int32_t *d_v0, const int32_t *d_v1, const double *d_poses,
	const double *d_meas, double *d_J0, double *d_J1, double *d_r);
double se3_update(spp_ctx *ctx, int64_t nv, double *d_poses, const double *d_dx, bool apply);
void ba_linearize(spp_ctx *ctx, int64_t no, const int32_t *d_cam_of, const int32_t *d_pt_of, const double *d_cams,
	const double *d_intr, const double *d_pts, const double *d_meas, double *d_J0, double *d_J1, double *d_r);
void ba_stereo_linearize(spp_ctx *ctx, int64_t no, const int32_t *d_cam_of, const int32_t *d_pt_of, const double *d_cams,
	const double *d_intr, const double *d_pts, const double *d_meas, double *d_J0, double *d_J1, double *d_r);
void ba_intrinsics_linearize(spp_ctx *ctx, int64_t no, const int32_t *d_cam_of, const int32_t *d_pt_of, const int32_t *d_intr_of,
	const double *d_cams, const double *d_intr, const double *d_pts, const double *d_meas, double *d_J0, double *d_J1, double *d_J2,
	double *d_r);
double ba_intrinsics_update(spp_ctx *ctx, int64_t ni, double *d_intr, const int64_t *d_intr_dxoff, const double *d_dx, bool apply);
double ba_update(spp_ctx *ctx, int64_t nc, double *d_cams, const int64_t *d_cam_dxoff, int64_t np, double *d_pts,
	const int64_t *d_pt_dxoff, const double *d_dx, int64_t n_dx, bool apply);
void sim3_ba_linearize(spp_ctx *ctx, int64_t no, const int32_t *d_cam_of, const int32_t *d_pt_of, const double *d_cams,
	const double *d_intr, const double *d_pts, const double *d_meas, double *d_J0, double *d_J1, double *d_r);
double sim3_update(spp_ctx *ctx, int64_t nc, double *d_cams, const int64_t *d_cam_dxoff, int64_t np, double *d_pts,
	const int64_t *d_pt_dxoff, const double *d_dx, int64_t n_dx, bool apply);

void min_degree_order(int64_t nb, const int64_t *col_ptr, const int64_t *row_idx, std::vector<int64_t> &order);
void nested_dissection_order(int64_t nb, const int64_t *col_ptr, const int64_t *row_idx, std::vector<int64_t> &order);

void tile_mask_mark(int64_t n, int bs, int64_t nblk, const int32_t *i1, const int32_t *i2, std::vector<uint64_t> &words);
int64_t tile_mask_close(int64_t n, bool has_rhs, bool fill, std::vector<uint64_t> &words);
constexpr double TAIL_MODEL_STEP_US = 36.5, TAIL_MODEL_UPDATE_US = 2.0, TAIL_MODEL_START_US = 45.0;
constexpr int TAIL_MODEL_RESIDENT = 256;
struct TileDagCost {
	int64_t tiles = 0, updates = 0, path = 0;
	double cost_us = 0;
};
TileDagCost tile_dag_cost(int64_t n, const std::vector<uint64_t> &filled, int resident);
void tail_order_table(const std::vector<uint64_t> &bits, int Tr, int Tc, bool have_pre, double beta, int resident, bool early,
	std::vector<int> &order, int *info, bool lead = false);
TailPlan tail_plan(const std::vector<uint64_t> *mask, const std::vector<int32_t> *step_order, int64_t nsteps, int64_t rows,
	int64_t ncols, int64_t k, int resident, const TailSwitches &sw, TailPlan *former = nullptr);
bool is_permutation(const int32_t *v, int64_t n);
void tail_step_order(const std::vector<uint64_t> &filled, std::vector<int32_t> &order);

void build_schur_plan(spp_ctx *ctx, bool sparse_S, bool mis = false);
int64_t schur_buffer_doubles(const spp_ctx *ctx);
bool schur_applicable(const Structure &st, int *dp, int *dl);
double schur_plan_host_probe(const Structure &st, int shard_rank, int shard_world, bool sparse_S, bool mis, int64_t *out);
void schur_tile_mask_host_probe(const Structure &st, std::vector<uint64_t> &words);
bool schur_cam_order_host_probe(const Structure &st, int shard_rank, int shard_world, bool sparse_S, bool mis, const int64_t *order_in,
	std::vector<int32_t> &cam_order, TileDagCost cost[2]);
bool schur_step_order_host_probe(const Structure &st, int shard_rank, int shard_world, bool sparse_S, bool mis, std::vector<int32_t> &step_order);

void sparse_analyze(spp_ctx *ctx, const Structure &st);
int sparse_factor_solve(spp_ctx *ctx, const double *d_vals, double *d_rhs);
void sparse_release(spp_ctx *ctx);
void sparse_dag_disable(spp_ctx *ctx);
int64_t sparse_info(const spp_ctx *ctx, int what);
// ... 132 lines not shown
```

### slam_plus_plus_amd/csrc/spp_switches.h

```cpp
#pragma once

#include <stdint.h>
#include <stdlib.h>
#include <string.h>
#include <algorithm>

namespace spp {

constexpr long long WAIT_TICKS_PER_MS = 100000;
constexpr long long WAIT_TICKS_DEFAULT = 500 * WAIT_TICKS_PER_MS;

enum Ordering { ORDERING_AUTO, ORDERING_AMD, ORDERING_ND };
constexpr int MID_FRONT_MAX = 640;

struct Switches {
	bool verbose;
	int plan_threads;
	int64_t plan_min_work;

	int dense_sched;
	int fused;
	int aux_reserve_cus;
	int tile_444;
	int dense_la;
	int la_chain_mask;
	int la_g2;
	int la_bulk_acquire;
	int64_t la_slots;
	int la_trace;
	int tail_rows;
	int tail_mask;
	double tail_order_beta;
	int tail_early;
	int tail_step_order;
	int tail_early_lead;
	long long tail_timeout_ticks;
	int tail_trace;
	int trsv_chain;
	int trsv_mform;
	long long chain_timeout_ticks;
	int trsm_fused;

	bool sacc_ulm;
	bool sacc_factored;
	int64_t sacc_tile;
	int64_t sacc_tile_cols;
	int sacc_xcd;
	int sacc_chunk;
	int schur_cam_order;
	int backsubst_fused;
	int schur_side;
	int solve_async;
	int lm_stream;

	int mid_front_max;
	Ordering ordering;
	int64_t amalg_small;
	double amalg_zeros;
	int64_t amalg_relax_h;
	double amalg_zeros_small;
	bool sparse_teams;
	int sparse_team_max;
	int sparse_team_cols;
	int sparse_dag;
	int dag_split;
	long long dag_timeout_ticks;
	int dag_trace;
};

inline int env_int(const char *name, int dflt)
{
	const char *e = getenv(name);
	return e ? atoi(e) : dflt;
}

inline long long env_i64(const char *name, long long dflt)
{
	const char *e = getenv(name);
	return e ? atoll(e) : dflt;
}

inline double env_double(const char *name, double dflt)
{
	const char *e = getenv(name);
	return e ? atof(e) : dflt;
}

inline Switches parse_switches()
{
	Switches w;
	w.verbose = getenv("SPP_VERBOSE") != nullptr;
	const char *threads = getenv("SPP_PLAN_THREADS");
	w.plan_threads = threads ? std::max(1, atoi(threads)) : 0;
	w.plan_min_work = std::max<int64_t>(1, env_i64("SPP_PLAN_MIN_WORK", int64_t(1) << 18));

	w.dense_sched = env_int("SPP_DENSE_SCHED", 1);
	w.fused = env_int("SPP_FUSED", 1);
	w.aux_reserve_cus = env_int("SPP_AUX_RESERVE_CUS", 32);
	w.tile_444 = env_int("SPP_TILE_444", 0);
	w.dense_la = env_int("SPP_DENSE_LA", 0);
	w.la_chain_mask = env_int("SPP_LA_CHAIN_MASK", 1);
	w.la_g2 = env_int("SPP_LA_G2", 0);
	w.la_bulk_acquire = env_int("SPP_LA_BULK_ACQUIRE", 1);
	w.la_slots = env_i64("SPP_LA_SLOTS", 0);
	w.la_trace = env_int("SPP_LA_TRACE", 0);
	w.tail_rows = env_int("SPP_DENSE_TAIL", 1) ? env_int("SPP_TAIL_ROWS", 44) : 0;
	w.tail_mask = env_int("SPP_TAIL_MASK", 1);
	w.tail_order_beta = env_double("SPP_TAIL_ORDER_BETA", 0.0);
	w.tail_early = env_int("SPP_TAIL_EARLY", 1);
	w.tail_step_order = env_int("SPP_TAIL_STEP_ORDER", 1);
	w.tail_early_lead = env_int("SPP_TAIL_EARLY_LEAD", 1);
	w.tail_timeout_ticks = env_i64("SPP_TAIL_TIMEOUT_TICKS", WAIT_TICKS_DEFAULT);
	w.tail_trace = env_int("SPP_TAIL_TRACE", 0);
	w.trsv_chain = env_int("SPP_TRSV_CHAIN", 2);
	w.trsv_mform = env_int("SPP_TRSV_MFORM", 1);
	w.chain_timeout_ticks = env_i64("SPP_CHAIN_TIMEOUT_TICKS", WAIT_TICKS_DEFAULT);
	w.trsm_fused = env_int("SPP_TRSM_FUSED", 1);

	w.sacc_ulm = env_int("SPP_SACC_ULM", 1) != 0;
	w.sacc_factored = env_int("SPP_SACC_FACTORED", 1) != 0;
	w.sacc_tile = std::max<int64_t>(1, env_i64("SPP_SACC_TILE", 4));
	w.sacc_tile_cols = env_i64("SPP_SACC_TILE_COLS", -2);
	w.sacc_xcd = env_int("SPP_SACC_XCD", 1);
	w.sacc_chunk = env_int("SPP_SACC_CHUNK", 1);
	w.schur_cam_order = env_int("SPP_SCHUR_CAM_ORDER", 1);
	w.backsubst_fused = env_int("SPP_BACKSUBST_FUSED", 1);
	w.schur_side = env_int("SPP_SCHUR_SIDE", 1);
	w.solve_async = env_int("SPP_SOLVE_ASYNC", 1);
	w.lm_stream = env_int("SPP_LM_STREAM", 1);

	w.mid_front_max = std::max(128, std::min(MID_FRONT_MAX, env_int("SPP_MID_FRONT_MAX", 320)));
	const char *ordering = getenv("SPP_ORDERING");
	w.ordering = !ordering ? ORDERING_AUTO : (!strcmp(ordering, "nd") ? ORDERING_ND : ORDERING_AMD);
	w.amalg_small = env_i64("SPP_AMALG_SMALL", 32);
	w.amalg_zeros = env_double("SPP_AMALG_ZEROS", 0.12);
	w.amalg_relax_h = env_i64("SPP_AMALG_RELAX_H", 96);
	w.amalg_zeros_small = env_double("SPP_AMALG_ZEROS_SMALL", 0.2);
	w.sparse_teams = env_int("SPP_SPARSE_TEAMS", 1) != 0;
	w.sparse_team_max = std::max(1, std::min(64, env_int("SPP_SPARSE_TEAM_MAX", 40)));
	w.sparse_team_cols = std::max(8, std::min(256, env_int("SPP_SPARSE_TEAM_COLS", 16)));
	w.sparse_dag = env_int("SPP_SPARSE_DAG", 1);
	w.dag_split = env_int("SPP_DAG_SPLIT", 1);
	w.dag_timeout_ticks = env_i64("SPP_DAG_TIMEOUT_TICKS", WAIT_TICKS_DEFAULT);
	w.dag_trace = env_int("SPP_DAG_TRACE", 0);
	return w;
}

inline const Switches &switches()
{
	static const Switches w = parse_switches();
	return w;
}

}
```

### slam_plus_plus_amd/csrc/spp_tile_plan.cpp

```cpp

#include "spp_internal.h"
#include <algorithm>

namespace spp {

void tile_mask_mark(int64_t n, int bs, int64_t nblk, const int32_t *i1, const int32_t *i2, std::vector<uint64_t> &words)
{
	words.clear();
	const int64_t Tr = (n + DENSE_NB - 1) / DENSE_NB, Tc = n / DENSE_NB + 1;
	if(Tr < 1 || Tc > 64)
		return;
	words.assign((size_t)Tr, 0);
	for(int64_t q = 0; q < nblk; ++ q) {
		const int64_t a = std::min(i1[q], i2[q]), b = std::max(i1[q], i2[q]);
		const int64_t r0 = a * bs / DENSE_NB, r1 = std::min<int64_t>(a * bs + bs - 1, n - 1) / DENSE_NB;
		const int64_t c0 = b * bs / DENSE_NB, c1 = std::min<int64_t>(b * bs + bs - 1, n - 1) / DENSE_NB;
		if(a < 0 || r0 >= Tr || c0 >= Tr)
			continue;
		words[r0] |= (1ull << c0) | (1ull << c1);
		words[r1] |= (1ull << c0) | (1ull << c1);
	}
}

int64_t tile_mask_close(int64_t n, bool has_rhs, bool fill, std::vector<uint64_t> &words)
// ... 20 lines not shown
			const uint64_t f = r & ~((1ull << a) - 1);
			if(fill)
				words[a] |= f;
			updates += __builtin_popcountll(words[a] & f);
		}
	}
	return updates;
}

void tail_order_table(const std::vector<uint64_t> &bits, int Tr, int Tc, bool have_pre, double beta, int resident, bool early,
	std::vector<int> &order, int *info, bool lead)
{
	std::vector<std::pair<double, int> > key;
	for(int i = 0; i < Tr; ++ i)
		for(int j = i; j < Tc; ++ j)
			if((bits[(size_t)i + 1] >> j) & 1)
				key.push_back(std::make_pair((double)i + beta * (double)j, (i << 16) | j));
	std::stable_sort(key.begin(), key.end(), [](const std::pair<double, int> &x, const std::pair<double, int> &y) { return x.first < y.first; });
	order.resize(key.size());
	for(size_t q = 0; q < key.size(); ++ q)
		order[q] = key[q].second;
	int widest = 1;
	for(int i = 0; i < Tr; ++ i)
		widest = std::max(widest, (int)__builtin_popcountll(bits[(size_t)i + 1]));
	const int D = std::max(resident, 0) / widest;
	if(info) {
		info[0] = 0;
		info[1] = Tr;
		info[2] = D;
		info[3] = 0;
		info[4] = widest;
	}
	if(!early || resident <= 0)
		return;
	auto first_step = [&](const int i, const int j) -> int {
		for(int k = have_pre ? -1 : 0; k < i; ++ k) {
			const uint64_t w = bits[(size_t)k + 1];
			if((w >> i) & (w >> j) & 1)
				return k;
		}
		return i;
	};
	int r_star = Tr;
	for(int i = Tr - 1; i >= 0; -- i) {
		bool all_lag = true;
		for(int j = i; j < Tc && all_lag; ++ j)
			if((bits[(size_t)i + 1] >> j) & 1)
				all_lag = i - first_step(i, j) > D;
		if(!all_lag)
			break;
		r_star = i;
	}
	int n_early = 0;
	std::vector<int> live((size_t)Tr + 1, 0);
	for(size_t q = 0; q < order.size(); ++ q) {
		const int i = order[q] >> 16, j = order[q] & 0xffff;
		if(i >= r_star)
			++ n_early;
		else {
			++ live[(size_t)std::max(first_step(i, j), 0)];
			-- live[(size_t)i + 1];
		}
	}
	int demand = 0;
	for(int r = 0, run = 0; r < Tr; ++ r) {
		run += live[(size_t)r];
		demand = std::max(demand, run);
	}
	if(info)
		info[3] = demand;
	if(n_early == 0)
		return;
	if(n_early > resident / 2 || resident - n_early < demand) {
		if(!lead)
			return;
		const int room = std::min(resident / 2, resident - demand);
		int r2 = r_star - 1, n_lead = 0;
		for(int i = r_star; i < Tr; ++ i) {
			const int row = (int)__builtin_popcountll(bits[(size_t)i + 1] & ~((1ull << i) - 1) & (Tc == 64 ? ~0ull : (1ull << Tc) - 1));
			if(n_lead + row > room)
				break;
			n_lead += row;
			r2 = i;
		}
		if(n_lead == 0)
			return;
		std::vector<int> depth((size_t)Tr, 1);
		for(int k = 0; k < Tr; ++ k)
			for(int j = 0; j < k; ++ j)
				if((bits[(size_t)j + 1] >> k) & 1)
					depth[k] = std::max(depth[k], depth[j] + 1);
		auto key = [&](const int t) { const int i = t >> 16; return i < r_star ? 1 + depth[i] : (i <= r2 ? 0 : 2 + Tr); };
		std::stable_sort(order.begin(), order.end(), [&key](const int x, const int y) { return key(x) < key(y); });
		if(info) {
			info[0] = n_lead;
			info[1] = r_star;
		}
		return;
	}
	std::stable_partition(order.begin(), order.end(), [r_star](const int t) { return (t >> 16) >= r_star; });
	if(info) {
		info[0] = n_early;
		info[1] = r_star;
	}
}

bool is_permutation(const int32_t *v, int64_t n)
{
	std::vector<char> seen((size_t)n, 0);
	for(int64_t q = 0; q < n; ++ q) {
		if(v[q] < 0 || v[q] >= n || seen[(size_t)v[q]])
			return false;
		seen[(size_t)v[q]] = 1;
	}
	return true;
}

TailPlan tail_plan(const std::vector<uint64_t> *mask, const std::vector<int32_t> *step_order, int64_t nsteps, int64_t rows,
	int64_t ncols, int64_t k, int resident, const TailSwitches &sw, TailPlan *former)
{
	TailPlan p;
	const int64_t f = k + 1;
	const int64_t Tr = nsteps - f, Tc = (ncols - f * DENSE_NB + DENSE_NB - 1) / DENSE_NB;
	if(nsteps * DENSE_NB < rows || Tr < 1 || Tr > sw.tail_rows || Tc < Tr || Tc > Tr + 1 || Tc > TAIL_MAX_ROWS)
		return p;
	p.applies = true;
	TailPlan::Key &key = p.key;
	key.Tr = (int)Tr;
	key.Tc = (int)Tc;
	key.have_pre = f > 0;
	if(!sw.tail_mask || (mask && (int64_t)mask->size() != nsteps))
		mask = nullptr;
	p.masked = mask != nullptr;
	const uint64_t all_cols = Tc == 64 ? ~0ull : (1ull << Tc) - 1;
	key.rowbits.resize((size_t)Tr + 1);
	for(int64_t i = -1; i < Tr; ++ i) {
		uint64_t w = (mask && f + i >= 0) ? ((*mask)[(size_t)(f + i)] >> f) : all_cols;
		if(i >= 0)
			w = (w | (1ull << i)) & ~((1ull << i) - 1);
		key.rowbits[(size_t)i + 1] = w & all_cols;
	}
	p.ordered = f == 0 && step_order && (int64_t)step_order->size() == nsteps;
	bool ascending = true;
	int list[TAIL_MAX_ROWS + 1], n = 0;
	if(p.ordered)
		SPP_REQUIRE(is_permutation(step_order->data(), Tr), SPP_E_BADARG, "streamed tail: the step order is not a permutation of the tile rows");
	if(key.have_pre)
		list[n ++] = -1;
	for(int q = 0; q < (int)Tr; ++ q) {
		list[n ++] = p.ordered ? (*step_order)[(size_t)q] : q;
		ascending = ascending && list[n - 1] == q;
	}
	tail_sorder_pack(p.sorder, list, n);
	key.early = p.masked && sw.tail_early != 0;
	key.lead = key.early && !ascending && sw.tail_early_lead != 0;
	p.resident = key.early ? resident : 0;
	if(former && former->key == key) {
		p.table.swap(former->table);
		std::copy(former->info, former->info + 5, p.info);
		return p;
	}
	p.table_fresh = true;
	tail_order_table(key.rowbits, key.Tr, key.Tc, key.have_pre, sw.tail_order_beta, p.resident, key.early, p.table, p.info, key.lead);
	return p;
}

void tail_step_order(const std::vector<uint64_t> &filled, std::vector<int32_t> &order)
{
	const int Tr = (int)std::min<size_t>(filled.size(), 64);
	std::vector<int> depth((size_t)Tr, 1);
	for(int k = 0; k < Tr; ++ k)
		for(int j = 0; j < k; ++ j)
			if((filled[(size_t)j] >> k) & 1)
				depth[k] = std::max(depth[k], depth[j] + 1);
	order.resize((size_t)Tr);
	for(int k = 0; k < Tr; ++ k)
		order[k] = k;
	std::stable_sort(order.begin(), order.end(), [&depth](const int32_t x, const int32_t y) { return depth[x] < depth[y]; });
}

TileDagCost tile_dag_cost(int64_t n, const std::vector<uint64_t> &filled, int resident)
{
	TileDagCost c;
	const int64_t Tr = (int64_t)filled.size();
	std::vector<uint64_t> w(filled);
	c.updates = tile_mask_close(n, true, true, w);
	std::vector<int> depth((size_t)Tr, 1);
	for(int64_t k = 0; k < Tr; ++ k) {
		c.tiles += __builtin_popcountll(w[k]);
		for(int64_t j = 0; j < k; ++ j)
			if((w[j] >> k) & 1)
				depth[k] = std::max(depth[k], depth[j] + 1);
		c.path = std::max<int64_t>(c.path, depth[k]);
	}
	c.cost_us = std::max(c.path * TAIL_MODEL_STEP_US, c.updates * TAIL_MODEL_UPDATE_US / std::max(1, resident)) + TAIL_MODEL_START_US;
	return c;
}

}
```

Measured before the change: 1.327 billion block-nnz/s.

## Let diagonal tail tiles form their last step's final row tile themselves

In the streamed dense tail factorization, each diagonal tile's final update sub-step is now formed locally from a published Y_7 panel slice and the owning step's Dinv_7 block. It no longer waits for the full panel row tile to be published. The panel workgroup of that last step publishes Y_7 early (after J==6) plus a flag, and the host plan computes the last step index per tile row. This is meant to shorten the critical path across dependent diagonal tiles. The cost is extra buffers, another cross-workgroup flag protocol and more code complexity. A failed-pivot info query and a host helper to inspect klast are also added.

```diff
diff --git a/include/spp_hip.h b/include/spp_hip.h
--- a/include/spp_hip.h
+++ b/include/spp_hip.h
@@ -68,6 +68,7 @@
 #define SPP_INFO_SOLVE_ASYNC    23
 #define SPP_INFO_FACTOR_KEPT    24
 #define SPP_INFO_SPARSE_FACTOR_KEPT 25
+#define SPP_INFO_DENSE_FAILED_PIVOT 27
 #define SPP_INFO_SCHUR_SPARSE_FACTOR_KEPT 26
 int spp_get_info(const spp_ctx *ctx, int what, int64_t *out);
 int spp_get_ordering(const spp_ctx *ctx, int64_t *h_order);
@@ -229,6 +230,8 @@
 	int32_t *table, int32_t *info);
 int spp_tail_plan_host(int64_t n, int has_rhs, const uint64_t *words, int64_t nwords, const int32_t *step_order, int64_t norder,
 	int front, int tail_rows, int resident, int early, double beta, uint64_t *rowbits, int32_t *steps, int32_t *table, int32_t *info);
+int spp_tail_klast_host(int64_t n, int has_rhs, const uint64_t *words, int64_t nwords, const int32_t *step_order, int64_t norder,
+	int front, int tail_rows, int tail_mask, int32_t *klast);
 int spp_dense_posv_ordered(spp_ctx *ctx, double *d_A, int64_t n, int64_t ld, double *d_b, const uint64_t *words, int64_t nwords,
 	const int32_t *step_order);
 int spp_tail_step_order_host(int64_t n, const uint64_t *words, int64_t nwords, int32_t *step_order);
diff --git a/slam_plus_plus_amd/api.py b/slam_plus_plus_amd/api.py
--- a/slam_plus_plus_amd/api.py
+++ b/slam_plus_plus_amd/api.py
@@ -12,7 +12,7 @@
 INFO = dict(MODE=0, N=1, NNZB=2, NVALS=3, FACTOR_NNZ=4, FACTOR_FLOPS=5, N_REDUCED=6, N_POSES=7,
             N_LANDMARKS=8, SCHUR_PAIRS=9, N_OBS=10, SOLVE_BYTES=11, N_SUPERNODES=12, N_LEVELS=13, S_LD=14, S_NNZB=15, DENSE_STREAMED=16,
             LM_STREAM=17, BS_GROUPS=18, SCHUR_SIDE=19, S_CLEAR=20, S_DEVICE_PTR=21, ASM_HUB_CHUNK=22, SOLVE_ASYNC=23, FACTOR_KEPT=24,
-            SPARSE_FACTOR_KEPT=25, SCHUR_SPARSE_FACTOR_KEPT=26)
+            SPARSE_FACTOR_KEPT=25, SCHUR_SPARSE_FACTOR_KEPT=26, DENSE_FAILED_PIVOT=27)
 PHASES = ["permute", "schur_inv", "schur_gemm", "schur_rhs", "factor", "trisolve", "backsubst", "assemble", "total"]
 
 EXPORTS = [
@@ -35,7 +35,7 @@
     "spp_microbench_copy", "spp_microbench_mfma_f64", "spp_microbench_ctile", "spp_microbench_update", "spp_block_ordering", "spp_schur_plan_host", "spp_set_profiling", "spp_se2_linearize_device", "spp_se2_update_device", "spp_ba_linearize_device", "spp_ba_stereo_linearize_device", "spp_ba_update_device", "spp_sim3_ba_linearize_device", "spp_sim3_update_device", "spp_se3_linearize_device", "spp_se3_update_device", "spp_edge_chi2_device", "spp_edge_robust_weights_device", "spp_edge_hessian_maxdiag_device",
     "spp_lm_gain_denominator_device", "spp_dense_potrf_upper", "spp_dense_posv", "spp_dense_posv_multi",
     "spp_dense_posv_masked", "spp_tile_mask_host", "spp_schur_tile_mask_host", "spp_tail_order_host", "spp_tail_plan_host", "spp_schur_cam_order_host",
-    "spp_dense_posv_ordered", "spp_tail_step_order_host", "spp_schur_step_order_host",
+    "spp_dense_posv_ordered", "spp_tail_klast_host", "spp_tail_step_order_host", "spp_schur_step_order_host",
     "spp_dense_gemm_tn_sub", "spp_dense_gemm_tn_sub_upper", "spp_dense_front_factor", "spp_version",
 ]
 
@@ -148,6 +148,7 @@
         "spp_schur_cam_order_host": (cint, [i64, vp, vp, vp, cint, cint, cint, vp, vp, vp]),
         "spp_dense_posv_ordered": (cint, [vp, vp, i64, i64, vp, vp, i64, vp]),
         "spp_tail_step_order_host": (cint, [i64, vp, i64, vp]),
+        "spp_tail_klast_host": (cint, [i64, cint, vp, i64, vp, i64, cint, cint, cint, vp]),
         "spp_schur_step_order_host": (cint, [i64, vp, vp, vp, cint, cint, cint, vp]),
         "spp_dense_gemm_tn_sub": (cint, [vp, i64, i64, i64, vp, i64, vp, i64, vp, i64]),
         "spp_dense_gemm_tn_sub_upper": (cint, [vp, i64, i64, i64, vp, i64, vp, i64, vp, i64]),
@@ -284,6 +285,20 @@
             "info": dict(zip(("n_early", "r_star", "rows_resident", "live_demand", "widest"), (int(v) for v in info)))}
 
 
+def tail_klast_host(n, words, step_order=None, front=0, has_rhs=True, tail_rows=44, tail_mask=True):
+    lib = load_library()
+    words = np.ascontiguousarray(words if words is not None else [], dtype=np.uint64)
+    so = np.ascontiguousarray(step_order if step_order is not None else [], dtype=np.int32)
+    out = np.zeros(64, dtype=np.int32)
+    code = lib.spp_tail_klast_host(int(n), 1 if has_rhs else 0, _ptr(words) if words.size else None, words.size,
+                                   _ptr(so) if so.size else None, so.size, int(front), int(tail_rows), 1 if tail_mask else 0, _ptr(out))
+    if code < 0:
+        err = SppError("spp_tail_klast_host failed: %d" % code)
+        err.code = code
+        raise err
+    return out[:code].copy() if code else None
+
+
 def tail_step_order_host(n, words):
     lib = load_library()
     words = np.ascontiguousarray(words, dtype=np.uint64)
diff --git a/slam_plus_plus_amd/csrc/spp_api.cpp b/slam_plus_plus_amd/csrc/spp_api.cpp
--- a/slam_plus_plus_amd/csrc/spp_api.cpp
+++ b/slam_plus_plus_amd/csrc/spp_api.cpp
@@ -168,6 +168,7 @@
 	ctx->dense.tail_order.release();
 	ctx->dense.tail_plan.key = TailPlan::Key();
 	ctx->dense.tail_dinv.release();
+	ctx->dense.tail_ybuf.release();
 	ctx->dense.tail_epoch = 0;
 	ctx->dense.epoch = 0;
 	ctx->dense.sync.release();
@@ -411,7 +412,7 @@
 		return SPP_E_BADARG;
 	if(ctx->mode < 0 && what != SPP_INFO_NNZB && what != SPP_INFO_NVALS && what != SPP_INFO_N && what != SPP_INFO_DENSE_STREAMED &&
 	   what != SPP_INFO_ASM_HUB_CHUNK && what != SPP_INFO_FACTOR_KEPT && what != SPP_INFO_SPARSE_FACTOR_KEPT &&
-	   what != SPP_INFO_SCHUR_SPARSE_FACTOR_KEPT)
+	   what != SPP_INFO_SCHUR_SPARSE_FACTOR_KEPT && what != SPP_INFO_DENSE_FAILED_PIVOT)
 		return SPP_E_STATE;
 	switch(what) {
 	case SPP_INFO_MODE: *out = (ctx->mode != SPP_MODE_SCHUR) ? ctx->mode : ctx->schur.mis ? SPP_MODE_SCHUR_MIS :
@@ -432,6 +433,7 @@
 	case SPP_INFO_S_LD: *out = (ctx->mode == SPP_MODE_SCHUR && !ctx->schur.sparse_S) ? ctx->schur.ld : 0; break;
 	case SPP_INFO_S_NNZB: *out = (ctx->mode == SPP_MODE_SCHUR) ? ctx->schur.n_sblk : 0; break;
 	case SPP_INFO_DENSE_STREAMED: *out = ctx->dense.tail_rows_last; break;
+	case SPP_INFO_DENSE_FAILED_PIVOT: *out = ctx->dense.failed_pivot_last; break;
 	case SPP_INFO_LM_STREAM: *out = (ctx->mode == SPP_MODE_SCHUR) ? ctx->schur.lm_stream_last : 0; break;
 	case SPP_INFO_BS_GROUPS: *out = (ctx->mode == SPP_MODE_SCHUR) ? ctx->schur.n_bs : 0; break;
 	case SPP_INFO_SCHUR_SIDE: *out = (ctx->mode == SPP_MODE_SCHUR) ? ctx->schur.side_last : 0; break;
@@ -1521,6 +1523,30 @@
 	}
 }
 
+int spp_tail_klast_host(int64_t n, int has_rhs, const uint64_t *words, int64_t nwords, const int32_t *step_order, int64_t norder,
+	int front, int tail_rows, int tail_mask, int32_t *klast)
+{
+	const int64_t nsteps = (n + DENSE_NB - 1) / DENSE_NB;
+	if(n <= 0 || nwords < 0 || nwords > TAIL_MAX_ROWS || (nwords && (!words || nwords != nsteps)) || norder < 0 || (norder && !step_order) ||
+	   front < 0 || !klast)
+		return SPP_E_BADARG;
+	try {
+		const std::vector<uint64_t> mask(words, words + nwords);
+		const std::vector<int32_t> order(step_order, step_order + norder);
+		const TailSwitches sw = {tail_rows, tail_mask ? 1 : 0, 0, 0, 0.0};
+		const TailPlan p = tail_plan(nwords ? &mask : nullptr, norder ? &order : nullptr, nsteps, n, has_rhs ? n + 1 : n, (int64_t)front - 1, 0, sw);
+		if(!p.applies)
+			return 0;
+		for(int j = 0; j < p.key.Tr; ++ j)
+			klast[j] = p.klast[j];
+		return p.key.Tr;
+	} catch(const Error &e) {
+		return e.code;
+	} catch(...) {
+		return SPP_E_NOMEM;
+	}
+}
+
 int spp_tail_order_host(int64_t n, int has_rhs, const uint64_t *words, int64_t nwords, int resident, int early, double beta,
 	int32_t *table, int32_t *info)
 {
diff --git a/slam_plus_plus_amd/csrc/spp_dense.hip b/slam_plus_plus_amd/csrc/spp_dense.hip
--- a/slam_plus_plus_amd/csrc/spp_dense.hip
+++ b/slam_plus_plus_amd/csrc/spp_dense.hip
@@ -1258,13 +1258,15 @@
 	dw.tail_plan = std::move(plan);
 	const TailPlan &p = dw.tail_plan;
 	const int Tr = p.key.Tr, Tc = p.key.Tc, ntile = (int)p.table.size();
-	if(dw.tail_pub.cap < (size_t)Tr * Tc) {
-		dw.tail_pub.reserve(std::max<size_t>((size_t)Tr * Tc, 24 * 25));
+	if(dw.tail_pub.cap < (size_t)Tr * Tc + Tr) {
+		dw.tail_pub.reserve(std::max<size_t>((size_t)Tr * Tc + Tr, 24 * 26));
 		SPP_HIP_CHECK(hipMemsetAsync(dw.tail_pub.p, 0, dw.tail_pub.cap * sizeof(int), s));
 		dw.tail_epoch = 0;
 	}
 	if(dw.tail_dinv.cap < (size_t)Tr * 8 * 256)
 		dw.tail_dinv.reserve(std::max<size_t>((size_t)Tr * 8 * 256, (size_t)24 * 8 * 256));
+	if(dw.tail_ybuf.cap < (size_t)Tr * 16 * NB)
+		dw.tail_ybuf.reserve(std::max<size_t>((size_t)Tr * 16 * NB, (size_t)24 * 16 * NB));
 	if(++ dw.tail_epoch >= (1 << 26)) {
 		SPP_HIP_CHECK(hipMemsetAsync(dw.tail_pub.p, 0, dw.tail_pub.cap * sizeof(int), s));
 		dw.tail_epoch = 1;
@@ -1294,6 +1296,13 @@
 	a.has_rhs = has_rhs ? 1 : 0;
 	a.tinv = dw.tinv_all.p + (size_t)(k + 1) * NB * NB;
 	a.dbuf = dw.tail_dinv.p;
+	a.ybuf = dw.tail_ybuf.p;
+	a.ypub = dw.tail_pub.p + (size_t)Tr * Tc;
+	static_assert(sizeof(a.klast) == sizeof(p.klast), "one layout of the last steps");
+	if(sw.tail_self_last)
+		memcpy(a.klast, p.klast, sizeof(a.klast));
+	else
+		memset(a.klast, -1, sizeof(a.klast));
 	a.pub = dw.tail_pub.p;
 	a.epoch = dw.tail_epoch;
 	a.info = dw.info.p;
@@ -1319,11 +1328,12 @@
 		std::vector<long long> h((size_t)Tr * 8);
 		SPP_HIP_CHECK(hipStreamSynchronize(s));
 		SPP_HIP_CHECK(hipMemcpy(h.data(), trace.p, h.size() * sizeof(long long), hipMemcpyDeviceToHost));
-		fprintf(stderr, "[spp] streamed tail, %d tile rows, %d of %d tiles launched (us from the launch's first stamp): diagonal tile: updates complete / factored+inverted | first panel tile: first row tile seen / last seen / last published\n", Tr, ntile, Tr * Tc - Tr * (Tr - 1) / 2);
+		fprintf(stderr, "[spp] streamed tail, %d tile rows, %d of %d tiles launched (us from the launch's first stamp): diagonal tile: updates complete / factored+inverted | first panel tile: first row tile seen / last seen / last published | diagonal tile, last row tile of its last step formed by itself: Dinv_7 seen / X_7 formed\n", Tr, ntile, Tr * Tc - Tr * (Tr - 1) / 2);
 		const long long t0 = h[0];
 		for(int i = 0; i < Tr; ++ i)
-			fprintf(stderr, "  row %2d  start %7.1f  updated %7.1f  done %7.1f | %7.1f %7.1f %7.1f\n", i, (h[8 * i] - t0) * 0.01, (h[8 * i + 1] - t0) * 0.01,
-				(h[8 * i + 2] - t0) * 0.01, h[8 * i + 3] ? (h[8 * i + 3] - t0) * 0.01 : 0.0, h[8 * i + 4] ? (h[8 * i + 4] - t0) * 0.01 : 0.0, h[8 * i + 5] ? (h[8 * i + 5] - t0) * 0.01 : 0.0);
+			fprintf(stderr, "  row %2d  start %7.1f  updated %7.1f  done %7.1f | %7.1f %7.1f %7.1f | %7.1f %7.1f\n", i, (h[8 * i] - t0) * 0.01, (h[8 * i + 1] - t0) * 0.01,
+				(h[8 * i + 2] - t0) * 0.01, h[8 * i + 3] ? (h[8 * i + 3] - t0) * 0.01 : 0.0, h[8 * i + 4] ? (h[8 * i + 4] - t0) * 0.01 : 0.0, h[8 * i + 5] ? (h[8 * i + 5] - t0) * 0.01 : 0.0,
+				h[8 * i + 6] ? (h[8 * i + 6] - t0) * 0.01 : 0.0, h[8 * i + 7] ? (h[8 * i + 7] - t0) * 0.01 : 0.0);
 	}
 	return true;
 }
@@ -1616,6 +1626,7 @@
 int dense_info_eval(spp_ctx *ctx, const int *h_status4, bool *dag_aborted, bool drain_first)
 {
 	const int h_info[4] = {h_status4[0], h_status4[1], h_status4[2], h_status4[3]};
+	ctx->dense.failed_pivot_last = h_info[0];
 	if(drain_first && (h_info[0] | h_info[2] | h_info[3]))
 		SPP_HIP_CHECK(hipStreamSynchronize(ctx->stream));
 	if(h_info[3]) {
diff --git a/slam_plus_plus_amd/csrc/spp_dense_tail.h b/slam_plus_plus_amd/csrc/spp_dense_tail.h
--- a/slam_plus_plus_amd/csrc/spp_dense_tail.h
+++ b/slam_plus_plus_amd/csrc/spp_dense_tail.h
@@ -22,6 +22,9 @@
 	const int *order;
 	unsigned long long rowbits[TAIL_MAX_ROWS + 1];
 	unsigned long long sorder[TAIL_MAX_ROWS / 8 + 1];
+	signed char klast[TAIL_MAX_ROWS + 1];
+	double *ybuf;
+	int *ypub;
 };
 
 constexpr int TAIL_ABORT_TIMEOUT = 2;
@@ -51,6 +54,58 @@
 	__builtin_amdgcn_fence(__ATOMIC_ACQ_REL, "wavefront");
 	__builtin_amdgcn_wave_barrier();
 	diag_tile_factor<TS>(sm, potrf_lds2_dv(sm), potrf_lds2_gd0(sm), potrf_lds2_dinv(sm), 0, lane, potrf_lds2_fail(sm), info, k0);
+}
+
+constexpr int TAIL_PS = 18;
+
+__device__ __noinline__ bool tail_self_last_round(const double *y, const int *yflag, double *stage, double *img, int *st, const int *flag,
+	const int epoch, const double *dinv7, const WaitBound bound, const int ncol_live, long long *trace)
+{
+	const int tid = threadIdx.x, lane = tid & 63, wave = tid >> 6;
+	double *Ys = stage, *Dvs = stage + NB * PT;
+	if(tid == 0)
+		st[1] = bounded_wait<1, 1>(bound, TAIL_ABORT_TIMEOUT, [&]() {
+			const int v = wait_ld(flag);
+			return (v >> 4) == epoch && (v & 15) >= 8 && wait_ld(yflag) == ((epoch << 4) | 1);
+		}) ? 1 : -1;
+	lds_barrier();
+	const int ok = st[1];
+	if(ok < 0)
+		return false;
+	if(trace && tid == 0)
+		trace[6] = wall_clock64();
+	{
+		const int c = tid >> 4;
+		const double y0 = (c < ncol_live) ? tail_ld(y + tid) : 0.0, y1 = (c + 64 < ncol_live) ? tail_ld(y + tid + POTRF_THREADS) : 0.0;
+		double dv = 0;
+		if(tid < 256)
+			dv = tail_ld(dinv7 + tid);
+		Ys[(tid & 15) + c * PT] = y0;
+		Ys[(tid & 15) + (c + 64) * PT] = y1;
+		if(tid < 256)
+			Dvs[(tid & 15) + c * PT] = dv;
+	}
+	lds_barrier();
+	if(wave < 8) {
+		const int l15 = lane & 15, l4 = lane >> 4, live = ncol_live - 16 * wave;
+		const v4f64 x = tile_atb(Dvs, 1, PT, Ys + 16 * wave * PT, 1, PT, lane);
+#pragma unroll
+		for(int r = 0; r < 4; ++ r)
+			img[(4 * l4 + r) + (16 * wave + l15) * TAIL_PS] = (l15 < live) ? x[r] : 0.0;
+	}
+	if(trace && tid == 0)
+		trace[7] = wall_clock64();
+	return true;
+}
+
+__device__ __forceinline__ void tail_publish_y7(const double *T, double *y, const int lane, const int b, const int ncol_live)
+{
+	const int l15 = lane & 15, l4 = lane >> 4;
+	if(16 * b + l15 < ncol_live) {
+#pragma unroll
+		for(int r = 0; r < 4; ++ r)
+			__hip_atomic_store(y + (l4 + 4 * r) + 16 * (16 * b + l15), T[16 * 7 + (l4 + 4 * r) + (16 * b + l15) * TS], __ATOMIC_RELAXED, __HIP_MEMORY_SCOPE_AGENT);
+	}
 }
 
 __global__ __launch_bounds__(POTRF_THREADS)
@@ -126,7 +181,7 @@
 	bool pre_first = false;
 	{
 		const int ek = tid & 15, ec = tid >> 4;
-		constexpr int PS = 18;
+		constexpr int PS = TAIL_PS;
 		const int ekp = 4 * (ek & 3) + (ek >> 2);
 		unsigned long long ksteps = 0;
 		for(int k = a.have_pre ? -1 : 0; k < ti; ++ k) {
@@ -154,51 +209,13 @@
 				vb[h] = (!diag && cb < a.ncols) ? tail_ld(rowp + cb * a.ld) : 0.0;
 			}
 		};
+		const int self_sidx = (diag && nst > 0 && a.klast[ti] >= 0 && a.klast[ti] == tail_sorder_at(a.sorder, 63 - __builtin_clzll(steps))) ? nst - 1 : -1;
 		int avail = a.have_pre ? 8 : 0;
 		pre_first = diag && nst > 0 && (nst & 1) == 0 && a.rows - i0 >= 16;
 		bool inflight = false;
 		int k = a.have_pre ? -1 : 0;
 		int knext = steps ? tail_sorder_at(a.sorder, __builtin_ctzll(steps)) : k;
-		for(int sidx = 0; sidx < nst; ++ sidx) {
-			const int J = sidx & 7;
-			if(J == 0) {
-				k = knext;
-				steps &= steps - 1;
-				if(steps)
-					knext = tail_sorder_at(a.sorder, __builtin_ctzll(steps));
-			}
-			if(J == 0 && k >= 0)
-				avail = 0;
-			if(!inflight) {
-				if(J >= avail) {
-					avail = wait_pub(a.pub + k * a.Tc + ti, a.pub + k * a.Tc + tj, J + 1);
-					if(avail < 0)
-						return;
-				}
-				fetch(k, J);
-			}
-			int pk = -1;
-			if(tid == 0 && k >= 0 && J + 1 < 8 && J + 1 >= avail)
-				pk = pub_count(__hip_atomic_load(a.pub + k * a.Tc + ti, __ATOMIC_RELAXED, __HIP_MEMORY_SCOPE_AGENT),
-					__hip_atomic_load(a.pub + k * a.Tc + tj, __ATOMIC_RELAXED, __HIP_MEMORY_SCOPE_AGENT));
-			double *sa = sm + (sidx & 1) * 2 * NB * PS, *sb = diag ? sa : sa + NB * PS;
-#pragma unroll
-			for(int h = 0; h < 2; ++ h) {
-				sa[ekp + (ec + 64 * h) * PS] = va[h];
-				if(!diag)
-					sb[ekp + (ec + 64 * h) * PS] = vb[h];
-			}
-			if(tid == 0)
-				st[2 + (sidx & 1)] = pk;
-			lds_barrier();
-			{
-				const int seen = st[2 + (sidx & 1)];
-				if(seen > avail)
-					avail = seen;
-			}
-			inflight = (sidx + 1 < nst) && (J + 1 < 8) && (J + 1 < avail);
-			if(inflight)
-				fetch(k, J + 1);
+		auto update = [&](const double *sa, const double *sb, const int sidx) {
 			double fa[4];
 #pragma unroll
 			for(int u = 0; u < 4; ++ u) {
@@ -227,6 +244,57 @@
 					tail_first_tile(sm, acc[0], lane, a.info, i0);
 				}
 			}
+		};
+		for(int sidx = 0; sidx < (self_sidx >= 0 ? nst - 1 : nst); ++ sidx) {
+			const int J = sidx & 7;
+			if(J == 0) {
+				k = knext;
+				steps &= steps - 1;
+				if(steps)
+					knext = tail_sorder_at(a.sorder, __builtin_ctzll(steps));
+			}
+			if(J == 0 && k >= 0)
+				avail = 0;
+			if(!inflight) {
+				if(J >= avail) {
+					avail = wait_pub(a.pub + k * a.Tc + ti, a.pub + k * a.Tc + tj, J + 1);
+					if(avail < 0)
+						return;
+				}
+				fetch(k, J);
+			}
+			int pk = -1;
+			if(tid == 0 && k >= 0 && J + 1 < 8 && J + 1 >= avail)
+				pk = pub_count(__hip_atomic_load(a.pub + k * a.Tc + ti, __ATOMIC_RELAXED, __HIP_MEMORY_SCOPE_AGENT),
+					__hip_atomic_load(a.pub + k * a.Tc + tj, __ATOMIC_RELAXED, __HIP_MEMORY_SCOPE_AGENT));
+			double *sa = sm + (sidx & 1) * 2 * NB * PS, *sb = diag ? sa : sa + NB * PS;
+#pragma unroll
+			for(int h = 0; h < 2; ++ h) {
+				sa[ekp + (ec + 64 * h) * PS] = va[h];
+				if(!diag)
+					sb[ekp + (ec + 64 * h) * PS] = vb[h];
+			}
+			if(tid == 0)
+				st[2 + (sidx & 1)] = pk;
+			lds_barrier();
+			{
+				const int seen = st[2 + (sidx & 1)];
+				if(seen > avail)
+					avail = seen;
+			}
+			inflight = (sidx + 1 < nst) && (J + 1 < 8) && (J + 1 < avail);
+			if(inflight)
+				fetch(k, J + 1);
+			update(sa, sb, sidx);
+		}
+		if(self_sidx >= 0) {
+			double *sa = sm + (self_sidx & 1) * 2 * NB * PS;
+			const int64_t live = a.ncols - i0;
+			if(!tail_self_last_round(a.ybuf + (size_t)ti * 16 * NB, a.ypub + ti, sm + 4 * NB * PS, sa, st, a.pub + k * a.Tc + k, a.epoch,
+			   a.dbuf + ((size_t)k * 8 + 7) * 256, a.bound, live > NB ? NB : (int)live, a.trace ? a.trace + ti * 8 : nullptr))
+				return;
+			lds_barrier();
+			update(sa, sa, self_sidx);
 		}
 		lds_barrier();
 	}
@@ -257,6 +325,9 @@
 	const double *Rii = a.A + i0 + i0 * a.ld;
 	int avail = 0;
 	bool inflight = false;
+	const bool pub_y = tj < a.Tr && (int)a.klast[tj] == ti;
+	if(tid == 0)
+		st[4] = 0;
 	double dvr = 0, rr[2] = {0, 0};
 	auto fetch_panel = [&](const int J) {
 		if(tid < 256)
@@ -276,6 +347,14 @@
 					return;
 			}
 			fetch_panel(J);
+		}
+		if(J == 7 && pub_y && wave >= 8) {
+			asm volatile("s_waitcnt vmcnt(0)" ::: "memory");
+			int old_cnt = 0;
+			if(lane == 0)
+				old_cnt = __hip_atomic_fetch_add(&st[4], 1, __ATOMIC_RELAXED, __HIP_MEMORY_SCOPE_WORKGROUP);
+			if(lane == 0 && old_cnt == 7)
+				__hip_atomic_store(a.ypub + tj, tag | 1, __ATOMIC_RELAXED, __HIP_MEMORY_SCOPE_AGENT);
 		}
 		if(tj == ti + 1 && J == 0) stamp(3);
 		if(tj == ti + 1 && J == 7) stamp(4);
@@ -344,6 +423,10 @@
 			lds_barrier();
 			if(tid == 0)
 				__hip_atomic_store(a.pub + ti * a.Tc + tj, tag | (J + 1), __ATOMIC_RELAXED, __HIP_MEMORY_SCOPE_AGENT);
+			if(J == 6 && pub_y && wave >= 8) {
+				const int64_t live = a.ncols - j0;
+				tail_publish_y7(T, a.ybuf + (size_t)tj * 16 * NB, lane, wave - 8, live > NB ? NB : (int)live);
+			}
 			for(int I = J + 3 + (wave >> 3); I < 8; I += 2)
 				row_update(I);
 			lds_barrier();
diff --git a/slam_plus_plus_amd/csrc/spp_internal.h b/slam_plus_plus_amd/csrc/spp_internal.h
--- a/slam_plus_plus_amd/csrc/spp_internal.h
+++ b/slam_plus_plus_amd/csrc/spp_internal.h
@@ -289,6 +289,7 @@
 	bool masked = false;
 	bool ordered = false;
 	unsigned long long sorder[TAIL_SORDER_WORDS];
+	signed char klast[TAIL_MAX_ROWS + 1];
 	int resident = 0;
 	bool table_fresh = false;
 	std::vector<int> table;
@@ -304,6 +305,7 @@
 	DevBuf<int> flags;
 	DevBuf<int> tail_pub;
 	DevBuf<double> tail_dinv;
+	DevBuf<double> tail_ybuf;
 	int tail_epoch = 0;
 	DevBuf<int> tail_order;
 	TailPlan tail_plan;
@@ -311,6 +313,7 @@
 	const std::vector<uint64_t> *tile_mask = nullptr;
 	const std::vector<int32_t> *step_order = nullptr;
 	bool tail_masked_whole = false;
+	int failed_pivot_last = 0;
 	int tail_rows_last = 0;
 	bool tail_disabled = false;
 	DevBuf<double> trsv_m;
diff --git a/slam_plus_plus_amd/csrc/spp_switches.h b/slam_plus_plus_amd/csrc/spp_switches.h
--- a/slam_plus_plus_amd/csrc/spp_switches.h
+++ b/slam_plus_plus_amd/csrc/spp_switches.h
@@ -34,6 +34,7 @@
 	int tail_early;
 	int tail_step_order;
 	int tail_early_lead;
+	int tail_self_last;
 	long long tail_timeout_ticks;
 	int tail_trace;
 	int trsv_chain;
@@ -110,6 +111,7 @@
 	w.tail_early = env_int("SPP_TAIL_EARLY", 1);
 	w.tail_step_order = env_int("SPP_TAIL_STEP_ORDER", 1);
 	w.tail_early_lead = env_int("SPP_TAIL_EARLY_LEAD", 1);
+	w.tail_self_last = env_int("SPP_TAIL_SELF_LAST", 1);
 	w.tail_timeout_ticks = env_i64("SPP_TAIL_TIMEOUT_TICKS", WAIT_TICKS_DEFAULT);
 	w.tail_trace = env_int("SPP_TAIL_TRACE", 0);
 	w.trsv_chain = env_int("SPP_TRSV_CHAIN", 2);
diff --git a/slam_plus_plus_amd/csrc/spp_tile_plan.cpp b/slam_plus_plus_amd/csrc/spp_tile_plan.cpp
--- a/slam_plus_plus_amd/csrc/spp_tile_plan.cpp
+++ b/slam_plus_plus_amd/csrc/spp_tile_plan.cpp
@@ -196,6 +196,11 @@
 		ascending = ascending && list[n - 1] == q;
 	}
 	tail_sorder_pack(p.sorder, list, n);
+	std::fill(p.klast, p.klast + TAIL_MAX_ROWS + 1, (signed char)-1);
+	for(int j = 0; j < (int)Tr; ++ j)
+		for(int q = 0; q < n; ++ q)
+			if(list[q] < j && ((key.rowbits[(size_t)list[q] + 1] >> j) & 1))
+				p.klast[j] = (signed char)list[q];
 	key.early = p.masked && sw.tail_early != 0;
 	key.lead = key.early && !ascending && sw.tail_early_lead != 0;
 	p.resident = key.early ? resident : 0;
```

Measured after the change: 1.322 billion block-nnz/s. About the same (-0.4%).
